# amidos2006/gym-pcgrl

Hardware: AMD Instinct MI355X
Metric: env-steps/sec (whole node), binary-narrow 14x14 @ 65536 envs (higher is better)
Workload: dtype u8; 1 GPU; binary-narrow-v0 14x14, 65536 envs/GPU; envs_per_gpu=65536, width=14, height=14, max_changes=39, actions=uniform random, device-generated before the timed region, parallelism=env-axis shard x1, no collective on the step path

## Files before the change

### gym_pcgrl_amd/_lib.py

```python
import ctypes as C
import os
import subprocess

PKG = os.path.dirname(os.path.abspath(__file__))
ROOT = os.path.dirname(PKG)
CSRC = os.path.join(PKG, "csrc")
LIBDIR = os.path.join(PKG, "lib")
SO = os.path.join(LIBDIR, "libpcgrl_hip.so")
SOURCES = [os.path.join(CSRC, "pcgrl_abi.hip")]
HIPCC_FLAGS = ["--offload-arch=gfx950", "-O3", "-std=c++17", "-ffp-contract=off", "-fPIC", "-shared", "-mllvm", "-amdgpu-sched-strategy=max-ilp"]

PCGRL_OK, PCGRL_EINVAL, PCGRL_EHIP, PCGRL_ESTATE = 0, -1, -2, -3


class Config(C.Structure):
    _fields_ = [(n, C.c_int32) for n in (
        "prob", "rep", "num_envs", "width", "height", "prob_width", "prob_height", "max_changes", "max_iterations",
        "random_start", "random_tile", "warp", "random_probs", "auto_reset", "target_path",
        "max_enemies", "target_enemy_dist", "max_crates", "target_solution", "solver_power", "max_potions",
        "max_treasures", "max_diamonds", "min_spikes", "target_jumps", "min_empty", "min_enemies", "min_jumps")] + [
        ("target_col_enemies", C.c_double), ("tile_probs", C.c_double * 8), ("rewards", C.c_double * 12)]


class Layout(C.Structure):
    _fields_ = [(n, C.c_int32) for n in ("group", "mask_bytes", "nplanes", "nstats")] + [
        (n, C.c_size_t) for n in ("map", "old_map", "heatmap", "pos", "planes", "counters", "stats", "start_stats",
                                  "info", "reward", "done", "tile_p", "rng_rep", "rng_prob", "rng_cursor", "scratch")]


TUNING_FIELDS = ("no_fused", "fused_zelda", "step_epb", "no_inc", "inline_reset", "pair_min", "no_wide", "wide_waves", "wide_grid",
                 "wide_pairs", "wide_few", "sok_generic", "sok_hard_cap", "sok_spawn", "md_only_agent", "smb_lds_heap", "full_per_wave", "inc_per_wave", "wide_spin", "step_prio", "no_touch", "touch_tight", "step_pair", "async_split", "big_team", "obs_at_end", "touch_resume",
                 "changes_grid", "changes_chunk")


class Tuning(C.Structure):
    _fields_ = [(n, C.c_int32) for n in TUNING_FIELDS]


TUNING_OVERRIDES = {}


def make_tuning(overrides=None):
    t = Tuning(*([-1] * len(TUNING_FIELDS)))
    for k, v in list(TUNING_OVERRIDES.items()) + list((overrides or {}).items()):
        if k not in TUNING_FIELDS:
            raise KeyError("unknown tuning switch %r (known: %s)" % (k, ", ".join(TUNING_FIELDS)))
        setattr(t, k, int(v))
    return t


BUFFER_NAMES = ("map", "old_map", "heatmap", "pos", "planes", "counters", "stats", "start_stats", "info", "reward",
                "done", "tile_p", "rng_rep", "rng_prob", "rng_cursor", "scratch")


class Buffers(C.Structure):
    _fields_ = [(n, C.c_void_p) for n in BUFFER_NAMES]


ROW_FIELDS = ("actions_out", "reward", "done", "start_in", "start_out", "ep_return", "ep_length", "took", "fresh")


class Row(C.Structure):
    _fields_ = [(n, C.c_void_p) for n in ROW_FIELDS] + [("actions_i64", C.c_int32)]


class RenderDesc(C.Structure):
    _fields_ = [("indices", C.c_void_p), ("count", C.c_int32), ("tiles", C.c_void_p), ("tile_size", C.c_int32),
                ("border_x", C.c_int32), ("border_y", C.c_int32), ("border_tile", C.c_int32), ("cursor", C.c_int32),
                ("grid_rows", C.c_int32), ("grid_cols", C.c_int32), ("out", C.c_void_p)]


class TileGraphDesc(C.Structure):
    _fields_ = [("maps", C.c_void_p), ("count", C.c_int32), ("passable", C.c_uint32), ("source_tiles", C.c_uint32), ("reach_tiles", C.c_uint32),
                ("sources", C.c_void_p), ("regions_out", C.c_void_p), ("longest_out", C.c_void_p), ("labels_out", C.c_void_p),
                ("dist_out", C.c_void_p), ("reach_out", C.c_void_p), ("source_out", C.c_void_p)]


ABI_VERSION = 15
EXPORTS = ("pcgrl_abi_version", "pcgrl_error_string", "pcgrl_last_hip_error", "pcgrl_query_layout", "pcgrl_create",
           "pcgrl_destroy", "pcgrl_bind", "pcgrl_configure", "pcgrl_seed", "pcgrl_set_tile_probs", "pcgrl_reset",
           "pcgrl_step", "pcgrl_set_maps", "pcgrl_observe", "pcgrl_action_map", "pcgrl_status", "pcgrl_profile",
           "pcgrl_profile_read", "pcgrl_bind_episode_stats", "pcgrl_seed_words", "pcgrl_rollout", "pcgrl_bind_observation", "pcgrl_selftest_heap",
           "pcgrl_tuning_defaults", "pcgrl_set_tuning", "pcgrl_clear_status", "pcgrl_step_flat",
           "pcgrl_async_bytes", "pcgrl_bind_async", "pcgrl_step_async", "pcgrl_async_flush", "pcgrl_step_multi", "pcgrl_selftest_step_pool", "pcgrl_step_threads", "pcgrl_selftest_range_reward",
           "pcgrl_bind_row", "pcgrl_render", "pcgrl_get_stats_bytes", "pcgrl_get_stats", "pcgrl_get_reward",
           "pcgrl_get_solution_bytes", "pcgrl_get_solution", "pcgrl_get_playthrough_bytes", "pcgrl_get_playthrough",
           "pcgrl_get_smb_play_bytes", "pcgrl_get_smb_play", "pcgrl_get_paths_legs", "pcgrl_get_paths_bytes", "pcgrl_get_paths",
           "pcgrl_get_changes_bytes", "pcgrl_get_changes", "pcgrl_tile_graph_bytes", "pcgrl_tile_graph")
NPHASE = 6
PHASES = ("update", "stats", "reset_or_idle", "solver_or_reset", "reset2", "solver2")


def sources_newer_than_lib():
    if not os.path.exists(SO):
        return True
    t = os.path.getmtime(SO)
    deps = [os.path.join(CSRC, f) for f in os.listdir(CSRC)] + [os.path.join(ROOT, "include", "pcgrl_hip.h")]
    return any(os.path.getmtime(d) > t for d in deps)


def source_hash():
    import hashlib
    h = hashlib.sha256()
    files = sorted(os.path.join(CSRC, f) for f in os.listdir(CSRC)) + [os.path.join(ROOT, "include", "pcgrl_hip.h")]
    h.update(" ".join(HIPCC_FLAGS).encode() + b"\0")
    for f in files:
        h.update(os.path.basename(f).encode() + b"\0")
        with open(f, "rb") as fh:
            h.update(fh.read())
    return h.hexdigest()[:16]


NPARTS = 8


def build(force=False, verbose=False, jobs=None):
    if not force and not sources_newer_than_lib():
        return SO
    os.makedirs(LIBDIR, exist_ok=True)
    objdir = os.path.join(LIBDIR, "obj")
    os.makedirs(objdir, exist_ok=True)
    hipcc = os.environ.get("HIPCC", "hipcc")
    flags = [f for f in HIPCC_FLAGS if f != "-shared"]
    jobs = jobs or int(os.environ.get("PCGRL_BUILD_JOBS", "0")) or min(NPARTS, os.cpu_count() or 1)
    objs = [os.path.join(objdir, "part%d.o" % k) for k in range(NPARTS)]
    cmds = [[hipcc] + flags + ["-DPCGRL_PART=%d" % k, "-c", SOURCES[0], "-o", objs[k]] for k in range(NPARTS)]
    running, todo, failed = [], list(range(NPARTS)), []
    while todo or running:
        while todo and len(running) < jobs:
            k = todo.pop(0)
            if verbose:
                print(" ".join(cmds[k]), flush=True)
            running.append((k, subprocess.Popen(cmds[k])))
        k, p = running.pop(0)
        if p.wait() != 0:
            failed.append(k)
    if failed:
        raise subprocess.CalledProcessError(1, cmds[failed[0]])
    link = [hipcc, "--offload-arch=gfx950", "-shared", "-fPIC"] + objs + ["-o", SO]
    if verbose:
        print(" ".join(link), flush=True)
    subprocess.check_call(link)
    return SO


_lib = None


def load():
    global _lib, SO
    if _lib is not None:
        return _lib
    SO = os.environ.get("PCGRL_HIP_SO", SO)
    if not os.path.exists(SO):
        raise RuntimeError(
            "gym_pcgrl_amd: HIP library %s is missing. Build it with `python -c 'import __graft_entry__ as g; g.build()'` "
            "(hipcc --offload-arch=gfx950). There is no CPU fallback for the batched environment." % SO)
    import torch
    L = C.CDLL(SO)
    for name in EXPORTS:
        if not hasattr(L, name):
            raise RuntimeError("gym_pcgrl_amd: %s does not export %s (stale build?)" % (SO, name))
    L.pcgrl_abi_version.restype = C.c_int
    if L.pcgrl_abi_version() != ABI_VERSION:
        raise RuntimeError("gym_pcgrl_amd: %s has ABI version %d, this package needs %d (stale build?)" % (SO, L.pcgrl_abi_version(), ABI_VERSION))
    L.pcgrl_error_string.restype = C.c_char_p
    L.pcgrl_error_string.argtypes = [C.c_int]
    L.pcgrl_last_hip_error.restype = C.c_int
    L.pcgrl_query_layout.argtypes = [C.POINTER(Config), C.POINTER(Layout)]
    L.pcgrl_create.argtypes = [C.POINTER(Config), C.POINTER(C.c_void_p)]
    L.pcgrl_destroy.argtypes = [C.c_void_p]
    L.pcgrl_tuning_defaults.argtypes = [C.POINTER(Tuning)]
    L.pcgrl_tuning_defaults.restype = None
    L.pcgrl_set_tuning.argtypes = [C.c_void_p, C.POINTER(Tuning)]
    L.pcgrl_bind.argtypes = [C.c_void_p, C.POINTER(Buffers), C.c_void_p]
    L.pcgrl_configure.argtypes = [C.c_void_p, C.POINTER(Config)]
    L.pcgrl_seed.argtypes = [C.c_void_p, C.c_void_p, C.c_int32, C.c_int32, C.c_void_p]
    L.pcgrl_seed_words.argtypes = [C.c_void_p, C.c_void_p, C.c_int32, C.c_int32, C.c_void_p]
    L.pcgrl_set_tile_probs.argtypes = [C.c_void_p, C.c_void_p]
    L.pcgrl_reset.argtypes = [C.c_void_p, C.c_void_p]
    L.pcgrl_step.argtypes = [C.c_void_p, C.c_void_p, C.c_void_p]
    L.pcgrl_rollout.argtypes = [C.c_void_p, C.c_void_p, C.c_int32, C.c_void_p, C.c_void_p, C.c_void_p, C.c_void_p]
    L.pcgrl_set_maps.argtypes = [C.c_void_p, C.c_void_p, C.c_void_p]
    L.pcgrl_observe.argtypes = [C.c_void_p, C.c_void_p, C.c_int32, C.c_int32, C.c_int32, C.c_int32, C.c_int32, C.c_void_p]
    L.pcgrl_bind_observation.argtypes = [C.c_void_p, C.c_void_p, C.c_int32, C.c_int32, C.c_int32, C.c_int32, C.c_int32, C.c_int32]
    L.pcgrl_bind_row.argtypes = [C.c_void_p, C.POINTER(Row)]
    L.pcgrl_render.argtypes = [C.c_void_p, C.POINTER(RenderDesc), C.c_void_p]
    L.pcgrl_get_stats_bytes.argtypes = [C.POINTER(Config), C.c_int32]
    L.pcgrl_get_stats_bytes.restype = C.c_size_t
    L.pcgrl_get_stats.argtypes = [C.c_void_p, C.c_void_p, C.c_int32, C.c_void_p, C.c_void_p, C.c_size_t, C.c_void_p]
    L.pcgrl_get_reward.argtypes = [C.c_void_p, C.c_void_p, C.c_void_p, C.c_int32, C.c_void_p, C.c_void_p, C.c_void_p]
    moves_args = (C.c_void_p, C.c_void_p, C.c_int32, C.c_int32, C.c_void_p, C.c_void_p, C.c_void_p, C.c_void_p, C.c_void_p, C.c_size_t, C.c_void_p)
    for name in ("pcgrl_get_solution", "pcgrl_get_playthrough", "pcgrl_get_smb_play"):
        getattr(L, name + "_bytes").argtypes = [C.POINTER(Config), C.c_int32, C.c_int32]
        getattr(L, name + "_bytes").restype = C.c_size_t
        getattr(L, name).argtypes = list(moves_args)
    L.pcgrl_get_paths_legs.argtypes = [C.POINTER(Config)]
    L.pcgrl_get_paths_legs.restype = C.c_int32
    L.pcgrl_get_paths_bytes.argtypes = [C.POINTER(Config), C.c_int32, C.c_int32]
    L.pcgrl_get_paths_bytes.restype = C.c_size_t
    L.pcgrl_get_paths.argtypes = [C.c_void_p, C.c_void_p, C.c_int32, C.c_int32, C.c_void_p, C.c_void_p, C.c_void_p, C.c_void_p, C.c_size_t, C.c_void_p]
    L.pcgrl_get_changes_bytes.argtypes = [C.POINTER(Config), C.c_int32, C.c_int32]
    L.pcgrl_get_changes_bytes.restype = C.c_size_t
    L.pcgrl_get_changes.argtypes = [C.c_void_p, C.c_void_p, C.c_int32, C.c_void_p, C.c_int32, C.c_void_p, C.c_void_p, C.c_void_p, C.c_void_p, C.c_void_p,
                                    C.c_void_p, C.c_size_t, C.c_void_p]
    L.pcgrl_tile_graph_bytes.argtypes = [C.POINTER(Config), C.c_int32]
    L.pcgrl_tile_graph_bytes.restype = C.c_size_t
    L.pcgrl_tile_graph.argtypes = [C.c_void_p, C.POINTER(TileGraphDesc), C.c_void_p, C.c_size_t, C.c_void_p]
    L.pcgrl_action_map.argtypes = [C.c_void_p, C.c_void_p, C.c_void_p, C.c_void_p]
    L.pcgrl_step_flat.argtypes = [C.c_void_p, C.c_void_p, C.c_void_p, C.c_void_p]
    L.pcgrl_selftest_heap.argtypes = [C.c_void_p, C.c_int32, C.c_void_p, C.c_void_p, C.c_void_p, C.c_void_p]
    L.pcgrl_selftest_step_pool.argtypes = [C.c_int32, C.c_int32, C.c_int32, C.c_void_p]
    L.pcgrl_selftest_range_reward.argtypes = [C.c_void_p, C.c_int32, C.c_void_p, C.c_void_p]
    L.pcgrl_step_threads.argtypes = [C.c_int32]
    L.pcgrl_step_threads.restype = C.c_int32
    L.pcgrl_status.argtypes = [C.c_void_p, C.c_void_p, C.POINTER(C.c_int32)]
    L.pcgrl_clear_status.argtypes = [C.c_void_p, C.c_void_p]
    L.pcgrl_profile.argtypes = [C.c_void_p, C.c_int]
    L.pcgrl_bind_episode_stats.argtypes = [C.c_void_p, C.c_void_p, C.c_void_p, C.c_void_p, C.c_void_p, C.c_void_p]
    L.pcgrl_profile_read.argtypes = [C.c_void_p, C.POINTER(C.c_double), C.POINTER(C.c_int32)]
    L.pcgrl_async_bytes.argtypes = [C.POINTER(Config), C.c_int32]
    L.pcgrl_async_bytes.restype = C.c_size_t
    L.pcgrl_bind_async.argtypes = [C.c_void_p, C.c_void_p, C.c_size_t, C.c_int32, C.c_void_p]
    L.pcgrl_step_async.argtypes = [C.c_void_p, C.c_void_p, C.c_int32, C.c_void_p]
    L.pcgrl_async_flush.argtypes = [C.c_void_p, C.c_void_p]
    L.pcgrl_step_multi.argtypes = [C.POINTER(C.c_void_p), C.POINTER(C.c_void_p), C.POINTER(C.c_void_p), C.c_int32]
    _lib = L
    return L


def check(rc, what):
    if rc != 0:
        L = load()
        msg = L.pcgrl_error_string(rc).decode()
        extra = " (hipError %d)" % L.pcgrl_last_hip_error() if rc == PCGRL_EHIP else ""
        raise RuntimeError("gym_pcgrl_amd: %s failed: %s%s" % (what, msg, extra))
```

### gym_pcgrl_amd/csrc/kernels_stats.h

```cpp
#pragma once
template <class MaskT>
__device__ __forceinline__ MaskT row_valid(int lane, int W, int H) {
    MaskT full = (W >= (int)(8 * sizeof(MaskT))) ? ~(MaskT)0 : (((MaskT)1 << W) - 1);
    return lane < H ? full : (MaskT)0;
}

template <int PROB = -1>
__device__ __forceinline__ bool finalize_item(const PcgrlParams& P, const DevBufs& B, int e, const int32_t* s,
                                              int mode, int parity, int shard, bool push_reset = true, int rst_list = WL_RST,
                                              const int2* pre = nullptr, const double* reward_pre = nullptr) {
    const int prob = PROB >= 0 ? PROB : P.prob;
    int32_t* st = B.stats + (size_t)e * 8;
    int32_t* start = B.start_stats + (size_t)e * 8;
    if (mode == MODE_STEP) {
        int32_t old[PCGRL_MAX_STATS], sv[PCGRL_MAX_STATS];
        for (int k = 0; k < 8; k++) { old[k] = st[k]; sv[k] = start[k]; }
        const int2 c = pre ? *pre : reinterpret_cast<const int2*>(B.counters)[e];
        const double r = reward_pre ? *reward_pre : compute_reward(P, s, old, prob);
        const bool d = episode_over(P, s, sv, prob) || c.y >= P.max_changes || c.x >= P.max_iterations;
        B.reward[e] = r;
        B.done[e] = d ? 1 : 0;
        episode_account(B, e, r, d);
        int32_t* inf = B.info + (size_t)e * 10;
#pragma unroll
        for (int k = 0; k < 8; k++) {
            st[k] = s[k];
            inf[k] = (prob == PCGRL_PROB_BINARY && k == 2) ? s[1] - sv[1] : ((prob == PCGRL_PROB_BINARY && k == 3) ? 0 : s[k]);
        }
        inf[8] = c.x; inf[9] = c.y;
        if (d && P.auto_reset && push_reset) wl_push(B, parity, rst_list, shard, e);
        return d && P.auto_reset;
    } else {
        for (int k = 0; k < 8; k++) st[k] = s[k];
        if (mode == MODE_START)
            for (int k = 0; k < 8; k++) start[k] = s[k];
    }
    return false;
}

template <int PROB, class G, class MaskT>
__device__ __forceinline__ bool compute_item_stats(G& g, const PcgrlParams& P, MaskT b0, MaskT b1, MaskT b2, MaskT valid, int32_t* s,
                                                   int32_t* status, MaskT& champ, bool tight = true) {
    champ = 0;
    if (PROB == PCGRL_PROB_BINARY) {
        int regions, path;
        if (G::kGroup == 16) {
            int ub2;
            regions_and_longest_path(g, (MaskT)(~b0 & valid), regions, path, champ, ub2, tight);
            s[3] = ub2 + 1;
        } else {
            regions_and_longest_path(g, (MaskT)(~b0 & valid), regions, path, champ);
        }
        s[0] = regions; s[1] = path; s[2] = g.any(champ) ? 1 : 0;
        return false;
    }
    if (PROB == PCGRL_PROB_ZELDA) { zelda_stats(g, P, b0, b1, b2, valid, s); return false; }
    if (PROB == PCGRL_PROB_MDUNGEON) return mdungeon_stats(g, P, b0, b1, b2, valid, s);
    if (PROB == PCGRL_PROB_DDAVE) {
        bool overflow = false;
        const bool ns = ddave_stats(g, P, b0, b1, b2, valid, s, &overflow);
        if (overflow && g.lane == 0) atomicOr(status, PCGRL_STATUS_TOO_MANY_CRATES);
        return ns;
    }
    if (PROB == PCGRL_PROB_SMB) return true;
    return sokoban_stats(g, P, b0, b1, b2, valid, s);
}
template <int PROB, class G, class MaskT>
__device__ __forceinline__ bool compute_item_stats(G& g, const PcgrlParams& P, MaskT b0, MaskT b1, MaskT b2, MaskT valid, int32_t* s, int32_t* status) {
    MaskT champ;
    return compute_item_stats<PROB>(g, P, b0, b1, b2, valid, s, status, champ);
}

template <int PROB = -1>
__device__ __forceinline__ bool finish_or_park(const PcgrlParams& P, const DevBufs& B, int e, const int32_t* s, bool need_solver,
                                               int mode, int parity, int shard, bool push_reset = true, int park_list = -1,
                                               const double* reward_pre = nullptr) {
    if (need_solver) {
        int32_t* park = (mode == MODE_STEP) ? B.info + (size_t)e * 10 : B.stats + (size_t)e * 8;
        for (int k = 0; k < 8; k++) park[k] = s[k];
        wl_push(B, parity, park_list >= 0 ? park_list : (mode == MODE_STEP ? WL_SOL : WL_SOL2), shard, e);
        return false;
    }
    return finalize_item<PROB>(P, B, e, s, mode, parity, shard, push_reset, WL_RST, nullptr, reward_pre);
}

template <int J>
__device__ __forceinline__ double dpp_down(double v) {
    const long long b = __double_as_longlong(v);
    const int lo = __builtin_amdgcn_update_dpp(0, (int)b, 0x100 + J, 0xF, 0xF, true), hi = __builtin_amdgcn_update_dpp(0, (int)(b >> 32), 0x100 + J, 0xF, 0xF, true);
    return __longlong_as_double(((long long)hi << 32) | (unsigned)lo);
}
__device__ __forceinline__ void zelda_reward_tab(const PcgrlParams& P, ZeldaRewardTab* T) {
    T->w[0] = P.rewards[0]; T->w[1] = P.rewards[1]; T->w[2] = P.rewards[2]; T->w[3] = P.rewards[4]; T->w[4] = P.rewards[3];
    T->w[5] = P.rewards[5]; T->w[6] = P.rewards[6]; T->w[7] = 0.0;
    T->lo[0] = 1; T->lo[1] = 1; T->lo[2] = 1; T->lo[3] = 2; T->lo[4] = 1; T->lo[5] = P.target_enemy_dist; T->lo[6] = PCGRL_IPOS; T->lo[7] = 0;
    T->hi[0] = 1; T->hi[1] = 1; T->hi[2] = 1; T->hi[3] = P.max_enemies; T->hi[4] = 1; T->hi[5] = PCGRL_IPOS; T->hi[6] = PCGRL_IPOS; T->hi[7] = 0;
}
__device__ __forceinline__ double zelda_reward_lanes(const ZeldaRewardTab* T, const int32_t* old, const int32_t* s, int k) {
    const int s0 = s[0], s1 = s[1], s2 = s[2], s3 = s[3], s4 = s[4], s5 = s[5], s6 = s[6];
    int n = s6;
    n = k == 5 ? s5 : n; n = k == 4 ? s4 : n; n = k == 3 ? s3 : n; n = k == 2 ? s2 : n; n = k == 1 ? s1 : n; n = k == 0 ? s0 : n;
    const int kk = k & 7;
    const int o = old[kk];
    const double t = k < 7 ? (double)range_reward_i(n, o, T->lo[kk], T->hi[kk]) * T->w[kk] : 0.0;
    double r = t;
    r = r + dpp_down<1>(t); r = r + dpp_down<2>(t); r = r + dpp_down<3>(t);
    r = r + dpp_down<4>(t); r = r + dpp_down<5>(t); r = r + dpp_down<6>(t);
    return r;
}

template <int PROB, int G, class MaskT, bool FUSED = false>
__device__ __forceinline__ void stats_wave_task(const PcgrlParams& P, const DevBufs& B, DevGroup<G, MaskT>& g, int lane64, int gw, bool lone,
                                                bool inc, bool pair, bool zinc, bool have, int raw, int shard, int mode, int parity,
                                                int inline_reset, int gen_map, uint32_t* mt, uint8_t* tiles, MaskT rowmask,
                                                StepLocal* SL = nullptr, bool step_obs = false) {
    constexpr bool kCanReset = PROB == PCGRL_PROB_BINARY || PROB == PCGRL_PROB_ZELDA;
    if (!kCanReset) inline_reset = 0;
    constexpr int GPW = 64 / G;
    constexpr bool kInc = PROB == PCGRL_PROB_BINARY;
    constexpr bool kZinc = PROB == PCGRL_PROB_ZELDA && G == 16 && sizeof(MaskT) == 4;
    constexpr int NPL = (PROB == PCGRL_PROB_BINARY) ? 1 : 3;
    MaskT* champ_base = reinterpret_cast<MaskT*>(B.champ);
    const bool tch = kInc && G == 16 && !inc && !lone && have && raw < 0;
    const bool packed = inc || (kZinc && zinc && !lone) || tch;
    const bool reset_only = have && !packed && (raw & WL_RESET_ONLY) != 0;
    const bool compute = have && !reset_only && !(lone && (gw & 1));
    const int e = packed ? wl_inc_env<G>(raw) : (raw & ~WL_RESET_ONLY);
    MaskT* planes_e = reinterpret_cast<MaskT*>(B.planes) + (size_t)e * NPL * G;
    MaskT b0 = 0, b1 = 0, b2 = 0;
    if (compute) {
        b0 = planes_e[g.lane * NPL];
        if (NPL > 1) { b1 = planes_e[g.lane * NPL + 1]; b2 = planes_e[g.lane * NPL + 2]; }
    }
    if (GPW >= 2 && lone && inline_reset) {
        const int role = gw & 1;
        int2 pre = make_int2(0, 0);
        if (g.lane == 0 && role == 0 && have) pre = reinterpret_cast<const int2*>(B.counters)[e];
        asm volatile("s_waitcnt vmcnt(0)" ::: "memory");
#pragma unroll
        for (int k = 0; k < GPW / 2; k++) {
            if (k > 0 && !pair) break;
            if (!__builtin_amdgcn_readlane((int)have, 2 * k * G)) continue;
            const int ek = __builtin_amdgcn_readlane(e, 2 * k * G);
            const int step_draws = (SL && P.rep == PCGRL_REP_NARROW && P.random_tile) ? 1 : 0;
            if (SL && lane64 == 0) SL->dirty[ek - SL->e0] = 1;
            ResetRows rr;
            wave_reset_env<PROB, !FUSED, FUSED>(P, B, ek, gen_map, mt, (uint8_t*)nullptr, lane64, step_draws, gw == 2 * k + 1 ? g.lane : -1, &rr);
            MaskT t0, t1, t2;
            reset_rows_to_planes<MaskT>(P, reinterpret_cast<MaskT*>(B.planes) + (size_t)ek * NPL * G, gw == 2 * k + 1 ? g.lane : -1, rr.m0, rr.m1, rr.m2, t0, t1, t2);
            if (gw == 2 * k + 1) { b0 = t0; b1 = t1; b2 = t2; }
            __builtin_amdgcn_wave_barrier();
        }
        TL(9);
        const bool act = have && (role == 1 || !reset_only);
        int32_t sl[PCGRL_MAX_STATS] = {0, 0, 0, 0, 0, 0, 0, 0};
        MaskT champ_l = 0;
        bool ns = false;
        if (act) ns = compute_item_stats<PROB>(g, P, b0, b1, b2, rowmask, sl, B.status, champ_l, (B.step_tight & 2) != 0);
        TL(10);
        constexpr bool kLaneReward = PROB == PCGRL_PROB_ZELDA && G == 16;
        double rpre = 0.0;
        if (kLaneReward && SL && role == 0 && act) rpre = zelda_reward_lanes(&SL->zr, B.stats + (size_t)e * 8, sl, g.lane);
        if (g.lane == 0 && role == 0 && act) finalize_item<PROB>(P, B, e, sl, MODE_STEP, parity, shard, false, WL_RST, &pre, (kLaneReward && SL) ? &rpre : nullptr);
        __builtin_amdgcn_wave_barrier();
        if (role == 1 && have) {
            if (kInc && champ_base) champ_base[(size_t)e * G + g.lane] = champ_l;
            if (g.lane == 0) finish_or_park<PROB>(P, B, e, sl, ns, MODE_START, parity, shard);
        }
        if (FUSED && step_obs) {
#pragma unroll
            for (int k = 0; k < GPW / 2; k++) {
                if (k > 0 && !pair) break;
                if (!__builtin_amdgcn_readlane((int)have, 2 * k * G)) continue;
                const ObsPlanes<MaskT, NPL> src = {reinterpret_cast<const MaskT*>(B.planes), G};
                obs_write_env_lean(src, obs_view_from_lds(&SL->obs_v), B.pos, __builtin_amdgcn_readlane(e, 2 * k * G), lane64);
            }
        }
        return;
    }
    int32_t s[PCGRL_MAX_STATS] = {0, 0, 0, 0, 0, 0, 0, 0};
    bool need_solver = false;
    MaskT champ = 0;
    if (kInc && inc) {
        if (compute) {
            const MaskT cbit = (g.lane == wl_inc_row<G>(raw)) ? (MaskT)1 << wl_inc_col<G>(raw) : (MaskT)0;
            const MaskT champ_old = champ_base[(size_t)e * G + g.lane];
            const int4 old = *reinterpret_cast<const int4*>(B.stats + (size_t)e * 8);
            int regions, path, ub2;
            binary_incremental(g, (MaskT)(~b0 & rowmask), cbit, wl_inc_code<G>(raw) != 0, old.x, old.y, champ_old, old.w - 1, regions, path, champ, ub2);
            s[0] = regions; s[1] = path; s[2] = 1; s[3] = ub2 + 1;
        }
    } else if (kZinc && packed) {
        if (compute) {
            const MaskT cbit = (g.lane == wl_inc_row<G>(raw)) ? (MaskT)1 << wl_inc_col<G>(raw) : (MaskT)0;
            zelda_stats(g, P, b0, b1, b2, rowmask, s, (int)wl_inc_code<G>(raw), cbit, B.stats[(size_t)e * 8 + 4]);
        }
    } else {
        bool full = compute;
        if (kInc && G == 16) {
            const bool t = compute && tch;
            TouchMemo<MaskT> memo = touch_memo_empty(g, b0);
            if (t) {
                const MaskT cbit = (g.lane == wl_inc_row<G>(raw)) ? (MaskT)1 << wl_inc_col<G>(raw) : (MaskT)0;
                const MaskT champ_old = champ_base[(size_t)e * G + g.lane];
                const int4 old = *reinterpret_cast<const int4*>(B.stats + (size_t)e * 8);
                int regions, path, ub2;
                if (binary_touch(g, (MaskT)(~b0 & rowmask), cbit, (wl_inc_code<G>(raw) & 1u) != 0, old.x, champ_old, old.w - 1, regions, path, champ, ub2, memo)) {
                    s[0] = regions; s[1] = path; s[2] = 1; s[3] = ub2 + 1;
                    full = false;
                }
            }
#ifdef PCGRL_TIMELINE
            {
                const uint64_t gu = __ballot(t && full && g.lane == 0), pl = __ballot(compute && !tch && g.lane == 0);
                TL(32 + __popcll(gu) + 8 * __popcll(pl));
            }
#endif
            constexpr bool kResume = FUSED && sizeof(MaskT) == 4;
            if (kResume && B.touch_resume) {
                if (full) {
                    int regions, path, ub2;
                    rlp_resume(g, (MaskT)(~b0 & rowmask), memo, regions, path, champ, ub2, (B.step_tight & 1) != 0);
                    s[0] = regions; s[1] = path; s[2] = g.any(champ) ? 1 : 0; s[3] = ub2 + 1;
                }
                full = false;
            }
        }
        if (full) need_solver = compute_item_stats<PROB>(g, P, b0, b1, b2, rowmask, s, B.status, champ, (B.step_tight & 1) != 0);
    }
    if (kInc && compute && champ_base) champ_base[(size_t)e * G + g.lane] = champ;
    TL(10);
    int want_reset = 0;
    constexpr bool kLaneReward = PROB == PCGRL_PROB_ZELDA && G == 16;
    double rpre = 0.0;
    const bool lane_reward = kLaneReward && SL != nullptr && mode == MODE_STEP;
    if (lane_reward && have && !reset_only) rpre = zelda_reward_lanes(&SL->zr, B.stats + (size_t)e * 8, s, g.lane);
    if (g.lane == 0 && have) {
        if (reset_only) want_reset = 1;
        else want_reset = finish_or_park<PROB>(P, B, e, s, need_solver, mode, parity, shard, !inline_reset, -1, lane_reward ? &rpre : nullptr) ? 1 : 0;
    }
    if (inline_reset) {
        const uint64_t want = __ballot(want_reset != 0);
        TL(11);
        if (want) {
            TL(12);
            if (SL) { while (__hip_atomic_load(&SL->refill_done[SL->par], __ATOMIC_ACQUIRE, __HIP_MEMORY_SCOPE_WORKGROUP) < SL->need) __builtin_amdgcn_s_sleep(2); }
            bool mine = false;
#pragma unroll
            for (int k = 0; k < GPW; k++) {
                if ((want >> (k * G)) & 1ull) {
                    const int ek = __builtin_amdgcn_readlane(e, k * G);
                    if (SL && lane64 == 0) { SL->dirty[ek - SL->e0] = 1; SL->late[ek - SL->e0] = 1; SL->n_late = 1; }
                    int pend = 0;
                    if (SL) {
                        if (lane64 == 0) {
                            pend = atomicExch(&SL->pend[ek - SL->e0], 0);
                            if (pend < 0) {
                                while (__hip_atomic_load(&SL->late_done[(ek - SL->e0) >> 6], __ATOMIC_ACQUIRE, __HIP_MEMORY_SCOPE_WORKGROUP) == 0) __builtin_amdgcn_s_sleep(2);
                                pend = 0;
                            }
                        }
                        pend = __builtin_amdgcn_readfirstlane(pend);
                    }
                    ResetRows rr;
                    wave_reset_env<PROB, !FUSED, FUSED>(P, B, ek, gen_map, mt, (uint8_t*)nullptr, lane64, 0, gw == k ? g.lane : -1, &rr, pend);
                    MaskT t0, t1, t2;
                    reset_rows_to_planes<MaskT>(P, reinterpret_cast<MaskT*>(B.planes) + (size_t)ek * NPL * G, gw == k ? g.lane : -1, rr.m0, rr.m1, rr.m2, t0, t1, t2);
                    if (gw == k) { b0 = t0; b1 = t1; b2 = t2; mine = true; }
                    __builtin_amdgcn_wave_barrier();
                }
            }
            if (mine) {
                int32_t st[PCGRL_MAX_STATS] = {0, 0, 0, 0, 0, 0, 0, 0};
                const bool ns = compute_item_stats<PROB>(g, P, b0, b1, b2, rowmask, st, B.status, champ, (B.step_tight & 2) != 0);
                if (kInc && champ_base) champ_base[(size_t)e * G + g.lane] = champ;
                if (g.lane == 0) finish_or_park<PROB>(P, B, e, st, ns, MODE_START, parity, shard);
            }
        }
    }
}

template <int PROB, int G, class MaskT>
__global__ __launch_bounds__(PCGRL_BLOCK) __attribute__((amdgpu_waves_per_eu(4, 8))) void k_stats(PcgrlParams P, DevBufs B, int list, int parity, int mode, int clear_parity,
                                                        int inline_reset, int gen_map, int lone0) {
    extern __shared__ __attribute__((aligned(16))) uint8_t smem[];
    __shared__ int s_pref[WL_NSHARD + 1], s_pref_inc[WL_NSHARD + 1], s_pref_rst[WL_NSHARD + 1];
    if (clear_parity >= 0 && blockIdx.x == 0) wl_clear(B, clear_parity);
    DevGroup<G, MaskT> g;
    constexpr int GPB = PCGRL_BLOCK / G, GPW = 64 / G;
    constexpr bool kInc = PROB == PCGRL_PROB_BINARY;
    constexpr bool kZinc = PROB == PCGRL_PROB_ZELDA && G == 16 && sizeof(MaskT) == 4;
    const bool zinc = kZinc && mode == MODE_STEP && B.zelda_inc;
    const bool with_inc = (kInc && mode == MODE_STEP && B.champ != nullptr) || zinc;
    int n_inc = 0, n_rst = 0;
    const int n_full = (with_inc || lone0 == 2 || list < 0) ? wl_load_prefix3(B, parity, list, with_inc ? WL_INC : -1, lone0 == 2 ? WL_RST : -1,
                                                                              s_pref, s_pref_inc, s_pref_rst, &n_inc, &n_rst)
                                                             : wl_load_prefix(B, parity, list, s_pref);
    const int n0 = lone0 == 1 ? s_pref[1] : (lone0 == 2 ? n_rst : 0);
    const int f0 = lone0 == 1 ? n0 : 0;
    const int w_full = (n_full - f0 + GPW - 1) / GPW;
    const bool pair = GPW >= 4 && n0 >= B.pair_min;
    const int w_lone = pair ? (n0 + 1) >> 1 : n0;
    const int w_total = w_lone + w_full + (n_inc + GPW - 1) / GPW;
    MaskT* champ_base = reinterpret_cast<MaskT*>(B.champ);
    const int lane64 = threadIdx.x & 63, wv = threadIdx.x >> 6, gw = lane64 / G;
    const int NPL = (PROB == PCGRL_PROB_BINARY) ? 1 : 3;
    const int W = P.width, H = P.height;
    uint32_t* mt = reinterpret_cast<uint32_t*>(smem + (size_t)wv * reset_stage_bytes(W * H));
    uint8_t* tiles = reinterpret_cast<uint8_t*>(mt + PCGRL_MT_N);
    const MaskT rowmask = row_valid<MaskT>(g.lane, W, H);
    for (int wid = blockIdx.x * (PCGRL_BLOCK / 64) + wv; wid < w_total; wid += gridDim.x * (PCGRL_BLOCK / 64)) {
        const bool lone = wid < w_lone;
        const bool inc = wid >= w_lone + w_full;
        const int item = lone ? (pair ? 2 * wid + (gw >> 1) : wid) : (inc ? (wid - w_lone - w_full) * GPW + gw : f0 + (wid - w_lone) * GPW + gw);
        const bool have = lone ? (item < n0 && (pair || gw < 2)) : item < (inc ? n_inc : n_full);
        const bool from_rst = lone && lone0 == 2;
        const int raw = !have ? 0 : (inc ? wl_get(B, WL_INC, s_pref_inc, item) : (from_rst ? wl_get(B, WL_RST, s_pref_rst, item) : wl_get(B, list, s_pref, item)));
        const int shard = (item >> 4) & (WL_NSHARD - 1);
        stats_wave_task<PROB, G, MaskT>(P, B, g, lane64, gw, lone, inc, pair, zinc, have, raw, shard, mode, parity, inline_reset, gen_map, mt, tiles, rowmask);
    }
}

template <class MaskT>
struct LdsShared {
    MaskT* rest; int* bestp; int lane;
    __device__ __forceinline__ MaskT load_rest() const { return *reinterpret_cast<volatile MaskT*>(rest + lane); }
    template <class G>
    __device__ __forceinline__ bool retire(G& g, MaskT comp) const {
        const MaskT fb = g.first_bit(comp);
        MaskT old = 0;
        if (fb) old = atomicAnd(rest + lane, ~fb);
        const bool won = __ballot((old & fb) != 0) != 0;
        if (comp) atomicAnd(rest + lane, ~comp);
        return won;
    }
    __device__ __forceinline__ int best() const { return *reinterpret_cast<volatile int*>(bestp); }
    __device__ __forceinline__ void raise(int v) const { if (lane == 0 && v > 0) atomicMax(bestp, v); }
};
template <class MaskT>
__device__ __forceinline__ void block_regions_and_path(DevGroup<64, MaskT>& g, MaskT pass, int tw, int ts, int lane, int H,
                                                       MaskT* s_rest, int* s_regions, int* s_best, int* s_owner, MaskT* champ_e) {
    const int bh = (H + ts - 1) / ts;
    const int row_lo = tw * bh, row_hi = (row_lo + bh < H) ? row_lo + bh : H;
    int tiny_regions, tiny_path;
    TL(20);
    const MaskT nontiny = rlp_prepare(g, pass, tiny_regions, tiny_path);
    TL(21);
    if (tw == 0) {
        s_rest[lane] = nontiny;
        if (lane == 0) { *s_regions = tiny_regions; *s_best = tiny_path; *s_owner = -1; }
    }
    __syncthreads();
    LdsShared<MaskT> sh = {s_rest, s_best, lane};
    int regions = 0, my_best = 0;
    MaskT my_champ = 0;
    MaskT rest = sh.load_rest();
    if (g.any(rest)) {
        const PcgFillCtx<DevGroup<64, MaskT>> ctx = pcg_fill_ctx(g, pass);
        do {
            rlp_process_seed(g, rlp_choose_seed(g, rest, row_lo, row_hi), ctx, sh, regions, my_best, my_champ);
            rest = sh.load_rest();
        } while (g.any(rest));
    }
    TL(22);
    if (lane == 0 && regions) atomicAdd(s_regions, regions);
    __syncthreads();
    TL(23);
    if (lane == 0 && my_best > tiny_path && my_best == *s_best) atomicCAS(s_owner, -1, tw);
    __syncthreads();
    if (champ_e) {
        const int owner = *s_owner;
        if (tw == (owner < 0 ? 0 : owner)) champ_e[lane] = owner < 0 ? (MaskT)0 : my_champ;
    }
}

template <class MaskT>
__device__ __forceinline__ void wave_incremental_item(const PcgrlParams& P, const DevBufs& B, DevGroup<64, MaskT>& g, int raw, int parity,
                                                      int inline_reset, int gen_map, uint32_t* mt, uint8_t* tiles, int lane, MaskT rowmask) {
    const int e = wl_inc_env<64>(raw);
    MaskT* planes_e = reinterpret_cast<MaskT*>(B.planes) + (size_t)e * 64;
    MaskT* champ_e = reinterpret_cast<MaskT*>(B.champ) + (size_t)e * 64;
    const MaskT b0 = planes_e[lane];
    const MaskT champ_old = champ_e[lane];
    const int2 old = *reinterpret_cast<const int2*>(B.stats + (size_t)e * 8);
    const MaskT cbit = (lane == wl_inc_row<64>(raw)) ? (MaskT)1 << wl_inc_col<64>(raw) : (MaskT)0;
    int regions, path;
    MaskT champ;
    binary_incremental(g, (MaskT)(~b0 & rowmask), cbit, wl_inc_code<64>(raw) != 0, old.x, old.y, champ_old, regions, path, champ);
    champ_e[lane] = champ;
    int want = 0;
    if (lane == 0) {
        int32_t s[PCGRL_MAX_STATS] = {regions, path, 1, 0, 0, 0, 0, 0};
        want = finalize_item<PCGRL_PROB_BINARY>(P, B, e, s, MODE_STEP, parity, e & (WL_NSHARD - 1), !inline_reset) ? 1 : 0;
    }
    want = __builtin_amdgcn_readfirstlane(want);
    if (inline_reset && want) {
        ResetRows rr;
        wave_reset_env<PCGRL_PROB_BINARY>(P, B, e, gen_map, mt, (uint8_t*)nullptr, lane, 0, lane, &rr);
        MaskT n0, n1, n2;
        reset_rows_to_planes<MaskT>(P, planes_e, lane, rr.m0, rr.m1, rr.m2, n0, n1, n2);
        int32_t st[PCGRL_MAX_STATS] = {0, 0, 0, 0, 0, 0, 0, 0};
        compute_item_stats<PCGRL_PROB_BINARY>(g, P, n0, n1, n2, rowmask, st, B.status, champ);
        champ_e[lane] = champ;
        if (lane == 0) finalize_item<PCGRL_PROB_BINARY>(P, B, e, st, MODE_START, parity, e & (WL_NSHARD - 1));
    }
}

#define WIDE_SPIN_LIMIT 400
__device__ __forceinline__ int wide_claim(int32_t* word, int epoch, int who) {
    int cur = __hip_atomic_load(word, __ATOMIC_RELAXED, __HIP_MEMORY_SCOPE_AGENT);
    for (;;) {
        if ((cur >> 1) == epoch) return 0;
        const int seen = atomicCAS(word, cur, (epoch << 1) | who);
        if (seen == cur) return 1;
        cur = seen;
    }
}

template <class MaskT, int NWAVES>
__global__ __launch_bounds__(NWAVES * 64) void k_stats_wide(PcgrlParams P, DevBufs B, int list, int parity, int mode, int clear_parity,
                                                             int inline_reset, int gen_map, int pair_few) {
    extern __shared__ __attribute__((aligned(16))) uint8_t smem[];
    __shared__ int s_pref[WL_NSHARD + 1], s_pref_rst[WL_NSHARD + 1], s_pref_inc[WL_NSHARD + 1];
    __shared__ MaskT s_rest[2][64];
    __shared__ int s_regions[2], s_best[2], s_owner[2], s_flag, s_flag2[2], s_cur, s_claim;
    __shared__ int2 s_pre;
    if (clear_parity >= 0 && blockIdx.x == 0) wl_clear(B, clear_parity);
// ... 167 lines not shown
```

### gym_pcgrl_amd/csrc/kernels_step.h

```cpp
#pragma once

struct StepLds { int planes, champ, stats, start, cnt, cur, fifo, tag, pos, act, flat, in_total, info, rew, done, total; };
__host__ __device__ constexpr StepLds step_lds_layout(int plane_row_bytes, int champ_row_bytes, bool fifo, int action_width, int epb) {
    StepLds L = {};
    int o = 0;
    L.planes = o; o += epb * plane_row_bytes;
    L.champ = o; o += epb * champ_row_bytes;
    L.stats = o; o += epb * 32;
    L.start = o; o += epb * 32;
    L.cnt = o; o += epb * 8;
    L.cur = o; o += epb * 8;
    L.fifo = o; o += fifo ? epb * PCGRL_FIFO_N * 4 : 0;
    L.tag = o; o += fifo ? epb * 4 : 0;
    L.pos = o; o += epb * 2;
    L.act = o; o += epb * 4 * action_width;
    L.flat = o; o += action_width == 3 ? epb * 4 : 0;
    L.in_total = o;
    L.info = o; o += epb * 40;
    L.rew = o; o += epb * 8;
    L.done = o; o += epb;
    L.total = (o + 15) & ~15;
    return L;
}

template <int TPB>
__device__ __forceinline__ void blk_copy(uint8_t* dst, const uint8_t* src, int bytes) {
    const int nv = bytes >> 4;
    for (int i = threadIdx.x; i < nv; i += TPB) reinterpret_cast<uint4*>(dst)[i] = reinterpret_cast<const uint4*>(src)[i];
    for (int i = (nv << 4) + threadIdx.x; i < bytes; i += TPB) dst[i] = src[i];
}
template <int TPB>
__device__ __forceinline__ void blk_copy_rows(uint8_t* dst, const uint8_t* src, int rows, int row, const uint8_t* flag) {
    const int per = row >> 4;
    for (int i = threadIdx.x; i < rows * per; i += TPB)
        if (flag[i / per]) reinterpret_cast<uint4*>(dst)[i] = reinterpret_cast<const uint4*>(src)[i];
}

template <int TPB, int C, int SLOT0, int NV>
__device__ __forceinline__ void seg_load_c(uint4& rc, const void* g, bool on, int tid) {
    if (C * TPB + TPB - 1 < SLOT0 || C * TPB >= SLOT0 + NV) return;
    const int slot = C * TPB + tid;
    if (on && slot >= SLOT0 && slot < SLOT0 + NV) rc = reinterpret_cast<const uint4*>(g)[slot - SLOT0];
}
#define PCGRL_SEG_LOAD(SLOT0, NV, G, ON) do { const void* g_ = (G); const bool on_ = (ON); \
    seg_load_c<TPB, 0, SLOT0, NV>(r0, g_, on_, tid0); seg_load_c<TPB, 1, SLOT0, NV>(r1, g_, on_, tid0); seg_load_c<TPB, 2, SLOT0, NV>(r2, g_, on_, tid0); \
    seg_load_c<TPB, 3, SLOT0, NV>(r3, g_, on_, tid0); seg_load_c<TPB, 4, SLOT0, NV>(r4, g_, on_, tid0); seg_load_c<TPB, 5, SLOT0, NV>(r5, g_, on_, tid0); \
    seg_load_c<TPB, 6, SLOT0, NV>(r6, g_, on_, tid0); seg_load_c<TPB, 7, SLOT0, NV>(r7, g_, on_, tid0); seg_load_c<TPB, 8, SLOT0, NV>(r8, g_, on_, tid0); } while (0)
template <int TPB, int C, int TOTAL>
__device__ __forceinline__ void seg_store_c(uint8_t* smem, const uint4& rc, int tid) {
    if (C * TPB >= TOTAL) return;
    const int slot = C * TPB + tid;
    if (slot < TOTAL) reinterpret_cast<uint4*>(smem)[slot] = rc;
}

__device__ __forceinline__ void fifo_refill(const DevBufs& B, int e, int k, int cur0) {
    uint32_t* ring = B.rng_rep + (size_t)e * PCGRL_MT_N;
    uint32_t* fl = B.fifo + (size_t)e * PCGRL_FIFO_N;
    const int base = mt_wrap(cur0 + PCGRL_FIFO_N), basem = mt_wrap(base + PCGRL_MT_M);
    uint32_t a[PCGRL_FIFO_N + 1], m[PCGRL_FIFO_N];
#pragma unroll
    for (int i = 0; i <= PCGRL_FIFO_N; i++) a[i] = (i <= k) ? ring[mt_wrap(base + i)] : 0u;
#pragma unroll
    for (int i = 0; i < PCGRL_FIFO_N; i++) m[i] = (i < k) ? ring[mt_wrap(basem + i)] : 0u;
#pragma unroll
    for (int i = 0; i < PCGRL_FIFO_N; i++) if (i < k) ring[mt_wrap(cur0 + i)] = fl[i];
#pragma unroll
    for (int j = 0; j < PCGRL_FIFO_N; j++) if (j + k < PCGRL_FIFO_N) fl[j] = fl[j + k];
#pragma unroll
    for (int i = 0; i < PCGRL_FIFO_N; i++) if (i < k) fl[PCGRL_FIFO_N - k + i] = mt_twist(a[i], a[i + 1], m[i]);
    B.fifo_tag[e] = mt_wrap(cur0 + k);
}

__device__ __forceinline__ void step_set_prio(int p) {
    if (p == 0) __builtin_amdgcn_s_setprio(0);
    else if (p == 1) __builtin_amdgcn_s_setprio(1);
    else if (p == 2) __builtin_amdgcn_s_setprio(2);
    else __builtin_amdgcn_s_setprio(3);
}

template <int PROB, int REP, class MaskT, bool MULTI, int EPB, bool OBS = false, bool ROW = false>
__global__ __launch_bounds__(EPB * 4) __attribute__((amdgpu_waves_per_eu(4, 8))) void k_step(PcgrlParams P, DevBufs Bg, const int32_t* __restrict__ actions, int parity, int gen_map,
                                                                                                     int steps, size_t action_stride, double* reward_out, uint8_t* done_out, int32_t* info_out) {
    extern __shared__ __attribute__((aligned(16))) uint8_t smem[];
    constexpr int TPB = EPB * 4, NUPD = EPB / 64;
    __shared__ int s_items[3][EPB];
    __shared__ int s_n[2][4];
    __shared__ StepLocal s_loc;
    __shared__ int s_obs_ticket;
    static_assert(!(OBS && MULTI), "the tape form writes its images at the end");
    static_assert(!(ROW && MULTI), "the tape form has its own outputs (pcgrl_rollout ignores the row binding)");
    constexpr int G = 16, GPW = 4;
    constexpr int NPL = (PROB == PCGRL_PROB_BINARY) ? 1 : 3;
    constexpr int kPlaneRow = G * NPL * (int)sizeof(MaskT);
    const int W = P.width, H = P.height;
    TL_INIT(); TL(1);
    const int e0 = blockIdx.x * EPB;
    const int ne = (P.num_envs - e0) < EPB ? (P.num_envs - e0) : EPB;
    const bool has_champ = PROB == PCGRL_PROB_BINARY && Bg.champ != nullptr;
    const bool has_fifo = REP == PCGRL_REP_NARROW && Bg.fifo != nullptr;
    constexpr int kChampRow = PROB == PCGRL_PROB_BINARY ? G * (int)sizeof(MaskT) : 0;
    constexpr int AW = REP == PCGRL_REP_WIDE ? 3 : 1;
    constexpr StepLds L = step_lds_layout(kPlaneRow, kChampRow, REP == PCGRL_REP_NARROW, AW, EPB);
    const int champ_row = kChampRow;
    DevBufs B = Bg;
    const size_t cells_ = (size_t)W * H;
    B.map = Bg.map + (size_t)e0 * cells_;
    B.old_map = Bg.old_map + (size_t)e0 * cells_;
    B.heat = Bg.heat + (size_t)e0 * cells_;
    B.tile_p = Bg.tile_p + (size_t)e0 * 2;
    B.rng_rep = Bg.rng_rep + (size_t)e0 * PCGRL_MT_N;
    if (Bg.rng_prob) B.rng_prob = Bg.rng_prob + (size_t)e0 * PCGRL_MT_N;
    if (Bg.ep_return) { B.ep_return = Bg.ep_return + e0; B.ep_length = Bg.ep_length + e0; B.last_return = Bg.last_return + e0; B.last_length = Bg.last_length + e0; }
    B.planes = smem + L.planes;
    if (has_champ) B.champ = smem + L.champ;
    B.stats = reinterpret_cast<int32_t*>(smem + L.stats);
    B.start_stats = reinterpret_cast<int32_t*>(smem + L.start);
    B.info = reinterpret_cast<int32_t*>(smem + L.info);
    B.reward = reinterpret_cast<double*>(smem + L.rew);
    B.counters = reinterpret_cast<int32_t*>(smem + L.cnt);
    B.rng_cur = reinterpret_cast<int32_t*>(smem + L.cur);
    if (has_fifo) {
        B.fifo = reinterpret_cast<uint32_t*>(smem + L.fifo);
        B.fifo_tag = reinterpret_cast<int32_t*>(smem + L.tag);
    } else {
        B.fifo = nullptr; B.fifo_tag = nullptr;
    }
    B.pos = smem + L.pos;
    B.done = smem + L.done;
    const int32_t* act_lds = reinterpret_cast<const int32_t*>(smem + L.act);
    const uint8_t* g_planes = reinterpret_cast<const uint8_t*>(Bg.planes) + (size_t)e0 * kPlaneRow;
    const uint8_t* g_champ = has_champ ? reinterpret_cast<const uint8_t*>(Bg.champ) + (size_t)e0 * champ_row : nullptr;
    const bool row_fl = ROW && AW == 3 && Bg.flat;
    const int row_per = row_fl ? 1 : AW;
    const size_t row_a0 = (size_t)e0 * row_per + threadIdx.x;
    const bool row_have = ROW && (int)threadIdx.x < ne * row_per;
    int64_t row_act = 0;
    static_assert(AW <= 4, "one action value per thread");
    if (row_have) {
        const int32_t* src = row_fl ? Bg.flat : actions;
        row_act = Bg.act_i64 ? reinterpret_cast<const int64_t*>(src)[row_a0] : (int64_t)src[row_a0];
    }
    if (ne == EPB) {
        static_assert(L.in_total / 16 <= 9 * TPB, "nine 16-byte slots per thread");
        uint4 r0 = {}, r1 = {}, r2 = {}, r3 = {}, r4 = {}, r5 = {}, r6 = {}, r7 = {}, r8 = {};
        const int tid0 = (int)threadIdx.x;
        PCGRL_SEG_LOAD(L.planes / 16, EPB * kPlaneRow / 16, g_planes, true);
        if (kChampRow) PCGRL_SEG_LOAD(L.champ / 16, (kChampRow ? EPB * kChampRow / 16 : 1), g_champ, has_champ);
        PCGRL_SEG_LOAD(L.stats / 16, EPB * 2, Bg.stats + (size_t)e0 * 8, true);
        PCGRL_SEG_LOAD(L.start / 16, EPB * 2, Bg.start_stats + (size_t)e0 * 8, true);
        PCGRL_SEG_LOAD(L.cnt / 16, EPB / 2, Bg.counters + (size_t)e0 * 2, true);
        PCGRL_SEG_LOAD(L.cur / 16, EPB / 2, Bg.rng_cur + (size_t)e0 * 2, true);
        if (REP == PCGRL_REP_NARROW) {
            PCGRL_SEG_LOAD(L.fifo / 16, EPB * PCGRL_FIFO_N * 4 / 16, has_fifo ? Bg.fifo + (size_t)e0 * PCGRL_FIFO_N : nullptr, has_fifo);
            PCGRL_SEG_LOAD(L.tag / 16, EPB / 4, has_fifo ? Bg.fifo_tag + e0 : nullptr, has_fifo);
        }
        PCGRL_SEG_LOAD(L.pos / 16, EPB / 8, Bg.pos + (size_t)e0 * 2, true);
        if (!ROW) PCGRL_SEG_LOAD(L.act / 16, EPB / 4 * AW, actions + (size_t)e0 * AW, !(AW == 3 && Bg.flat));
        if (!ROW && AW == 3) PCGRL_SEG_LOAD(L.flat / 16, (AW == 3 ? EPB / 4 : 1), Bg.flat ? Bg.flat + e0 : nullptr, Bg.flat != nullptr);
        asm volatile("" ::: "memory");
        static_assert(L.act % 16 == 0, "the prefetch ends on a slot boundary in front of the actions");
        constexpr int TOT = (ROW ? L.act : L.in_total) / 16;
        seg_store_c<TPB, 0, TOT>(smem, r0, tid0); seg_store_c<TPB, 1, TOT>(smem, r1, tid0); seg_store_c<TPB, 2, TOT>(smem, r2, tid0);
        seg_store_c<TPB, 3, TOT>(smem, r3, tid0); seg_store_c<TPB, 4, TOT>(smem, r4, tid0); seg_store_c<TPB, 5, TOT>(smem, r5, tid0);
        seg_store_c<TPB, 6, TOT>(smem, r6, tid0); seg_store_c<TPB, 7, TOT>(smem, r7, tid0); seg_store_c<TPB, 8, TOT>(smem, r8, tid0);
    } else {
        blk_copy<TPB>(smem + L.planes, g_planes, ne * kPlaneRow);
        if (has_champ) blk_copy<TPB>(smem + L.champ, g_champ, ne * champ_row);
        blk_copy<TPB>(smem + L.stats, reinterpret_cast<const uint8_t*>(Bg.stats + (size_t)e0 * 8), ne * 32);
        blk_copy<TPB>(smem + L.start, reinterpret_cast<const uint8_t*>(Bg.start_stats + (size_t)e0 * 8), ne * 32);
        blk_copy<TPB>(smem + L.cnt, reinterpret_cast<const uint8_t*>(Bg.counters + (size_t)e0 * 2), ne * 8);
        blk_copy<TPB>(smem + L.cur, reinterpret_cast<const uint8_t*>(Bg.rng_cur + (size_t)e0 * 2), ne * 8);
        blk_copy<TPB>(smem + L.pos, Bg.pos + (size_t)e0 * 2, ne * 2);
        if (has_fifo) {
            blk_copy<TPB>(smem + L.fifo, reinterpret_cast<const uint8_t*>(Bg.fifo + (size_t)e0 * PCGRL_FIFO_N), ne * PCGRL_FIFO_N * 4);
            blk_copy<TPB>(smem + L.tag, reinterpret_cast<const uint8_t*>(Bg.fifo_tag + e0), ne * 4);
        }
        if (ROW) {}
        else if (AW == 3 && Bg.flat) blk_copy<TPB>(smem + L.flat, reinterpret_cast<const uint8_t*>(Bg.flat + e0), ne * 4);
        else blk_copy<TPB>(smem + L.act, reinterpret_cast<const uint8_t*>(actions + (size_t)e0 * AW), ne * 4 * AW);
    }
    if (row_have) {
        reinterpret_cast<int32_t*>(smem + (row_fl ? L.flat : L.act))[threadIdx.x] = (int32_t)row_act;
        if (Bg.row.actions_out) Bg.row.actions_out[row_a0] = row_act;
    }
    if (threadIdx.x < EPB) { s_loc.dirty[threadIdx.x] = 0; if (OBS) { s_loc.obs_skip[threadIdx.x] = 0; s_loc.late[threadIdx.x] = 0; } }
    if (threadIdx.x < 8) s_n[threadIdx.x >> 2][threadIdx.x & 3] = 0;
    if (threadIdx.x == 0) { s_loc.e0 = 0; s_loc.need = NUPD; s_loc.refill_done[0] = 0; s_loc.refill_done[1] = 0; s_loc.n_late = 0; s_obs_ticket = 0; }
    constexpr int OBS_PER_TASK = 8;
    const bool obs_delta = OBS && REP == PCGRL_REP_WIDE && NPL == 3 && Bg.obs.delta;
    const int n_obs = (OBS && !obs_delta) ? (ne + OBS_PER_TASK - 1) / OBS_PER_TASK : 0;
    const ObsPlanes<MaskT, NPL> obs_src = {reinterpret_cast<const MaskT*>(smem + L.planes), G};
    if (OBS && threadIdx.x == 0) s_loc.obs_v = obs_view(P, Bg.obs, e0);
    if (PROB == PCGRL_PROB_ZELDA && threadIdx.x == 64) zelda_reward_tab(P, &s_loc.zr);
    uint8_t* reset_scratch = smem + L.total;
#pragma clang loop unroll(disable)
  for (int t = 0; t < (MULTI ? steps : 1); t++) {
    int tid = (int)threadIdx.x;
    if (MULTI) asm volatile("" : "+v"(tid));
    const int lane64 = tid & 63, wv = tid >> 6, gw = lane64 / G;
    const int sp = t & 1;
    DevGroup<G, MaskT> g(lane64);
    if (MULTI && t > 0) {
        const int32_t* row = actions + (size_t)t * action_stride + (size_t)e0 * AW;
        for (int i = tid; i < ne * AW; i += TPB) reinterpret_cast<int32_t*>(smem + L.act)[i] = row[i];
    }
    __syncthreads();
    TL(17);
    const int prio = B.step_prio, prio_nfull = (prio >> 8) & 15;
    int prio_now = 0;
    if (wv < NUPD) {
        if ((prio >> 6) & 3) { prio_now = (prio >> 6) & 3; step_set_prio(prio_now); }
        const int e = wv * 64 + lane64;
        UpdateOut u = {};
        UpdateMid mid = {};
        if (REP == PCGRL_REP_WIDE && !MULTI && Bg.flat && e < ne) {
            const int dim = P.ntiles, total = W * H * dim;
            int a = reinterpret_cast<const int32_t*>(smem + L.flat)[e];
            if (a < 0 || a >= total) atomicOr(B.status, PCGRL_STATUS_BAD_ACTION);
            a = a < 0 ? 0 : (a >= total ? total - 1 : a);
            int32_t* t3 = reinterpret_cast<int32_t*>(smem + L.act) + 3 * e;
            const int q = a / dim;
            t3[0] = q % W; t3[1] = q / W; t3[2] = a - q * dim;
        }
        if (e < ne) u = update_env<REP, MaskT, true, true, true>(P, B, act_lds, e, &mid);
        TL(2);
        const bool first = u.rst || u.sure_done;
        const bool packed_full = PROB == PCGRL_PROB_ZELDA && B.zelda_inc;
        int dest = -1, v = e;
        if (first) { dest = 0; v = u.rst ? (e | WL_RESET_ONLY) : e; }
        else if (u.chg) { dest = u.cheap ? 2 : 1; v = (u.cheap || packed_full) ? u.inc_item : ((u.touch && B.step_touch) ? (u.inc_item | (int)0x80000000) : e); }
        if (u.chg) s_loc.dirty[e] = 1;
        if (OBS && first && e < EPB) s_loc.obs_skip[e] = 1;
        const uint64_t m0 = __ballot(dest == 0), m1 = __ballot(dest == 1), m2 = __ballot(dest == 2);
        const uint64_t below = (1ull << lane64) - 1ull;
        int b0 = 0, b1 = 0, b2 = 0;
        if (lane64 == 0) {
            b0 = m0 ? atomicAdd(&s_n[sp][0], __popcll(m0)) : 0;
            b1 = m1 ? atomicAdd(&s_n[sp][1], __popcll(m1)) : 0;
            b2 = m2 ? atomicAdd(&s_n[sp][2], __popcll(m2)) : 0;
            if (wv == 0) { s_n[sp ^ 1][0] = 0; s_n[sp ^ 1][1] = 0; s_n[sp ^ 1][2] = 0; s_n[sp ^ 1][3] = 0; s_loc.refill_done[sp ^ 1] = 0; s_loc.par = sp; }
        }
        b0 = __builtin_amdgcn_readfirstlane(b0); b1 = __builtin_amdgcn_readfirstlane(b1); b2 = __builtin_amdgcn_readfirstlane(b2);
        if (dest == 0) s_items[0][b0 + __popcll(m0 & below)] = v;
        if (dest == 2) s_items[2][b2 + __popcll(m2 & below)] = v;
        {
            const int lvl = (u.bucket >> 3) & 7;
            int pos1 = 0;
#pragma unroll
            for (int b = 0; b < 8; b++) {
                const uint64_t mb = __ballot(dest == 1 && lvl == b);
                pos1 += b > lvl ? __popcll(mb) : (b == lvl ? __popcll(mb & below) : 0);
            }
            if (dest == 1) s_items[1][b1 + pos1] = v;
        }
        asm volatile("s_waitcnt lgkmcnt(0)" ::: "memory");
        __builtin_amdgcn_s_barrier();
        int k_used = 0, cur0 = 0;
        if (lane64 == 0) s_loc.late_done[wv] = 0;
        if (e < ne && !first) update_env_cursor<REP, MaskT>(P, B, e, mid, k_used, cur0);
        if (OBS && REP == PCGRL_REP_WIDE && NPL == 3 && obs_delta && e < ne && !first && u.chg) obs_write_delta_piece(obs_src, obs_view_from_lds(&s_loc.obs_v), e, act_lds[3 * e], act_lds[3 * e + 1]);
        if (e < EPB) s_loc.pend[e] = (has_fifo && e < ne && !first) ? k_used : 0;
        asm volatile("s_waitcnt vmcnt(0) lgkmcnt(0)" ::: "memory");
        if (lane64 == 0) __hip_atomic_fetch_add(&s_loc.refill_done[sp], 1, __ATOMIC_RELEASE, __HIP_MEMORY_SCOPE_WORKGROUP);
    }
    int n0 = 0, n1 = 0, n2 = 0, w_full = 0, w_total = 0, w_lone = 0;
    bool stats_left = true, obs_left = OBS;
    bool pair = false;
    const int fpw = B.step_fpw, ipw = B.step_ipw;
    const int tiles_bytes = (W * H + 15) & ~15;
    uint32_t* mt = reinterpret_cast<uint32_t*>(reset_scratch + (size_t)wv * (PCGRL_MT_N * 4 + tiles_bytes));
    uint8_t* tiles = reinterpret_cast<uint8_t*>(mt + PCGRL_MT_N);
    const MaskT rowmask = row_valid<MaskT>(g.lane, W, H);
    const bool zinc = PROB == PCGRL_PROB_ZELDA && sizeof(MaskT) == 4 && B.zelda_inc;
    for (bool first_round = true;; first_round = false) {
        if (first_round) {
            if (wv >= NUPD) {
                asm volatile("s_waitcnt lgkmcnt(0)" ::: "memory");
                __builtin_amdgcn_s_barrier();
                asm volatile("" ::: "memory");
            }
            TL(3);
            n0 = s_n[sp][0]; n1 = s_n[sp][1]; n2 = s_n[sp][2];
            w_full = (n1 + fpw - 1) / fpw;
            pair = PROB == PCGRL_PROB_ZELDA && B.step_pair > 0 && n0 >= B.step_pair;
            w_lone = pair ? (n0 + 1) >> 1 : n0;
            w_total = w_lone + w_full + (n2 + ipw - 1) / ipw;
        }
        if (OBS && !first_round && obs_left) {
            int oid = 0;
            if (lane64 == 0) oid = atomicAdd(&s_obs_ticket, 1);
            oid = __builtin_amdgcn_readfirstlane(oid);
            if (oid >= n_obs) obs_left = false;
            else {
                if (prio_now) { prio_now = 0; step_set_prio(0); }
                while (__hip_atomic_load(&s_loc.refill_done[sp], __ATOMIC_ACQUIRE, __HIP_MEMORY_SCOPE_WORKGROUP) < NUPD) __builtin_amdgcn_s_sleep(2);
                const int o0 = oid * OBS_PER_TASK;
                const ObsView V = obs_view_from_lds(&s_loc.obs_v);
#pragma clang loop unroll(disable)
                for (int j = 0; j < OBS_PER_TASK; j++) {
                    const int eo = o0 + j;
                    if (eo < ne && !s_loc.obs_skip[eo]) obs_write_env_lean(obs_src, V, smem + L.pos, eo, lane64);
                }
            }
        }
        if (!stats_left) { if (!OBS || !obs_left) break; continue; }
        int wid = 0;
        if (lane64 == 0) wid = atomicAdd(&s_n[sp][3], 1);
        wid = __builtin_amdgcn_readfirstlane(wid);
        TL(18);
        if (wid >= w_total) { stats_left = false; if (!OBS || !obs_left) break; continue; }
        const bool lone = wid < w_lone, inc = wid >= w_lone + w_full;
        const int item = lone ? (pair ? 2 * wid + (gw >> 1) : wid) : (inc ? (wid - w_lone - w_full) * ipw + gw : (wid - w_lone) * fpw + gw);
        const bool have = lone ? (item < n0 && (pair || gw < 2)) : (gw < (inc ? ipw : fpw) && item < (inc ? n2 : n1));
        const int raw = have ? s_items[lone ? 0 : (inc ? 2 : 1)][item] : 0;
        TL(lone ? 4 : (inc ? 6 : 5));
        if (prio) {
            const int want = lone ? (prio & 3) : (inc ? ((prio >> 4) & 3) : ((prio_nfull == 0 || wid - w_lone < prio_nfull) ? ((prio >> 2) & 3) : 0));
            if (want != prio_now) { prio_now = want; step_set_prio(want); }
        }
        stats_wave_task<PROB, G, MaskT, true>(P, B, g, lane64, gw, lone, inc, PROB == PCGRL_PROB_ZELDA && pair, zinc, have, raw, lane64, MODE_STEP, parity, 1, gen_map, mt, tiles, rowmask, &s_loc, OBS);
        TL(7);
    }
    if (prio_now) { prio_now = 0; step_set_prio(0); }
    if (has_fifo && wv < NUPD) {
        const int e = wv * 64 + lane64;
        int k = 0;
        if (e < ne) k = atomicExch(&s_loc.pend[e], -1);
        if (k > 0) {
            int c0 = B.rng_cur[2 * e] - k;
            c0 = c0 < 0 ? c0 + PCGRL_MT_N : c0;
            fifo_refill(B, e, k, c0);
        }
        asm volatile("s_waitcnt vmcnt(0) lgkmcnt(0)" ::: "memory");
        if (lane64 == 0) __hip_atomic_store(&s_loc.late_done[wv], 1, __ATOMIC_RELEASE, __HIP_MEMORY_SCOPE_WORKGROUP);
    }
    TL(8);
    if (MULTI && (reward_out || done_out || info_out)) {
        __syncthreads();
        const size_t row = (size_t)t * P.num_envs + e0;
        if (reward_out && tid < ne) reward_out[row + tid] = reinterpret_cast<const double*>(smem + L.rew)[tid];
        if (done_out && tid >= TPB / 2 && tid - TPB / 2 < ne) done_out[row + tid - TPB / 2] = smem[L.done + tid - TPB / 2];
        if (info_out) for (int i = tid; i < ne * 10; i += TPB) info_out[row * 10 + i] = reinterpret_cast<const int32_t*>(smem + L.info)[i];
    }
  }
    __syncthreads();
    blk_copy<TPB>(reinterpret_cast<uint8_t*>(Bg.stats + (size_t)e0 * 8), smem + L.stats, ne * 32);
    blk_copy<TPB>(reinterpret_cast<uint8_t*>(Bg.info + (size_t)e0 * 10), smem + L.info, ne * 40);
    blk_copy<TPB>(reinterpret_cast<uint8_t*>(Bg.reward + e0), smem + L.rew, ne * 8);
    blk_copy<TPB>(reinterpret_cast<uint8_t*>(Bg.counters + (size_t)e0 * 2), smem + L.cnt, ne * 8);
    blk_copy<TPB>(reinterpret_cast<uint8_t*>(Bg.rng_cur + (size_t)e0 * 2), smem + L.cur, ne * 8);
    blk_copy<TPB>(Bg.pos + (size_t)e0 * 2, smem + L.pos, ne * 2);
    blk_copy<TPB>(Bg.done + e0, smem + L.done, ne);
    if (has_fifo) {
        blk_copy<TPB>(reinterpret_cast<uint8_t*>(Bg.fifo + (size_t)e0 * PCGRL_FIFO_N), smem + L.fifo, ne * PCGRL_FIFO_N * 4);
        blk_copy<TPB>(reinterpret_cast<uint8_t*>(Bg.fifo_tag + e0), smem + L.tag, ne * 4);
    }
    blk_copy_rows<TPB>(reinterpret_cast<uint8_t*>(Bg.planes) + (size_t)e0 * kPlaneRow, smem + L.planes, ne, kPlaneRow, s_loc.dirty);
    if (has_champ) blk_copy_rows<TPB>(reinterpret_cast<uint8_t*>(Bg.champ) + (size_t)e0 * champ_row, smem + L.champ, ne, champ_row, s_loc.dirty);
    blk_copy_rows<TPB>(reinterpret_cast<uint8_t*>(Bg.start_stats + (size_t)e0 * 8), smem + L.start, ne, 32, s_loc.dirty);
    if (ROW) {
        const RowBind& R = Bg.row;
        const int q = (int)threadIdx.x / EPB, i = (int)threadIdx.x % EPB;
        if (i < ne) {
            const uint8_t d = smem[L.done + i] ? 1 : 0;
            if (q == 0) { if (R.reward) R.reward[e0 + i] = reinterpret_cast<const double*>(smem + L.rew)[i]; }
            else if (q == 1) {
                if (R.done) R.done[e0 + i] = d;
                if (R.start_out) R.start_out[e0 + i] = d;
                if (R.took) R.took[e0 + i] = 1;
                if (R.fresh) R.fresh[e0 + i] = 1;
            }
            else if (q == 2) { if (R.ep_return) R.ep_return[e0 + i] = d ? Bg.last_return[e0 + i] : __longlong_as_double(0x7FF8000000000000ll); }
            else if (R.ep_length) R.ep_length[e0 + i] = d ? Bg.last_length[e0 + i] : 0;
        }
    }
    if (!OBS && Bg.obs.out && Bg.obs.fused) {
        const ObsPlanes<MaskT, NPL> src = {reinterpret_cast<const MaskT*>(smem + L.planes), G};
        obs_write_block_lean(src, obs_view(P, Bg.obs, e0), smem + L.pos, ne, REP == PCGRL_REP_WIDE && !MULTI && Bg.obs.delta, act_lds, s_loc.dirty,
                             smem + L.done, (int)threadIdx.x, TPB);
    }
    if (OBS && s_loc.n_late) {
        asm volatile("s_waitcnt vmcnt(0)" ::: "memory");
        __syncthreads();
        const ObsView V = obs_view_from_lds(&s_loc.obs_v);
        for (int eo = __builtin_amdgcn_readfirstlane((int)threadIdx.x >> 6); eo < ne; eo += TPB >> 6)
            if (s_loc.late[eo]) obs_write_env_lean(obs_src, V, smem + L.pos, eo, (int)threadIdx.x & 63);
    }
}
```

### gym_pcgrl_amd/csrc/lanegroup_dev.h

```cpp
#pragma once
#include <hip/hip_runtime.h>
#include "pcgrl_common.h"
#include "bfs_asm.h"

template <int CTRL>
__device__ __forceinline__ uint32_t dpp_mov0(uint32_t v) {
    return (uint32_t)__builtin_amdgcn_update_dpp(0, (int)v, CTRL, 0xF, 0xF, true);
}
template <int CTRL>
__device__ __forceinline__ uint64_t dpp_mov0(uint64_t v) {
    uint32_t lo = dpp_mov0<CTRL>((uint32_t)v), hi = dpp_mov0<CTRL>((uint32_t)(v >> 32));
    return ((uint64_t)hi << 32) | lo;
}
__device__ __forceinline__ int pcg_popc(uint32_t v) { return __popc(v); }
__device__ __forceinline__ int pcg_popc(uint64_t v) { return __popcll(v); }
__device__ __forceinline__ uint32_t pcg_brev(uint32_t v) { return __brev(v); }
__device__ __forceinline__ uint64_t pcg_brev(uint64_t v) { return __brevll(v); }

template <class MaskT>
struct DevLaneOps {
    typedef MaskT mask_t;
    typedef int ivec_t;
    __device__ __forceinline__ ivec_t izero() const { return 0; }
    __device__ __forceinline__ bool wave_any(mask_t m) const { return __ballot(m != 0) != 0; }
    __device__ __forceinline__ ivec_t popc_lanes(mask_t m) const { return pcg_popc(m); }
    __device__ __forceinline__ ivec_t isel_ne(mask_t a, mask_t b, int x, ivec_t y) const { return a != b ? x : y; }
    __device__ __forceinline__ mask_t msel_ne(mask_t a, mask_t b, mask_t x, mask_t y) const { return a != b ? x : y; }
    __device__ __forceinline__ mask_t keep_where_eq(ivec_t v, int x, mask_t m) const { return v == x ? m : (mask_t)0; }
    __device__ __forceinline__ mask_t bitrev(mask_t m) const { return pcg_brev(m); }
};

template <int G, class MaskT>
struct DevGroup;

template <class MaskT>
struct DevGroup<16, MaskT> : DevLaneOps<MaskT> {
    typedef MaskT mask_t;
    enum { kGroup = 16, kLog2Group = 4, kHistBfs = 1 };
    template <bool WANT_LAST>
    __device__ __forceinline__ bool bfs_run(MaskT& n, MaskT pass, int& hist, MaskT& prev, int& it) const { return pcg_bfs_run<WANT_LAST, false>(n, pass, hist, prev, it); }
    __device__ __forceinline__ int hist_fold(int hist, int it, int last_it) const { return hist != 0 ? it - (int)__builtin_ctz((unsigned)hist) : last_it; }
    __device__ __forceinline__ mask_t rows_down(mask_t m, int k) const {
        switch (k) { case 0: return dpp_mov0<0x111>(m); case 1: return dpp_mov0<0x112>(m); case 2: return dpp_mov0<0x114>(m); default: return dpp_mov0<0x118>(m); }
    }
    __device__ __forceinline__ mask_t rows_up(mask_t m, int k) const {
        switch (k) { case 0: return dpp_mov0<0x101>(m); case 1: return dpp_mov0<0x102>(m); case 2: return dpp_mov0<0x104>(m); default: return dpp_mov0<0x108>(m); }
    }
    int lane;
    int shift;
    __device__ __forceinline__ DevGroup() {
        int l = (int)(threadIdx.x & 63);
        lane = l & 15;
        shift = l & 48;
    }
    __device__ __forceinline__ explicit DevGroup(int lane64) { lane = lane64 & 15; shift = lane64 & 48; }
    __device__ __forceinline__ mask_t up(mask_t m) const { return dpp_mov0<0x111>(m); }
    __device__ __forceinline__ mask_t down(mask_t m) const { return dpp_mov0<0x101>(m); }
    __device__ __forceinline__ uint32_t ballot(bool p) const {
        return (uint32_t)(__ballot(p) >> shift) & 0xFFFFu;
    }
    __device__ __forceinline__ bool any(mask_t m) const { return ballot(m != 0) != 0; }
    __device__ __forceinline__ mask_t rows_between(mask_t m, int lo, int hi) const { return (lane >= lo && lane < hi) ? m : (mask_t)0; }
    __device__ __forceinline__ int first_row(mask_t m) const { return __ffs((int)ballot(m != 0)) - 1; }
    __device__ __forceinline__ bool any_ne(mask_t a, mask_t b) const { return ballot(a != b) != 0; }
    __device__ __forceinline__ mask_t first_bit(mask_t m) const {
        uint32_t b = ballot(m != 0);
        int first = __ffs((int)b) - 1;
        return lane == first ? (m & (mask_t)(0 - m)) : (mask_t)0;
    }
    __device__ __forceinline__ int sum(int v) const {
        v += __builtin_amdgcn_update_dpp(0, v, 0xB1, 0xF, 0xF, true);
        v += __builtin_amdgcn_update_dpp(0, v, 0x4E, 0xF, 0xF, true);
        v += __builtin_amdgcn_update_dpp(0, v, 0x141, 0xF, 0xF, true);
        v += __builtin_amdgcn_update_dpp(0, v, 0x140, 0xF, 0xF, true);
        return v;
    }
    __device__ __forceinline__ int imax(int v) const {
        v = max(v, __builtin_amdgcn_update_dpp(0, v, 0xB1, 0xF, 0xF, true));
        v = max(v, __builtin_amdgcn_update_dpp(0, v, 0x4E, 0xF, 0xF, true));
        v = max(v, __builtin_amdgcn_update_dpp(0, v, 0x141, 0xF, 0xF, true));
        v = max(v, __builtin_amdgcn_update_dpp(0, v, 0x140, 0xF, 0xF, true));
        return v;
    }
    __device__ __forceinline__ int popcount_sum(mask_t m) const { return sum(pcg_popc(m)); }
    __device__ __forceinline__ void popcount_sum2(mask_t a, mask_t b, int& x, int& y) const {
        const int v = sum(pcg_popc(a) | (pcg_popc(b) << 16));
        x = v & 0xFFFF; y = (int)((unsigned)v >> 16);
    }
    __device__ __forceinline__ void popcount_sum3(mask_t a, mask_t b, mask_t c, int& x, int& y, int& z) const {
        if (sizeof(MaskT) == 4) {
            const int v = sum(pcg_popc(a) | (pcg_popc(b) << 10) | (pcg_popc(c) << 20));
            x = v & 1023; y = (v >> 10) & 1023; z = (int)((unsigned)v >> 20);
        } else { popcount_sum2(a, b, x, y); z = popcount_sum(c); }
    }
};

template <class MaskT>
struct DevGroup<64, MaskT> : DevLaneOps<MaskT> {
    typedef MaskT mask_t;
    enum { kGroup = 64, kLog2Group = 4, kHistBfs = 0 };
    template <bool WANT_LAST>
    __device__ __forceinline__ bool bfs_run(MaskT& n, MaskT pass, int& hist, MaskT& prev, int& it) const { return pcg_bfs_run<WANT_LAST, true>(n, pass, hist, prev, it); }
    __device__ __forceinline__ int hist_fold(int hist, int it, int last_it) const { return hist != 0 ? it - (int)__builtin_ctz((unsigned)hist) : last_it; }
    int lane;
    __device__ __forceinline__ DevGroup() { lane = (int)(threadIdx.x & 63); }
    __device__ __forceinline__ mask_t up(mask_t m) const { return dpp_mov0<0x138>(m); }
    __device__ __forceinline__ mask_t down(mask_t m) const { return dpp_mov0<0x130>(m); }
    __device__ __forceinline__ mask_t rows_down(mask_t m, int k) const {
        switch (k) { case 0: return dpp_mov0<0x111>(m); case 1: return dpp_mov0<0x112>(m); case 2: return dpp_mov0<0x114>(m); default: return dpp_mov0<0x118>(m); }
    }
    __device__ __forceinline__ mask_t rows_up(mask_t m, int k) const {
        switch (k) { case 0: return dpp_mov0<0x101>(m); case 1: return dpp_mov0<0x102>(m); case 2: return dpp_mov0<0x104>(m); default: return dpp_mov0<0x108>(m); }
    }
    __device__ __forceinline__ bool any(mask_t m) const { return __ballot(m != 0) != 0; }
    __device__ __forceinline__ mask_t rows_between(mask_t m, int lo, int hi) const { return (lane >= lo && lane < hi) ? m : (mask_t)0; }
    __device__ __forceinline__ int first_row(mask_t m) const { return __ffsll((unsigned long long)__ballot(m != 0)) - 1; }
    __device__ __forceinline__ bool any_ne(mask_t a, mask_t b) const { return __ballot(a != b) != 0; }
    __device__ __forceinline__ mask_t first_bit(mask_t m) const {
        uint64_t b = __ballot(m != 0);
        int first = __ffsll((unsigned long long)b) - 1;
        return lane == first ? (m & (mask_t)(0 - m)) : (mask_t)0;
    }
    __device__ __forceinline__ int sum(int v) const {
        v += __builtin_amdgcn_update_dpp(0, v, 0xB1, 0xF, 0xF, true);
        v += __builtin_amdgcn_update_dpp(0, v, 0x4E, 0xF, 0xF, true);
        v += __builtin_amdgcn_update_dpp(0, v, 0x141, 0xF, 0xF, true);
        v += __builtin_amdgcn_update_dpp(0, v, 0x140, 0xF, 0xF, true);
        return __builtin_amdgcn_readlane(v, 0) + __builtin_amdgcn_readlane(v, 16) + __builtin_amdgcn_readlane(v, 32) +
               __builtin_amdgcn_readlane(v, 48);
    }
    __device__ __forceinline__ int imax(int v) const {
        v = max(v, __builtin_amdgcn_update_dpp(0, v, 0xB1, 0xF, 0xF, true));
        v = max(v, __builtin_amdgcn_update_dpp(0, v, 0x4E, 0xF, 0xF, true));
        v = max(v, __builtin_amdgcn_update_dpp(0, v, 0x141, 0xF, 0xF, true));
        v = max(v, __builtin_amdgcn_update_dpp(0, v, 0x140, 0xF, 0xF, true));
        return max(max(__builtin_amdgcn_readlane(v, 0), __builtin_amdgcn_readlane(v, 16)),
                   max(__builtin_amdgcn_readlane(v, 32), __builtin_amdgcn_readlane(v, 48)));
    }
    __device__ __forceinline__ int popcount_sum(mask_t m) const { return sum(pcg_popc(m)); }
    __device__ __forceinline__ void popcount_sum2(mask_t a, mask_t b, int& x, int& y) const {
        const int v = sum(pcg_popc(a) | (pcg_popc(b) << 16));
        x = v & 0xFFFF; y = (int)((unsigned)v >> 16);
    }
    __device__ __forceinline__ void popcount_sum3(mask_t a, mask_t b, mask_t c, int& x, int& y, int& z) const { popcount_sum2(a, b, x, y); z = popcount_sum(c); }
};
```

### gym_pcgrl_amd/csrc/pcgrl_abi.hip

```cpp
#include <hip/hip_runtime.h>
#include <stdio.h>
#include <stdlib.h>
#include <string.h>

#include <type_traits>
#include <vector>

#include "../../include/pcgrl_hip.h"

#ifdef PCGRL_PART
#define PCGRL_IN_PART(k) (PCGRL_PART == (k))
#else
#define PCGRL_IN_PART(k) 1
#endif
#define PCGRL_LOCAL __attribute__((visibility("hidden")))
#define PART_CORE 0
#define PART_STATS 1
#define PART_UPDATE 2
#define PART_STEP_BINARY 3
#define PART_STEP_ZELDA 4
#define PART_SEARCH 5
#define PART_SMB 6
#define PART_STEP_SOLVER 7

#include "lanegroup_dev.h"
#include "mt19937.h"
#include "pcgrl_algos.h"
#include "path_trace.h"
#include "sokoban_solver.h"
#include "sokoban_fast.h"
#include "mdungeon_solver.h"
#include "mdungeon_fast.h"
#include "ddave_solver.h"
#include "ddave_fast.h"
#include "level_build_wave.h"

#include "worklist.h"
#include "kernels_update.h"
#include "kernels_obs.h"
#include "reset_env.h"
#include "kernels_stats.h"
#include "kernels_reset.h"
#include "bigmap.h"
#include "bigmap_team.h"
#include "kernels_big.h"
#include "kernels_step.h"
#include "search_game.h"
#include "kernels_sokoban.h"
#include "kernels_agents4.h"
#include "kernels_smb.h"
#include "kernels_step_solver.h"
#include "kernels_search_async.h"
#include "kernels_evaluate.h"
#include "kernels_changes.h"
#include "kernels_paths.h"
#include "kernels_tile_graph.h"
#include "kernels_moves.h"
#include "kernels_smb_play.h"
#include "search_big.h"
#include "kernels_search_big.h"
#if PCGRL_IN_PART(PART_CORE)
#include "kernels_misc.h"
#include "kernels_render.h"
#endif

#if PCGRL_IN_PART(PART_CORE)
PCGRL_LOCAL thread_local int g_last_hip = 0;
#else
extern PCGRL_LOCAL thread_local int g_last_hip;
#endif
#if PCGRL_IN_PART(PART_CORE)
#include "step_pool.h"
#endif
struct BigArenaDims { int nblocks, nodes_cap, tsize, stride; size_t heap_off, table_off, block_bytes; };
struct pcgrl_env {
    BigArenaDims big_dims;
    pcgrl_config cfg;
    PcgrlParams P;
    pcgrl_layout L;
    DevBufs B;
    int bound;
    int has_old;
    int was_reset;
    int parity;
    int device;
    int alloc_solver_power;
    int smb_replay;
    pcgrl_tuning tun;
    int no_wide, wide_waves, wide_grid, wide_pairs, fused_zelda, no_fused, step_epb, smb_heap, obs_at_end, no_inc;
    int profiling;
    int obs_incremental;
    const uint8_t* obs_synced;
    int obs_hold;
    RowBind row; int row_on, row_i64, row_live;
    AsyncCtl async;
    int async_on, async_dirty, async_split;
    int big_team_waves;
    std::vector<hipEvent_t> events;
    size_t ev_used;
    int prof_steps;
};
static int gen_flag(const pcgrl_env* h) { return (h->P.random_start || !h->has_old) ? 1 : 0; }
#define PCGRL_NPHASE 6
static int prof_mark(pcgrl_env* h, hipStream_t st) {
    if (!h->profiling) return PCGRL_OK;
    if (h->ev_used == h->events.size()) {
        hipEvent_t e;
        if (hipEventCreate(&e) != hipSuccess) return PCGRL_EHIP;
        h->events.push_back(e);
    }
    if (hipEventRecord(h->events[h->ev_used++], st) != hipSuccess) return PCGRL_EHIP;
    return PCGRL_OK;
}

#define HIPCHK(expr) do { hipError_t err_ = (expr); if (err_ != hipSuccess) { g_last_hip = (int)err_; return PCGRL_EHIP; } } while (0)

static size_t align_up(size_t v, size_t a) { return (v + a - 1) / a * a; }
static int tun_or(int v, int dflt) { return v < 0 ? dflt : v; }

struct DeviceGuard {
    int prev, dev;
    explicit DeviceGuard(int d) : prev(-1), dev(d) {
        if (hipGetDevice(&prev) != hipSuccess) prev = -1;
        if (prev != dev) (void)hipSetDevice(dev);
    }
    ~DeviceGuard() { if (prev >= 0 && prev != dev) (void)hipSetDevice(prev); }
};

static bool solver_prob(int prob) { return prob == PCGRL_SOKOBAN || prob == PCGRL_MDUNGEON || prob == PCGRL_DDAVE || prob == PCGRL_SMB; }
#define PCGRL_MAX_DIM 255
#define PCGRL_MAX_DIM_WIDE 4096
#define PCGRL_BIG_LDS_BUDGET ((size_t)150 * 1024)
#define PCGRL_MAX_LEVEL_CELLS 16384
#define PCGRL_MAX_SOLVER_POWER 1000000
static bool big_map(const pcgrl_config* c) { return c->prob != PCGRL_SMB && (c->width > 64 || c->height > 64); }
static bool big_search(const pcgrl_config* c) {
    return solver_prob(c->prob) && c->prob != PCGRL_SMB && ((c->width + 2) * (c->height + 2) > 256 || c->solver_power > 16383);
}
static int validate_config(const pcgrl_config* c) {
    if (!c) return PCGRL_EINVAL;
    if (c->prob < 0 || c->prob > 5 || c->rep < 0 || c->rep > 5) return PCGRL_EINVAL;
    if (c->num_envs < 1) return PCGRL_EINVAL;
    if (c->prob == PCGRL_SMB) {
        if (c->width < 1 || c->width > 250 || c->height < 3 || c->height > SMB_MAX_H) return PCGRL_EINVAL;
    } else {
        const int max_dim = c->rep == PCGRL_REP_WIDE ? PCGRL_MAX_DIM_WIDE : PCGRL_MAX_DIM;
        if (c->width < 1 || c->width > max_dim || c->height < 1 || c->height > max_dim) return PCGRL_EINVAL;
        if (big_map(c)) {
            const int kw = (c->width + 63) >> 6;
            if (big_wave_lds(c->width, c->height) > PCGRL_BIG_LDS_BUDGET || (long long)big_words(c->width, c->height) * kw >= 65536) return PCGRL_EINVAL;
        }
    }
    if (c->max_changes < 1 || c->max_iterations < 1) return PCGRL_EINVAL;
    if (c->auto_reset && c->max_changes > 65535) return PCGRL_EINVAL;
    if (solver_prob(c->prob)) {
        if (c->prob != PCGRL_SMB && (c->width + 2) * (c->height + 2) > PCGRL_MAX_LEVEL_CELLS) return PCGRL_EINVAL;
        if (c->solver_power < 1 || c->solver_power > (c->prob == PCGRL_SMB ? 16383 : PCGRL_MAX_SOLVER_POWER)) return PCGRL_EINVAL;
    }
    return PCGRL_OK;
}
static int ntiles_of(int prob) { return prob == PCGRL_BINARY ? 2 : (prob == PCGRL_SOKOBAN ? 5 : ((prob == PCGRL_DDAVE || prob == PCGRL_SMB) ? 7 : 8)); }

static void fill_params(const pcgrl_config* c, PcgrlParams* P) {
    memset(P, 0, sizeof(*P));
    P->prob = c->prob; P->rep = c->rep; P->num_envs = c->num_envs;
    P->width = c->width; P->height = c->height;
    P->prob_width = c->prob_width > 0 ? c->prob_width : c->width;
    P->prob_height = c->prob_height > 0 ? c->prob_height : c->height;
    P->ntiles = ntiles_of(c->prob);
    P->big = big_map(c) ? 1 : 0;
    P->big_search = big_search(c) ? 1 : 0;
    P->nplanes = (c->prob == PCGRL_SMB || P->big) ? 0 : (c->prob == PCGRL_BINARY ? 1 : 3);
    P->group = c->height <= 16 ? 16 : 64;
    P->mask_bytes = c->width <= 32 ? 4 : 8;
    P->max_changes = c->max_changes; P->max_iterations = c->max_iterations;
    P->random_start = c->random_start; P->random_tile = c->random_tile; P->warp = c->warp;
    P->random_probs = c->random_probs; P->auto_reset = c->auto_reset;
    P->target_path = c->target_path; P->max_enemies = c->max_enemies; P->target_enemy_dist = c->target_enemy_dist;
    P->max_crates = c->max_crates; P->target_solution = c->target_solution; P->solver_power = c->solver_power;
    P->max_potions = c->max_potions; P->max_treasures = c->max_treasures; P->target_col_enemies = c->target_col_enemies;
    P->max_diamonds = c->max_diamonds; P->min_spikes = c->min_spikes; P->target_jumps = c->target_jumps;
    P->min_empty = c->min_empty; P->min_enemies = c->min_enemies; P->min_jumps = c->min_jumps;
    for (int i = 0; i < PCGRL_MAX_REWARDS; i++) P->rewards[i] = c->rewards[i];
    pcgrl_build_cdf(c->tile_probs, P->ntiles, P->cdf);
}

static const size_t WL_CNT_BYTES = 2 * WL_NLIST * WL_NSHARD * WL_CSTRIDE * sizeof(int32_t);
static int wl_capacity(int num_envs, int list) {
    return list == WL_CHG ? num_envs : 2 * ((num_envs + WL_NSHARD - 1) / WL_NSHARD + 256);
}
static size_t wl_list_bytes(int num_envs, int list) { return align_up((size_t)WL_NSHARD * wl_capacity(num_envs, list) * 4, 256); }
#define SOK_BLOCKS 256
enum { SOK_RES_WORDS = 16, SOK_CNT_WORDS = 1, SOK_STOP_WORDS = 1 };
static int sok_table_size(int power) { int t = 1024; while (t < 2 * power) t <<= 1; return t; }
static bool sok_in_lds(const pcgrl_config* c) { return c->solver_power <= SOK_LDS_POWER || c->prob == PCGRL_SMB; }
static size_t sok_heap_bytes(int power) { return align_up((4 * (size_t)power + 4) * 4, 256); }
static size_t sok_pool_bytes(const pcgrl_config* c) {
    const size_t full = 4 * (size_t)c->solver_power + 4, small = (size_t)SS_SEARCH_WAVES * SS_SMALL_NODES;
    size_t nodes = full > small ? full : small;
    if (c->prob == PCGRL_SMB)
        nodes = (SMB_MAX_WAVES * smb_wave_arena_bytes(c->solver_power) + sizeof(SokNode) - 1) / sizeof(SokNode);
    return align_up(nodes * sizeof(SokNode), 256);
}
static int play_trace_words(const pcgrl_config* c) { return (int)(align_up(sok_pool_bytes(c) / sizeof(SokNode) * 4, 256) / 4); }
static_assert(SS_SMALL_NODES >= 4 * SS_SMALL_POPS + 4, "a small-tier search pushes up to four nodes per pop");
static size_t champ_bytes(const pcgrl_config* c) {
    if (c->prob == PCGRL_SMB) return (c->rep <= PCGRL_REP_TURTLE && c->num_envs < SMB_KEEP_PLAY) ? align_up((size_t)c->num_envs * c->width * 4, 256) : 0;
    if (c->prob != PCGRL_BINARY) return 0;
    if (big_map(c))
        return (c->rep <= PCGRL_REP_TURTLE && c->width <= 256 && c->height <= 256 && c->num_envs <= WL_INCBIG_ENV_MASK + 1)
                   ? align_up((size_t)c->num_envs * big_words(c->width, c->height) * 8, 256) : 0;
    if (c->height <= 16) return (c->width <= 32 && c->num_envs <= WL_INC_ENV_MASK) ? align_up((size_t)c->num_envs * 64, 256) : 0;
    return c->num_envs <= WL_INC64_ENV_MASK ? align_up((size_t)c->num_envs * 64 * (c->width > 32 ? 8 : 4), 256) : 0;
}
static BigArenaDims big_arena_of(const pcgrl_config* c) {
    BigArenaDims A;
    const int cells = (c->width + 2) * (c->height + 2), nwb = (cells + 63) / 64, inner = c->width * c->height;
    A.nodes_cap = 4 * c->solver_power + 4;
    A.tsize = sok_table_size(c->solver_power);
    while (align_up((size_t)A.nodes_cap * 8, 256) + (size_t)A.tsize * 4 < (size_t)2 * cells) A.tsize <<= 1;
    A.stride = c->prob == PCGRL_SOKOBAN ? sokb_stride(inner < SOKB_MAXC ? inner : SOKB_MAXC) : mdb_stride(nwb);
    A.heap_off = align_up((size_t)A.nodes_cap * A.stride, 256);
    A.table_off = A.heap_off + align_up((size_t)A.nodes_cap * 8, 256);
    A.block_bytes = A.table_off + align_up((size_t)A.tsize * 4, 256);
    const size_t budget = (size_t)6 << 30;
    size_t nb = budget / A.block_bytes;
    nb = nb > SOK_BLOCKS ? SOK_BLOCKS : (nb < 4 ? 4 : nb);
    if (nb > (size_t)c->num_envs) nb = (size_t)c->num_envs;
    A.nblocks = (int)nb;
    return A;
}
struct Region { size_t off, bytes; };
struct Bump { size_t off; Region take(size_t bytes) { const Region r = {off, bytes}; off += bytes; return r; } };
template <class T> static T* at(uint8_t* base, Region r) { return r.bytes ? reinterpret_cast<T*>(base + r.off) : nullptr; }
struct ScratchPlan {
    Region wl_cnt, status, wl_items[WL_NLIST];
    Region arena;
    Region sok_env, sok_sync;
    Region sok_heap, sok_table;
    Region champ, fifo, fifo_tag, wide_sync;
    size_t total;
    BigArenaDims big;
};
static ScratchPlan scratch_plan(const pcgrl_config* c) {
    ScratchPlan S = {};
    Bump b = {0};
    S.wl_cnt = b.take(WL_CNT_BYTES);
    S.status = b.take(256);
    for (int k = 0; k < WL_NLIST; k++) S.wl_items[k] = b.take(wl_list_bytes(c->num_envs, k));
    if (solver_prob(c->prob)) {
        const bool big = big_search(c);
        if (big) S.big = big_arena_of(c);
        S.arena = b.take(big ? (size_t)S.big.nblocks * S.big.block_bytes : SOK_BLOCKS * sok_pool_bytes(c));
        S.sok_env = b.take(align_up((size_t)c->num_envs * (SOK_RES_WORDS + SOK_CNT_WORDS + SOK_STOP_WORDS) * 4, 256));
        S.sok_sync = b.take(align_up(2 * (size_t)(SOK_SY_WORDS + SOK_HARD_CAP) * 4, 256));
        if (!big && !sok_in_lds(c)) {
            S.sok_heap = b.take(SOK_BLOCKS * sok_heap_bytes(c->solver_power));
            S.sok_table = b.take(SOK_BLOCKS * (size_t)sok_table_size(c->solver_power) * 4);
        }
    }
    S.champ = b.take(champ_bytes(c));
    const size_t n = (size_t)c->num_envs;
    S.fifo = b.take(c->rep == PCGRL_NARROW ? align_up(n * PCGRL_FIFO_N * 4, 256) : 0);
    S.fifo_tag = b.take(c->rep == PCGRL_NARROW ? align_up(n * 4, 256) : 0);
    S.wide_sync = b.take((c->prob == PCGRL_BINARY && c->height > 16 && !big_map(c)) ? align_up(n * 16, 256) : 0);
    S.total = b.off;
    return S;
}

PCGRL_LOCAL int search_device_setup(pcgrl_env* h);
PCGRL_LOCAL int smb_device_setup(pcgrl_env* h);
#if PCGRL_IN_PART(PART_CORE)
static int device_setup(pcgrl_env* h) {
    {
        uint32_t tab[PCGRL_MT_N];
        tab[0] = 19650218u;
        for (int i = 1; i < PCGRL_MT_N; i++) tab[i] = 1812433253u * (tab[i - 1] ^ (tab[i - 1] >> 30)) + (uint32_t)i;
        HIPCHK(hipMemcpyToSymbol(HIP_SYMBOL(g_mt_genrand), tab, sizeof(tab)));
    }
    if (h->cfg.prob == PCGRL_SMB) return smb_device_setup(h);
    if (solver_prob(h->cfg.prob) && !big_search(&h->cfg)) return search_device_setup(h);
    return PCGRL_OK;
}

static void resolve_tuning(pcgrl_env* h) {
    const pcgrl_tuning& T = h->tun;
    DevBufs& B = h->B;
    h->no_wide = tun_or(T.no_wide, 0) ? 1 : 0;
    h->wide_waves = tun_or(T.wide_waves, 8);
    h->wide_pairs = tun_or(T.wide_pairs, 1);
    h->wide_grid = tun_or(T.wide_grid, 2048);
    if (h->wide_grid < 1) h->wide_grid = 2048;
    h->fused_zelda = tun_or(T.fused_zelda, 1) ? 1 : 0;
    h->no_fused = tun_or(T.no_fused, 0) ? 1 : 0;
    h->obs_at_end = tun_or(T.obs_at_end, 0) ? 1 : 0;
    h->async_split = tun_or(T.async_split, h->cfg.prob == PCGRL_SOKOBAN ? 1 : 0) ? 1 : 0;
    const int n_ = h->cfg.num_envs;
    h->step_epb = T.step_epb > 0 ? T.step_epb : ((n_ >= 192 * 256 && n_ <= 256 * 256) ? 256 : (n_ >= 192 * 128 ? 128 : 64));
    if (h->step_epb != 128 && h->step_epb != 256) h->step_epb = 64;
    h->smb_heap = T.smb_lds_heap > 0 ? T.smb_lds_heap : SMB_LDS_HEAP;
    if (h->smb_heap < 256 || h->smb_heap > 4096) h->smb_heap = SMB_LDS_HEAP;
    const int f = tun_or(T.full_per_wave, 4), i = tun_or(T.inc_per_wave, 4);
    B.step_fpw = (f == 1 || f == 2) ? f : 4;
    B.step_prio = tun_or(T.step_prio, h->cfg.prob == PCGRL_BINARY ? (h->cfg.rep == PCGRL_NARROW ? (15 | (3 << 6)) : 15) : 0) & 0xFFF;
    B.step_ipw = (i == 1 || i == 2) ? i : 4;
    B.step_touch = tun_or(T.no_touch, 0) ? 0 : 1;
    B.touch_resume = tun_or(T.touch_resume, 1) ? 1 : 0;
    B.step_pair = tun_or(T.step_pair, 6);
    B.step_tight = B.step_touch ? tun_or(T.touch_tight, 1) : 0;
    h->no_inc = tun_or(T.no_inc, 0) != 0;
    B.zelda_inc = (h->cfg.prob == PCGRL_ZELDA && h->cfg.rep <= PCGRL_REP_TURTLE && h->cfg.height <= 16 && h->cfg.width <= 32 &&
                   h->cfg.num_envs <= WL_INC_ENV_MASK && !h->no_inc) ? 1 : 0;
    B.pair_min = tun_or(T.pair_min, 2048);
    B.big_team = tun_or(T.big_team, 1) ? 1 : 0;
    h->big_team_waves = tun_or(T.big_team, 1) >= 2 ? (tun_or(T.big_team, 1) > BIG_TEAM_MAX_WAVES ? BIG_TEAM_MAX_WAVES : tun_or(T.big_team, 1)) : 4;
    B.wide_few = tun_or(T.wide_few, WL_WIDE_FEW_REGIONS);
    B.wide_spin = T.wide_spin > 0 ? T.wide_spin : WIDE_SPIN_LIMIT;
    B.inline_reset = (!solver_prob(h->cfg.prob) && tun_or(T.inline_reset, 1) != 0) ? 1 : 0;
    if (big_search(&h->cfg)) {
        B.sok_fast_maxc = -1; B.md_only_agent = -1; B.sok_hard_cap = 0; B.sok_spawn_iters = SOK_SPAWN_ITERS;
    } else if (solver_prob(h->cfg.prob)) {
        B.sok_fast_maxc = tun_or(T.sok_generic, 0) ? -1 : SOKF_MAXC;
        B.md_only_agent = T.md_only_agent;
        B.sok_hard_cap = tun_or(T.sok_hard_cap, SOK_HARD_CAP);
        B.sok_spawn_iters = T.sok_spawn > 0 ? T.sok_spawn : SOK_SPAWN_ITERS;
        if (B.sok_hard_cap > SOK_HARD_CAP) B.sok_hard_cap = SOK_HARD_CAP;
    }
}
static int bind_buffers(pcgrl_env* h, const pcgrl_buffers* b, hipStream_t st) {
    const pcgrl_config& c = h->cfg;
    DevBufs& B = h->B;
    B.map = (uint8_t*)b->map; B.old_map = (uint8_t*)b->old_map; B.heat = (uint16_t*)b->heatmap; B.pos = (uint8_t*)b->pos;
    B.heat_end = B.heat + (size_t)c.num_envs * c.width * c.height;
    B.heat32 = c.auto_reset ? 0 : 1;
    B.ep_return = nullptr; B.ep_length = nullptr; B.last_return = nullptr; B.last_length = nullptr;
    B.planes = b->planes; B.counters = (int32_t*)b->counters; B.stats = (int32_t*)b->stats;
    B.start_stats = (int32_t*)b->start_stats; B.info = (int32_t*)b->info; B.reward = (double*)b->reward;
    B.done = (uint8_t*)b->done; B.tile_p = (double*)b->tile_p; B.rng_rep = (uint32_t*)b->rng_rep;
    B.rng_prob = (uint32_t*)b->rng_prob; B.rng_cur = (int32_t*)b->rng_cursor;
    B.obs = ObsSpec{nullptr, 0, 0, 0, 0, 0, 0, 0};
    B.local = nullptr; B.flat = nullptr;
    const ScratchPlan S = scratch_plan(&c);
    uint8_t* s = (uint8_t*)b->scratch;
    B.wl_cnt = at<int32_t>(s, S.wl_cnt); B.status = at<int32_t>(s, S.status);
    for (int k = 0; k < WL_NLIST; k++) { B.wl_cap[k] = wl_capacity(c.num_envs, k); B.wl_items[k] = at<int32_t>(s, S.wl_items[k]); }
    HIPCHK(hipMemsetAsync(B.wl_cnt, 0, S.wl_cnt.bytes + S.status.bytes, st));
    B.champ = h->no_inc ? nullptr : at<uint8_t>(s, S.champ);
    if (B.champ) HIPCHK(hipMemsetAsync(B.champ, c.prob == PCGRL_SMB ? 0xFF : 0, S.champ.bytes, st));
    B.fifo = at<uint32_t>(s, S.fifo); B.fifo_tag = at<int32_t>(s, S.fifo_tag);
    if (B.fifo_tag) HIPCHK(hipMemsetAsync(B.fifo_tag, 0xFF, S.fifo_tag.bytes, st));
    B.wide_sync = at<int32_t>(s, S.wide_sync); B.wide_epoch = 0;
    if (B.wide_sync) HIPCHK(hipMemsetAsync(B.wide_sync, 0, S.wide_sync.bytes, st));
    const bool big = big_search(&c);
    B.big_arena = big ? at<uint8_t>(s, S.arena) : nullptr;
    B.sok_pool = big ? nullptr : at<SokNode>(s, S.arena);
    B.sok_heap = at<uint32_t>(s, S.sok_heap); B.sok_table = at<uint32_t>(s, S.sok_table);
    if (solver_prob(c.prob)) {
        const int power = h->alloc_solver_power = c.solver_power;
        h->big_dims = S.big;
        B.sok_res = at<int32_t>(s, S.sok_env);
        B.sok_cnt = B.sok_res + (size_t)c.num_envs * SOK_RES_WORDS;
        B.sok_stop = B.sok_cnt + (size_t)c.num_envs * SOK_CNT_WORDS;
        B.sok_sync = at<int32_t>(s, S.sok_sync);
        HIPCHK(hipMemsetAsync(B.sok_res, 0, S.sok_env.bytes + S.sok_sync.bytes, st));
        B.sok_use_lds = !big && sok_in_lds(&c);
        B.sok_table_size = big ? S.big.tsize : sok_table_size(power);
        B.sok_pool_stride = big ? 0 : (int32_t)(sok_pool_bytes(&c) / sizeof(SokNode));
        B.sok_heap_stride = big ? 0 : (int32_t)(sok_heap_bytes(power) / 4);
    }
    return PCGRL_OK;
}

extern "C" {

int pcgrl_abi_version(void) { return PCGRL_ABI_VERSION; }
int pcgrl_last_hip_error(void) { return g_last_hip; }
const char* pcgrl_error_string(int code) {
    switch (code) {
        case PCGRL_OK: return "ok";
        case PCGRL_EINVAL: return "invalid argument or unsupported configuration";
        case PCGRL_EHIP: return "HIP runtime error";
        case PCGRL_ESTATE: return "call order violated (bind, seed and reset before step)";
        default: return "unknown error";
    }
}

int pcgrl_query_layout(const pcgrl_config* c, pcgrl_layout* L) {
    int rc = validate_config(c);
    if (rc) return rc;
    if (!L) return PCGRL_EINVAL;
    PcgrlParams P;
    fill_params(c, &P);
    const size_t n = (size_t)c->num_envs, cells = (size_t)c->width * c->height;
    memset(L, 0, sizeof(*L));
    L->group = P.group; L->mask_bytes = P.mask_bytes; L->nplanes = P.nplanes; L->nstats = num_stats(c->prob);
    L->map = n * cells; L->old_map = n * cells; L->heatmap = n * cells * (c->auto_reset ? 2 : 4); L->pos = n * 2;
    L->planes = n * P.nplanes * P.group * P.mask_bytes;
    L->counters = n * 8; L->stats = n * 32; L->start_stats = n * 32; L->info = n * 40;
    L->reward = n * 8; L->done = n; L->tile_p = n * 16;
    L->rng_rep = n * PCGRL_MT_N * 4; L->rng_prob = c->prob == PCGRL_BINARY ? n * PCGRL_MT_N * 4 : 0;
    L->rng_cursor = n * 8;
    L->scratch = scratch_plan(c).total;
    return PCGRL_OK;
}

int pcgrl_create(const pcgrl_config* c, pcgrl_env** out) {
    int rc = validate_config(c);
    if (rc) return rc;
    if (!out) return PCGRL_EINVAL;
    pcgrl_env* h = new pcgrl_env();
    h->bound = h->has_old = h->was_reset = h->parity = h->device = 0;
    h->smb_replay = 0;
    h->profiling = 0; h->ev_used = 0; h->prof_steps = 0; h->obs_hold = 0; h->obs_incremental = 0; h->obs_synced = nullptr;
    memset(&h->row, 0, sizeof(h->row)); h->row_on = h->row_i64 = h->row_live = 0;
    memset(&h->async, 0, sizeof(h->async)); h->async_on = h->async_dirty = 0;
    memset(&h->B, 0, sizeof(h->B));
    pcgrl_tuning_defaults(&h->tun);
    h->cfg = *c;
    fill_params(c, &h->P);
    pcgrl_query_layout(c, &h->L);
    *out = h;
    return PCGRL_OK;
}

void pcgrl_tuning_defaults(pcgrl_tuning* t) {
    if (!t) return;
    int32_t* f = reinterpret_cast<int32_t*>(t);
    for (size_t i = 0; i < sizeof(pcgrl_tuning) / sizeof(int32_t); i++) f[i] = -1;
}
int pcgrl_set_tuning(pcgrl_env* h, const pcgrl_tuning* t) {
    if (!h || !t) return PCGRL_EINVAL;
    if (h->bound) return PCGRL_ESTATE;
    h->tun = *t;
    return PCGRL_OK;
}

int pcgrl_destroy(pcgrl_env* h) {
    if (h) {
        for (hipEvent_t e : h->events) (void)hipEventDestroy(e);
    }
    delete h;
    return PCGRL_OK;
}

int pcgrl_bind(pcgrl_env* h, const pcgrl_buffers* b, void* stream) {
    if (!h || !b) return PCGRL_EINVAL;
    if (!b->map || !b->old_map || !b->heatmap || !b->pos || !b->planes || !b->counters || !b->stats ||
        !b->start_stats || !b->info || !b->reward || !b->done || !b->tile_p || !b->rng_rep || !b->rng_cursor || !b->scratch)
        return PCGRL_EINVAL;
    if (h->cfg.prob == PCGRL_BINARY && !b->rng_prob) return PCGRL_EINVAL;
    {
        hipPointerAttribute_t at;
        if (hipPointerGetAttributes(&at, b->map) == hipSuccess) h->device = at.device;
        else { (void)hipGetLastError(); HIPCHK(hipGetDevice(&h->device)); }
    }
    DeviceGuard guard(h->device);
    int rc = device_setup(h);
    if (rc) return rc;
    resolve_tuning(h);
    if ((rc = bind_buffers(h, b, (hipStream_t)stream))) return rc;
    h->bound = 1; h->has_old = 0; h->was_reset = 0; h->parity = 0;
    h->async_on = h->async_dirty = 0;
    return PCGRL_OK;
}

int pcgrl_configure(pcgrl_env* h, const pcgrl_config* c) {
    if (!h) return PCGRL_EINVAL;
    int rc = validate_config(c);
    if (rc) return rc;
    if (c->prob != h->cfg.prob || c->rep != h->cfg.rep || c->num_envs != h->cfg.num_envs ||
        c->width != h->cfg.width || c->height != h->cfg.height)
        return PCGRL_EINVAL;
    if (h->bound && solver_prob(c->prob) && c->solver_power > h->alloc_solver_power) return PCGRL_EINVAL;
    const bool was_big = h->bound && h->P.big_search;
    if (h->bound && big_search(c) && !was_big) return PCGRL_EINVAL;
    if (h->bound && c->prob == PCGRL_SMB && c->solver_power != h->cfg.solver_power) h->smb_replay = 1;
    h->cfg = *c;
    fill_params(c, &h->P);
    if (was_big) h->P.big_search = 1;
    return PCGRL_OK;
}

int pcgrl_set_tile_probs(pcgrl_env* h, void* stream) {
    if (!h || !h->bound) return PCGRL_ESTATE;
    DeviceGuard guard(h->device);
    const int n = h->cfg.num_envs;
    hipLaunchKernelGGL(k_bcast_tile_p, dim3((n + 255) / 256), dim3(256), 0, (hipStream_t)stream, h->B.tile_p, n,
                       h->cfg.tile_probs[0], h->cfg.tile_probs[1]);
    HIPCHK(hipGetLastError());
    return PCGRL_OK;
}

int pcgrl_seed(pcgrl_env* h, const uint32_t* keys, int32_t first, int32_t count, void* stream) {
    if (!h || !h->bound) return PCGRL_ESTATE;
    if (!keys || first < 0 || count < 1 || first + count > h->cfg.num_envs) return PCGRL_EINVAL;
    DeviceGuard guard(h->device);
    const size_t bytes = (size_t)count * PCGRL_MT_N * 4, off = (size_t)first * PCGRL_MT_N;
    HIPCHK(hipMemcpyAsync(h->B.rng_rep + off, keys, bytes, hipMemcpyHostToDevice, (hipStream_t)stream));
    if (h->B.fifo_tag) HIPCHK(hipMemsetAsync(h->B.fifo_tag + first, 0xFF, (size_t)count * 4, (hipStream_t)stream));
    if (h->B.rng_prob) HIPCHK(hipMemcpyAsync(h->B.rng_prob + off, keys, bytes, hipMemcpyHostToDevice, (hipStream_t)stream));
    hipLaunchKernelGGL(k_zero_cursors, dim3((count + 255) / 256), dim3(256), 0, (hipStream_t)stream, h->B.rng_cur, first, count);
    HIPCHK(hipGetLastError());
    HIPCHK(hipStreamSynchronize((hipStream_t)stream));
    return PCGRL_OK;
}

int pcgrl_seed_words(pcgrl_env* h, const uint32_t* words, int32_t first, int32_t count, void* stream) {
    if (!h || !h->bound) return PCGRL_ESTATE;
    if (!words || first < 0 || count < 1 || first + count > h->cfg.num_envs) return PCGRL_EINVAL;
    DeviceGuard guard(h->device);
    hipStream_t st = (hipStream_t)stream;
    HIPCHK(hipMemcpy2DAsync(h->B.rng_rep + (size_t)first * PCGRL_MT_N, PCGRL_MT_N * 4, words, 12, 12, (size_t)count, hipMemcpyHostToDevice, st));
    if (h->B.fifo_tag) HIPCHK(hipMemsetAsync(h->B.fifo_tag + first, 0xFF, (size_t)count * 4, st));
    hipLaunchKernelGGL(k_init_by_array, dim3((count + 63) / 64), dim3(64), 0, st, h->B.rng_rep, h->B.rng_prob, h->B.rng_cur, first, count);
    HIPCHK(hipGetLastError());
    HIPCHK(hipStreamSynchronize(st));
    return PCGRL_OK;
}

}
#endif

struct RolloutArgs { int steps; size_t action_stride; double* reward_out; uint8_t* done_out; int32_t* info_out; };
PCGRL_LOCAL int launch_stats(pcgrl_env* h, int list, int parity, int mode, int clr, int inline_reset, hipStream_t st);
PCGRL_LOCAL int launch_reset(pcgrl_env* h, int list, int park_list, int parity, int clr, hipStream_t st);
PCGRL_LOCAL int launch_planes_from_map(pcgrl_env* h, const uint8_t* maps, hipStream_t st);
PCGRL_LOCAL int launch_update(pcgrl_env* h, const int32_t* actions, int parity, hipStream_t st);
PCGRL_LOCAL int launch_step_binary(pcgrl_env* h, const int32_t* actions, int parity, hipStream_t st, const RolloutArgs& R);
PCGRL_LOCAL int launch_step_zelda(pcgrl_env* h, const int32_t* actions, int parity, hipStream_t st, const RolloutArgs& R);
PCGRL_LOCAL int launch_search(pcgrl_env* h, int32_t* sync, int list_a, int mode_a, int list_b, int mode_b, int parity, int rst_list, int clr, hipStream_t st);
PCGRL_LOCAL int launch_smb(pcgrl_env* h, int32_t* sync, int list_a, int mode_a, int list_b, int mode_b, int parity, int rst_list, int clr, hipStream_t st, int inline_reset);
PCGRL_LOCAL int launch_step_solver(pcgrl_env* h, const int32_t* actions, hipStream_t st, const RolloutArgs& R, int epb);
PCGRL_LOCAL int launch_get_stats(pcgrl_env* h, const uint8_t* maps, int count, int32_t* rows_out, int32_t* head, int32_t* jobs, hipStream_t st);
PCGRL_LOCAL int launch_get_stats_search(pcgrl_env* h, const uint8_t* maps, int32_t* rows_out, int32_t* head, const int32_t* jobs, SokNode* pools, int blocks, hipStream_t st);
PCGRL_LOCAL int launch_get_paths(pcgrl_env* h, const uint8_t* maps, int count, int max_len, int16_t* cells_out, int32_t* length_out, int32_t* rows_out, hipStream_t st);
PCGRL_LOCAL int launch_tile_graph(pcgrl_env* h, const pcgrl_tile_graph_desc& D, hipStream_t st);
struct ChangesArgs {
    const uint8_t* maps; int count; const int32_t* cells; int ncells; const int32_t* start_rows;
    int32_t* base_rows; int32_t* rows; double* reward; uint8_t* over;
    int chunk, nchunks, grid_cap;
};
PCGRL_LOCAL int launch_get_changes(pcgrl_env* h, const ChangesArgs& A, int32_t* head, int32_t* jobs, hipStream_t st);
static int changes_group(const PcgrlParams& P) { return (P.group == 16 && P.mask_bytes == 8) ? 64 : P.group; }
PCGRL_LOCAL int launch_get_changes_search(pcgrl_env* h, const ChangeJobs& src, int32_t* head, const int32_t* jobs, SokNode* pools, int blocks, hipStream_t st);
PCGRL_LOCAL int launch_get_moves(pcgrl_env* h, const uint8_t* maps, int32_t* rows_out, const SolOut& out, int32_t* head, const int32_t* jobs, SokNode* pools, uint32_t* traces, int blocks, hipStream_t st);
PCGRL_LOCAL int launch_smb_play(pcgrl_env* h, const uint8_t* maps, int count, int32_t* rows_out, const SolOut& out, int32_t* ticket, uint8_t* arenas, int slots, hipStream_t st);
PCGRL_LOCAL int launch_search_async(pcgrl_env* h, int32_t* tickets, int list_a, int mode_a, int list_b, int mode_b, int parity, int rst_list, int clr, int budget, int resume, int small, hipStream_t st);
template <auto KFN>
static int lds_cap(int device, size_t lds) {
    static size_t cap[64];
    if (lds <= 64 * 1024) return PCGRL_OK;
    const int d = device & 63;
    if (lds > cap[d]) {
        HIPCHK(hipFuncSetAttribute(reinterpret_cast<const void*>(KFN), hipFuncAttributeMaxDynamicSharedMemorySize, (int)lds));
        cap[d] = lds;
    }
    return PCGRL_OK;
}
template <class... Params, class... Args>
static int launch_fn(void (*kfn)(Params...), int grid, int block, size_t lds, hipStream_t st, const Args&... args) {
    hipLaunchKernelGGL(kfn, dim3(grid), dim3(block), lds, st, args...);
    HIPCHK(hipGetLastError());
    return PCGRL_OK;
}
template <auto KFN, class... Args>
static int launch(pcgrl_env* h, int grid, int block, size_t lds, hipStream_t st, const Args&... args) {
    { const int rc = lds_cap<KFN>(h->device, lds); if (rc) return rc; }
    return launch_fn(KFN, grid, block, lds, st, args...);
}
static int grid_for(int items, int per_block, int cap) {
    int g = (items + per_block - 1) / per_block;
    if (g < 1) g = 1;
    return g < cap ? g : cap;
}
template <int V> using Int = std::integral_constant<int, V>;
template <class T> struct Type { using type = T; };
template <class Tag> using type_of = typename Tag::type;
template <int... VS, class F>
static int with_value(int v, F&& f) {
    int rc = PCGRL_EINVAL;
    (void)(... || (v == VS ? (rc = f(Int<VS>{}), true) : false));
    return rc;
}
template <int... PROBS, class F> static int with_prob(int prob, F&& f) { return with_value<PROBS...>(prob, f); }
template <int... REPS, class F> static int with_rep(int rep, F&& f) { return with_value<REPS...>(rep, f); }
template <class F> static int with_mask(int mask_bytes, F&& f) { return mask_bytes == 4 ? f(Type<uint32_t>{}) : f(Type<uint64_t>{}); }
template <class F>
static int with_lanes(int group, int mask_bytes, F&& f) {
    if (group == 16) return with_mask(mask_bytes, [&](auto m) { return f(Int<16>{}, m); });
    return with_mask(mask_bytes, [&](auto m) { return f(Int<64>{}, m); });
}

#if PCGRL_IN_PART(PART_STATS)
template <int PROB>
static int launch_stats_p(pcgrl_env* h, int list, int parity, int mode, int clr, int inline_reset, hipStream_t st) {
    const PcgrlParams& P = h->P;
    const int gpb = PCGRL_BLOCK / P.group;
    const int grid = grid_for(P.num_envs, gpb, 8192);
    const size_t lds = inline_reset ? 4 * (size_t)reset_stage_bytes(P.width * P.height) : 0;
    const int gen = gen_flag(h);
    const int lone0 = !(mode == MODE_STEP && inline_reset) ? 0 : ((PROB == PCGRL_PROB_BINARY && P.group == 16 && P.rep <= PCGRL_REP_TURTLE) ? 1 : 2);
    if (PROB == PCGRL_PROB_BINARY && P.group == 64 && !h->no_wide) {
        const int nw = h->wide_waves;
        const size_t set1 = reset_stage_bytes(P.width * P.height);
        const size_t need1 = set1 + (size_t)8 * P.width * P.height + 8 * ((size_t)(P.width * P.height + 63) / 64 + 2);
        const size_t sets1 = (size_t)(nw == 8 ? 8 : 4) * set1;
        const size_t lds1 = inline_reset ? (sets1 > need1 ? sets1 : need1) : 0;
        int gridw = P.num_envs < h->wide_grid ? P.num_envs : h->wide_grid;
        if (gridw > 1) gridw &= ~1;
        h->B.wide_epoch = (h->B.wide_epoch % 0x3FFFFFFF) + 1;
        const int pair_few = (mode == MODE_STEP && list == WL_CHG && P.rep <= PCGRL_REP_TURTLE && h->wide_pairs) ? 1 : 0;
        const auto wide = [&](auto waves) {
            constexpr int NW = waves();
            return with_mask(P.mask_bytes, [&](auto m) {
                return launch<k_stats_wide<type_of<decltype(m)>, NW>>(h, gridw, NW * 64, lds1, st, P, h->B, list, parity, mode, clr, inline_reset, gen, pair_few);
            });
        };
        return nw == 8 ? wide(Int<8>{}) : wide(Int<4>{});
    }
    return with_lanes(P.group, P.mask_bytes, [&](auto g, auto m) {
        return launch<k_stats<PROB, g(), type_of<decltype(m)>>>(h, grid, PCGRL_BLOCK, lds, st, P, h->B, list, parity, mode, clr, inline_reset, gen, lone0);
    });
}
template <int PROB>
static int launch_big_p(pcgrl_env* h, int list, int parity, int mode, int clr, int inline_reset, int park_list, hipStream_t st) {
    const PcgrlParams& P = h->P;
    const size_t per_wave = big_wave_lds(P.width, P.height);
    int nw = (int)(PCGRL_BIG_LDS_BUDGET / per_wave);
    const int nw_max = (PROB == PCGRL_PROB_BINARY && h->B.big_team && mode == MODE_STEP) ? h->big_team_waves : 4;
    nw = nw > nw_max ? nw_max : nw;
    if (nw < 1) return PCGRL_EINVAL;
    const size_t lds = (size_t)nw * per_wave;
    return launch<k_big<PROB>>(h, grid_for(P.num_envs, nw, 2048), nw * 64, lds, st, P, h->B, list, parity, mode, clr, inline_reset, gen_flag(h), park_list);
}
static int launch_big(pcgrl_env* h, int list, int parity, int mode, int clr, int inline_reset, int park_list, hipStream_t st) {
    return with_prob<PCGRL_PROB_BINARY, PCGRL_PROB_ZELDA, PCGRL_PROB_MDUNGEON, PCGRL_PROB_DDAVE, PCGRL_PROB_SOKOBAN>(h->P.prob, [&](auto prob) {
        return launch_big_p<prob()>(h, list, parity, mode, clr, inline_reset, park_list, st);
    });
}
PCGRL_LOCAL int launch_stats(pcgrl_env* h, int list, int parity, int mode, int clr, int inline_reset, hipStream_t st) {
    if (solver_prob(h->P.prob)) inline_reset = 0;
    if (h->P.big) return launch_big(h, list, parity, mode, clr, inline_reset, -1, st);
    return with_prob<PCGRL_PROB_BINARY, PCGRL_PROB_ZELDA, PCGRL_PROB_MDUNGEON, PCGRL_PROB_DDAVE, PCGRL_PROB_SOKOBAN>(h->P.prob, [&](auto prob) {
        return launch_stats_p<prob()>(h, list, parity, mode, clr, inline_reset, st);
    });
}

#endif

#if PCGRL_IN_PART(PART_UPDATE)
PCGRL_LOCAL int launch_update(pcgrl_env* h, const int32_t* actions, int parity, hipStream_t st) {
    const PcgrlParams& P = h->P;
    const int nthreads = P.num_envs > h->B.async_nslots ? P.num_envs : h->B.async_nslots;
    const int grid = (nthreads + PCGRL_BLOCK - 1) / PCGRL_BLOCK;
    return with_mask(P.mask_bytes, [&](auto m) {
        using MaskT = type_of<decltype(m)>;
        return with_rep<PCGRL_REP_NARROW, PCGRL_REP_WIDE, PCGRL_REP_TURTLE, PCGRL_REP_NARROW_CAST, PCGRL_REP_NARROW_MULTI, PCGRL_REP_TURTLE_CAST>(P.rep, [&](auto rep) {
            if constexpr (rep() <= PCGRL_REP_TURTLE) return launch<k_update<rep(), MaskT>>(h, grid, PCGRL_BLOCK, 0, st, P, h->B, actions, parity);
            else return launch<k_update_block<rep(), MaskT>>(h, grid, PCGRL_BLOCK, 0, st, P, h->B, actions, parity);
        });
    });
}
struct MapGrid { int grid; size_t lds; };
static MapGrid map_grid(const PcgrlParams& P, int count) {
    const int per_block = (PCGRL_BLOCK / 64) * (64 / P.group);
    const long long blocks = ((long long)count + per_block - 1) / per_block;
    return {(int)(blocks < 8192 ? blocks : 8192), (size_t)per_block * reset_tile_bytes(P.width * P.height)};
}
PCGRL_LOCAL int launch_get_stats(pcgrl_env* h, const uint8_t* maps, int count, int32_t* rows_out, int32_t* head, int32_t* jobs, hipStream_t st) {
    const PcgrlParams& P = h->P;
    const MapGrid G = map_grid(P, count);
    return with_prob<PCGRL_PROB_BINARY, PCGRL_PROB_ZELDA, PCGRL_PROB_MDUNGEON, PCGRL_PROB_DDAVE, PCGRL_PROB_SOKOBAN>(P.prob, [&](auto prob) {
        constexpr int PROB = prob();
        return with_lanes(P.group, P.mask_bytes, [&](auto g, auto m) {
            return launch<k_get_stats<PROB, g(), type_of<decltype(m)>>>(h, G.grid, PCGRL_BLOCK, G.lds, st, P, maps, count, rows_out, h->B.status, head, jobs);
        });
    });
}
PCGRL_LOCAL int launch_get_paths(pcgrl_env* h, const uint8_t* maps, int count, int max_len, int16_t* cells_out, int32_t* length_out, int32_t* rows_out, hipStream_t st) {
    const PcgrlParams& P = h->P;
    const MapGrid G = map_grid(P, count);
    return with_prob<PCGRL_PROB_BINARY, PCGRL_PROB_ZELDA>(P.prob, [&](auto prob) {
        constexpr int PROB = prob();
        return with_lanes(P.group, P.mask_bytes, [&](auto g, auto m) {
            return launch<k_get_paths<PROB, g(), type_of<decltype(m)>>>(h, G.grid, PCGRL_BLOCK, G.lds, st, P, maps, count, max_len, cells_out, length_out, rows_out, h->B.status);
        });
    });
}
PCGRL_LOCAL int launch_tile_graph(pcgrl_env* h, const pcgrl_tile_graph_desc& D, hipStream_t st) {
    const PcgrlParams& P = h->P;
    const MapGrid G = map_grid(P, D.count);
    return with_lanes(P.group, P.mask_bytes, [&](auto g, auto m) {
        return launch<k_tile_graph<g(), type_of<decltype(m)>>>(h, G.grid, PCGRL_BLOCK, G.lds, st, P, D, h->B.status);
    });
}
PCGRL_LOCAL int launch_get_changes(pcgrl_env* h, const ChangesArgs& A, int32_t* head, int32_t* jobs, hipStream_t st) {
    const PcgrlParams& P = h->P;
    const int group = changes_group(P), per_block = (PCGRL_BLOCK / 64) * (64 / group);
    const long long blocks = ((long long)A.count * A.nchunks + per_block - 1) / per_block;
    const int grid = (int)(blocks < A.grid_cap ? blocks : A.grid_cap);
    const size_t lds = (size_t)per_block * changes_group_bytes(P.width * P.height, group, P.mask_bytes);
    return with_prob<PCGRL_PROB_BINARY, PCGRL_PROB_ZELDA, PCGRL_PROB_MDUNGEON, PCGRL_PROB_DDAVE, PCGRL_PROB_SOKOBAN>(P.prob, [&](auto prob) {
        constexpr int PROB = prob();
        return with_lanes(group, P.mask_bytes, [&](auto g, auto m) {
            if constexpr (g() == 16 && sizeof(type_of<decltype(m)>) == 8) return PCGRL_EINVAL;
            else return launch<k_get_changes<PROB, g(), type_of<decltype(m)>>>(h, grid, PCGRL_BLOCK, lds, st, P, A.maps, A.count, A.cells, A.ncells, A.chunk, A.nchunks,
                                                                          A.start_rows, A.base_rows, A.rows, A.reward, A.over, h->B.status, head, jobs);
        });
    });
}
#endif

static bool fused_step_applies(const pcgrl_env* h, bool rollout = false) {
    const PcgrlParams& P = h->P;
    const bool prob_ok = P.prob == PCGRL_PROB_BINARY || (P.prob == PCGRL_PROB_ZELDA && (rollout || h->fused_zelda));
    return prob_ok && P.group == 16 && !P.big && P.rep <= PCGRL_REP_TURTLE && P.auto_reset &&
           h->B.inline_reset && !h->no_fused;
}
#if PCGRL_IN_PART(PART_STEP_BINARY) || PCGRL_IN_PART(PART_STEP_ZELDA)
template <int PROB, class MaskT, int EPB>
static int launch_step_pme(pcgrl_env* h, const int32_t* actions, int parity, hipStream_t st, const RolloutArgs& R) {
    const PcgrlParams& P = h->P;
    const StepLds SL = step_lds_layout(16 * P.nplanes * (int)sizeof(MaskT), PROB == PCGRL_PROB_BINARY ? 16 * (int)sizeof(MaskT) : 0,
                                       P.rep == PCGRL_REP_NARROW, P.rep == PCGRL_REP_WIDE ? 3 : 1, EPB);
    const size_t lds = (size_t)SL.total + (EPB / 16) * (size_t)reset_stage_bytes(P.width * P.height);
    const int grid = (P.num_envs + EPB - 1) / EPB;
    const bool multi = R.steps > 1 || R.reward_out || R.done_out || R.info_out;
    constexpr std::bool_constant<sizeof(MaskT) == 4> obs_kernel{};
    const bool obs = obs_kernel() && !multi && h->B.obs.out && h->B.obs.fused && !h->obs_at_end;
    const bool row = h->row_live != 0;
    return with_rep<PCGRL_REP_NARROW, PCGRL_REP_WIDE, PCGRL_REP_TURTLE>(P.rep, [&](auto rep) {
        constexpr int REP = rep();
        const auto go = [&](auto multi_t, auto obs_t, auto row_t) {
            return launch<k_step<PROB, REP, MaskT, multi_t(), EPB, obs_t(), row_t()>>(h, grid, EPB * 4, lds, st, P, h->B, actions, parity, gen_flag(h), R.steps,
                                                                                    R.action_stride, R.reward_out, R.done_out, R.info_out);
        };
        constexpr std::true_type yes{};
        constexpr std::false_type no{};
        if (multi) return go(yes, no, no);
        if (obs && row) return go(no, obs_kernel, yes);
        if (obs) return go(no, obs_kernel, no);
        if (row) return go(no, no, yes);
        return go(no, no, no);
    });
}
template <int PROB>
static int launch_step_p(pcgrl_env* h, const int32_t* actions, int parity, hipStream_t st, const RolloutArgs& R) {
    return with_mask(h->P.mask_bytes, [&](auto m) {
        using MaskT = type_of<decltype(m)>;
        if (sizeof(MaskT) == 4 && h->step_epb == 128) return launch_step_pme<PROB, uint32_t, 128>(h, actions, parity, st, R);
        if (sizeof(MaskT) == 4 && h->step_epb == 256) return launch_step_pme<PROB, uint32_t, 256>(h, actions, parity, st, R);
        return launch_step_pme<PROB, MaskT, 64>(h, actions, parity, st, R);
    });
}
#endif
#if PCGRL_IN_PART(PART_STEP_BINARY)
PCGRL_LOCAL int launch_step_binary(pcgrl_env* h, const int32_t* actions, int parity, hipStream_t st, const RolloutArgs& R) {
    return launch_step_p<PCGRL_PROB_BINARY>(h, actions, parity, st, R);
}
#endif
#if PCGRL_IN_PART(PART_STEP_ZELDA)
PCGRL_LOCAL int launch_step_zelda(pcgrl_env* h, const int32_t* actions, int parity, hipStream_t st, const RolloutArgs& R) {
    return launch_step_p<PCGRL_PROB_ZELDA>(h, actions, parity, st, R);
}
#endif
static int launch_step(pcgrl_env* h, const int32_t* actions, int parity, hipStream_t st, const RolloutArgs& R = RolloutArgs{1, 0, nullptr, nullptr, nullptr}) {
    return h->P.prob == PCGRL_PROB_BINARY ? launch_step_binary(h, actions, parity, st, R) : launch_step_zelda(h, actions, parity, st, R);
}
static int action_width(int rep) {
    return rep == PCGRL_REP_WIDE ? 3 : (rep == PCGRL_REP_NARROW_CAST || rep == PCGRL_REP_TURTLE_CAST) ? 2 : rep == PCGRL_REP_NARROW_MULTI ? 9 : 1;
}

#define SMB_LDS_BUDGET (160 * 1024 - 2048)
static size_t smb_play_wave_bytes(int power) { return smb_wave_arena_bytes(power) + smb_play_log_bytes(power); }
#if PCGRL_IN_PART(PART_SMB)
PCGRL_LOCAL int smb_device_setup(pcgrl_env*) {
    HIPCHK(hipFuncSetAttribute(reinterpret_cast<const void*>(k_smb<0>), hipFuncAttributeMaxDynamicSharedMemorySize, SMB_LDS_BUDGET));
    HIPCHK(hipFuncSetAttribute(reinterpret_cast<const void*>(k_smb_play<0>), hipFuncAttributeMaxDynamicSharedMemorySize, SMB_LDS_BUDGET));
    return PCGRL_OK;
}
struct SmbSplit { int heap_n, nw; size_t per_wave; };
static bool smb_lds_split(const pcgrl_env* h, int floor_words, SmbSplit* S) {
    S->heap_n = 4 * h->P.solver_power + 4 < h->smb_heap ? ((4 * h->P.solver_power + 4 + 3) & ~3) : h->smb_heap;
    if (S->heap_n < floor_words) S->heap_n = (floor_words + 3) & ~3;
    const size_t vis_words = ((size_t)((h->P.width + 6) * (h->P.height + SMB_YOFF + 1) * 5 + 31) / 32 + 3) & ~(size_t)3;
    S->per_wave = ((size_t)S->heap_n + vis_words) * 4;
    const int nw = (int)(SMB_LDS_BUDGET / S->per_wave);
    S->nw = nw > SMB_MAX_WAVES ? SMB_MAX_WAVES : (nw < 1 ? 1 : nw);
    return (size_t)S->nw * S->per_wave <= SMB_LDS_BUDGET;
}
PCGRL_LOCAL int launch_smb(pcgrl_env* h, int32_t* sync, int list_a, int mode_a, int list_b, int mode_b, int parity, int rst_list, int clr, hipStream_t st, int inline_reset) {
    SmbSplit S;
    if (!smb_lds_split(h, reset_stage_bytes(h->P.width * h->P.height) / 4, &S)) return PCGRL_EINVAL;
    return launch_fn(k_smb<0>, SOK_BLOCKS, S.nw * 64, S.nw * S.per_wave, st, h->P, h->B, (list_a == WL_CHG && mode_a == MODE_STEP) ? (int)WL_INC : -1,
                     list_a, mode_a, list_b, mode_b, parity, rst_list, sync, clr, S.heap_n, inline_reset, gen_flag(h));
}
PCGRL_LOCAL int launch_smb_play(pcgrl_env* h, const uint8_t* maps, int count, int32_t* rows_out, const SolOut& out, int32_t* ticket, uint8_t* arenas, int slots, hipStream_t st) {
    SmbSplit S;
    if (!smb_lds_split(h, 0, &S)) return PCGRL_EINVAL;
    const int nw = S.nw > count ? count : S.nw;
    int blocks = (count + nw - 1) / nw;
    blocks = blocks > SOK_BLOCKS ? SOK_BLOCKS : blocks;
    if ((long long)blocks * nw > slots) return PCGRL_EINVAL;
    return launch_fn(k_smb_play<0>, blocks, nw * 64, nw * S.per_wave, st, h->P, maps, count, rows_out, out, h->B.status, ticket, arenas,
                     smb_play_wave_bytes(h->P.solver_power), nw, S.heap_n);
}
#endif
#if PCGRL_IN_PART(PART_SEARCH)
typedef void (*AsyncKernel)(PcgrlParams, DevBufs, AsyncCtl, int, int, int, int, int, int, int32_t*, int, int, int, int, int, int);
typedef void (*Agents4Kernel)(PcgrlParams, DevBufs, int, int, int, int, int, int, int32_t*, int);
static AsyncKernel async_kernel(int prob) {
    return prob == PCGRL_PROB_DDAVE ? k_search_async<PCGRL_PROB_DDAVE> : prob == PCGRL_PROB_MDUNGEON ? k_search_async<PCGRL_PROB_MDUNGEON> : k_search_async<PCGRL_PROB_SOKOBAN>;
}
static Agents4Kernel agents4_kernel(int prob) { return prob == PCGRL_PROB_DDAVE ? k_ddave<0> : k_mdungeon<0>; }
PCGRL_LOCAL int search_device_setup(pcgrl_env* h) {
    const int lds = (int)sok_lds_bytes();
    const int prob = h->cfg.prob;
    const void* f = prob == PCGRL_PROB_SOKOBAN ? reinterpret_cast<const void*>(k_sokoban<0>) : reinterpret_cast<const void*>(agents4_kernel(prob));
    HIPCHK(hipFuncSetAttribute(f, hipFuncAttributeMaxDynamicSharedMemorySize, lds));
    HIPCHK(hipFuncSetAttribute(reinterpret_cast<const void*>(async_kernel(prob)), hipFuncAttributeMaxDynamicSharedMemorySize, lds));
    return PCGRL_OK;
}
PCGRL_LOCAL int launch_search_async(pcgrl_env* h, int32_t* tickets, int list_a, int mode_a, int list_b, int mode_b, int parity, int rst_list, int clr, int budget, int resume, int small, hipStream_t st) {
    const int toff = small ? ASYNC_SMALL_HEAP : SOK_LDS_HEAP, tsize = small ? ASYNC_SMALL_TABLE : SOK_LDS_TABLE;
    const size_t lds = (size_t)(toff + 2 * tsize) * 4;
    const int grid = small ? ASYNC_SMALL_BLOCKS : SOK_BLOCKS;
    return launch_fn(async_kernel(h->P.prob), grid, 128, lds, st, h->P, h->B, h->async, list_a, mode_a, list_b, mode_b, parity, rst_list, tickets, clr, budget, resume, toff, tsize, small);
}
template <int PROB>
static int launch_search_big_p(pcgrl_env* h, int32_t* sync, int list_a, int mode_a, int list_b, int mode_b, int parity, int rst_list, int clr, hipStream_t st) {
    const BigArenaDims& D = h->big_dims;
    const BigSearchArena A = {h->B.big_arena, D.block_bytes, D.heap_off, D.table_off, D.nodes_cap, D.tsize};
    const int cells = (h->P.width + 2) * (h->P.height + 2);
    const size_t lds = (((size_t)cells * 4 + 15) & ~(size_t)15) + (size_t)(BIG_MAX_WORDS + SOKB_MAXC / 64) * 8;
    return launch<k_search_big<PROB>>(h, D.nblocks, 64, lds, st, h->P, h->B, A, list_a, mode_a, list_b, mode_b, parity, rst_list, sync, clr);
}
PCGRL_LOCAL int launch_search(pcgrl_env* h, int32_t* sync, int list_a, int mode_a, int list_b, int mode_b, int parity, int rst_list, int clr, hipStream_t st) {
    if (h->P.big_search)
        return with_prob<PCGRL_PROB_DDAVE, PCGRL_PROB_MDUNGEON, PCGRL_PROB_SOKOBAN>(h->P.prob, [&](auto prob) {
            return launch_search_big_p<prob()>(h, sync, list_a, mode_a, list_b, mode_b, parity, rst_list, clr, st);
        });
    const size_t lds = h->B.sok_use_lds ? sok_lds_bytes() : 0;
    if (h->P.prob != PCGRL_PROB_SOKOBAN)
        return launch_fn(agents4_kernel(h->P.prob), SOK_BLOCKS, 128, lds, st, h->P, h->B, list_a, mode_a, list_b, mode_b, parity, rst_list, sync, clr);
    return launch_fn(k_sokoban<0>, SOK_BLOCKS, 128, lds, st, h->P, h->B, list_a, mode_a, list_b, mode_b, parity, rst_list, sync, sync + SOK_SY_WORDS, clr);
}
int pcgrl_selftest_heap(const uint32_t* ops, int32_t n_ops, uint32_t* pops, uint32_t* heap_out, int32_t* n_out, void* stream) {
    if (!ops || !pops || !heap_out || !n_out || n_ops < 0) return PCGRL_EINVAL;
    const int cap = 16384;
    HIPCHK(hipFuncSetAttribute(reinterpret_cast<const void*>(k_selftest_heap<0>), hipFuncAttributeMaxDynamicSharedMemorySize, cap * 4));
    return launch_fn(k_selftest_heap<0>, 1, 64, (size_t)cap * 4, (hipStream_t)stream, ops, n_ops, cap, pops, heap_out, n_out);
}
#endif
static int launch_solver(pcgrl_env* h, int slot, int list_a, int mode_a, int list_b, int mode_b, int parity, int rst_list, int clr,
                         hipStream_t st, int inline_reset = 0) {
    int32_t* sync = h->B.sok_sync + (size_t)slot * (SOK_SY_WORDS + SOK_HARD_CAP);
    HIPCHK(hipMemsetAsync(sync, 0, (size_t)(SOK_SY_WORDS + SOK_HARD_CAP) * 4, st));
    if (h->P.prob == PCGRL_PROB_SMB) return launch_smb(h, sync, list_a, mode_a, list_b, mode_b, parity, rst_list, clr, st, inline_reset);
    return launch_search(h, sync, list_a, mode_a, list_b, mode_b, parity, rst_list, clr, st);
}

#if PCGRL_IN_PART(PART_STATS)
PCGRL_LOCAL int launch_reset(pcgrl_env* h, int list, int park_list, int parity, int clr, hipStream_t st) {
    if (h->P.big) return launch_big(h, list, parity, MODE_START, clr, 0, park_list, st);
    const PcgrlParams& P = h->P;
    const size_t lds = 4 * (size_t)reset_stage_bytes(P.width * P.height);
    const int grid = grid_for(P.num_envs, 4, h->was_reset ? 512 : 4096);
    const int gen = gen_flag(h);
    return with_prob<PCGRL_PROB_BINARY, PCGRL_PROB_ZELDA, PCGRL_PROB_MDUNGEON, PCGRL_PROB_DDAVE, PCGRL_PROB_SMB, PCGRL_PROB_SOKOBAN>(P.prob, [&](auto prob) {
        constexpr int PROB = prob();
        return with_lanes(P.group, P.mask_bytes, [&](auto g, auto m) {
            return launch<k_reset<PROB, g(), type_of<decltype(m)>>>(h, grid, PCGRL_BLOCK, lds, st, P, h->B, list, park_list, parity, gen, clr);
        });
    });
}

PCGRL_LOCAL int launch_planes_from_map(pcgrl_env* h, const uint8_t* maps, hipStream_t st) {
    const PcgrlParams& P = h->P;
    if (P.big) {
        const size_t total = (size_t)P.num_envs * P.width * P.height;
        const size_t g = (total + 255) / 256;
        return launch<k_copy_map<0>>(h, (int)(g < 16384 ? g : 16384), 256, 0, st, P, h->B, maps);
    }
    const size_t lds = 4 * (size_t)reset_tile_bytes(P.width * P.height);
    const int grid = grid_for(P.num_envs, 4, 4096);
    return with_mask(P.mask_bytes, [&](auto m) { return launch<k_planes_from_map<type_of<decltype(m)>>>(h, grid, PCGRL_BLOCK, lds, st, P, h->B, maps); });
}
#endif

static bool solver_rollout_applies(const pcgrl_env* h, int* envs_per_block) {
    const PcgrlParams& P = h->P;
    if (!solver_prob(P.prob) || P.prob == PCGRL_PROB_SMB || P.rep > PCGRL_REP_TURTLE || !P.auto_reset || !h->B.sok_use_lds || P.group != 16 || h->no_fused || P.big ||
        P.big_search) return false;
    int epb = 64 * ((P.num_envs + SOK_BLOCKS * 64 - 1) / (SOK_BLOCKS * 64));
    epb = epb < 64 ? 64 : epb;
    if (epb > WL_LOCAL_CAP) return false;
    *envs_per_block = epb;
    return true;
}
#if PCGRL_IN_PART(PART_STEP_SOLVER)
PCGRL_LOCAL int launch_step_solver(pcgrl_env* h, const int32_t* actions, hipStream_t st, const RolloutArgs& R, int epb) {
    const size_t lds = sok_lds_bytes();
    const int grid = (h->P.num_envs + epb - 1) / epb;
    return with_prob<PCGRL_PROB_SOKOBAN, PCGRL_PROB_MDUNGEON, PCGRL_PROB_DDAVE>(h->P.prob, [&](auto prob) {
        constexpr int PROB = prob();
        return with_mask(h->P.mask_bytes, [&](auto m) {
            using MaskT = type_of<decltype(m)>;
            return with_rep<PCGRL_REP_NARROW, PCGRL_REP_WIDE, PCGRL_REP_TURTLE>(h->P.rep, [&](auto rep) {
                return launch<k_step_solver<PROB, rep(), MaskT>>(h, grid, SS_THREADS, lds, st, h->P, h->B, actions, gen_flag(h), R.steps, R.action_stride, epb,
                                                                 R.reward_out, R.done_out, R.info_out);
            });
        });
    });
}

static DevBufs search_devbufs(const pcgrl_env* h) {
    DevBufs Bs;
    memset(&Bs, 0, sizeof(Bs));
    Bs.status = h->B.status; Bs.sok_use_lds = h->B.sok_use_lds; Bs.sok_fast_maxc = h->B.sok_fast_maxc;
    return Bs;
// ... 813 lines not shown
```

### gym_pcgrl_amd/csrc/pcgrl_algos.h

```cpp
#pragma once
#include "pcgrl_common.h"

#if defined(__HIPCC__) && defined(__HIP_DEVICE_COMPILE__)
#define PCGRL_NO_IFCVT() asm volatile("" ::: "memory")
#else
#define PCGRL_NO_IFCVT() do {} while (0)
#endif
#ifndef PCGRL_TRACE
#define PCGRL_TRACE(g, site)
#endif

struct PcgrlParams {
    int32_t prob, rep, num_envs, width, height, ntiles, nplanes, group, mask_bytes;
    int32_t max_changes, max_iterations;
    int32_t random_start, random_tile, warp, random_probs, auto_reset;
    int32_t target_path, max_enemies, target_enemy_dist, max_crates, target_solution, solver_power;
    int32_t prob_width, prob_height;
    int32_t max_potions, max_treasures;
    int32_t max_diamonds, min_spikes, target_jumps;
    int32_t min_empty, min_enemies, min_jumps;
    int32_t big, big_search;
    double target_col_enemies;
    double rewards[PCGRL_MAX_REWARDS];
    double cdf[PCGRL_MAX_TILES];
// ... 54 lines not shown
        r = r + (double)range_reward_i(n[2], o[2], 1, 1) * w[2];
        r = r + (double)range_reward_i(n[3], o[3], 2, P.max_enemies) * w[4];
        r = r + (double)range_reward_i(n[4], o[4], 1, 1) * w[3];
        r = r + (double)range_reward_i(n[5], o[5], P.target_enemy_dist, PCGRL_IPOS) * w[5];
        r = r + (double)range_reward_i(n[6], o[6], PCGRL_IPOS, PCGRL_IPOS) * w[6];
        return r;
    } else if (prob == PCGRL_PROB_DDAVE) {
        double r = (double)range_reward_i(dd_player(n), dd_player(o), 1, 1) * w[0];
        r = r + (double)range_reward_i(n[1], o[1], 0, 0) * w[1];
        r = r + (double)range_reward_i(dd_exit(n), dd_exit(o), 1, 1) * w[2];
        r = r + (double)range_reward_i(n[3], o[3], P.min_spikes, PCGRL_IPOS) * w[5];
        r = r + (double)range_reward_i(n[2], o[2], PCGRL_INEG, P.max_diamonds) * w[3];
        r = r + (double)range_reward_i(dd_key(n), dd_key(o), 1, 1) * w[4];
        r = r + (double)range_reward_i(n[4], o[4], 1, 1) * w[6];
        r = r + (double)range_reward_i(n[5], o[5], PCGRL_IPOS, PCGRL_IPOS) * w[7];
        r = r + (double)range_reward_i(md_dist_win(n), md_dist_win(o), PCGRL_INEG, PCGRL_INEG) * w[8];
        r = r + (double)range_reward_i(md_sol_length(n), md_sol_length(o), PCGRL_IPOS, PCGRL_IPOS) * w[9];
        return r;
    } else if (prob == PCGRL_PROB_SMB) {
        double r = (double)range_reward_i(n[0], o[0], 0, 0) * w[0];
        r = r + (double)range_reward_i(n[1], o[1], 0, 0) * w[1];
        r = r + (double)range_reward_i(n[2], o[2], P.min_enemies, P.max_enemies) * w[2];
        r = r + (double)range_reward_i(n[3], o[3], P.min_empty, PCGRL_IPOS) * w[3];
        r = r + (double)range_reward_i(n[4], o[4], 0, 0) * w[4];
        r = r + (double)range_reward_i(n[5], o[5], P.min_jumps, PCGRL_IPOS) * w[5];
        r = r + (double)range_reward_i(n[6], o[6], 0, 0) * w[6];
        r = r + (double)range_reward_i(n[7], o[7], 0, 0) * w[7];
        return r;
    } else if (prob == PCGRL_PROB_MDUNGEON) {
        double r = (double)range_reward_i(n[0], o[0], 1, 1) * w[0];
        r = r + (double)range_reward_i(n[1], o[1], 1, 1) * w[1];
        r = r + (double)range_reward_i(n[4], o[4], 1, P.max_enemies) * w[4];
        r = r + (double)range_reward_i(n[3], o[3], PCGRL_INEG, P.max_treasures) * w[3];
        r = r + (double)range_reward_i(n[2], o[2], PCGRL_INEG, P.max_potions) * w[2];
        r = r + (double)range_reward_i(n[5], o[5], 1, 1) * w[5];
        r = r + (double)range_reward_i(md_col_enemies(n), md_col_enemies(o), PCGRL_IPOS, PCGRL_IPOS) * w[6];
        r = r + (double)range_reward_i(md_dist_win(n), md_dist_win(o), PCGRL_INEG, PCGRL_INEG) * w[7];
        r = r + (double)range_reward_i(md_sol_length(n), md_sol_length(o), PCGRL_IPOS, PCGRL_IPOS) * w[8];
        return r;
    } else {
        int nr = n[1] - n[2], orr = o[1] - o[2];
        nr = nr < 0 ? -nr : nr; orr = orr < 0 ? -orr : orr;
        double r = (double)range_reward_i(n[0], o[0], 1, 1) * w[0];
        r = r + (double)range_reward_i(n[1], o[1], 1, P.max_crates) * w[1];
        r = r + (double)range_reward_i(n[2], o[2], 1, P.max_crates) * w[2];
        r = r + (double)range_reward_i(n[3], o[3], 1, 1) * w[3];
        r = r + (double)range_reward_i(nr, orr, PCGRL_INEG, PCGRL_INEG) * w[4];
        r = r + (double)range_reward_i(n[4], o[4], PCGRL_INEG, PCGRL_INEG) * w[5];
        r = r + (double)range_reward_i(n[5], o[5], PCGRL_IPOS, PCGRL_IPOS) * w[6];
        return r;
    }
}
PCGRL_HD double compute_reward(const PcgrlParams& P, const int32_t* n, const int32_t* o) { return compute_reward(P, n, o, P.prob); }
PCGRL_HD bool episode_over(const PcgrlParams& P, const int32_t* n, const int32_t* start, int prob) {
    if (prob == PCGRL_PROB_BINARY) return n[0] == 1 && n[1] - start[1] >= P.target_path;
    if (prob == PCGRL_PROB_ZELDA) return n[5] >= P.target_enemy_dist && n[6] >= P.target_path;
    if (prob == PCGRL_PROB_DDAVE) return md_sol_length(n) >= P.target_solution && n[5] > P.target_jumps;
    if (prob == PCGRL_PROB_SMB) return n[7] <= 0;
    if (prob == PCGRL_PROB_MDUNGEON) {
        const int en = n[4] > 1 ? n[4] : 1;
        return md_sol_length(n) >= P.target_solution && n[4] > 0 && (double)md_col_enemies(n) / (double)en > P.target_col_enemies;
    }
    return n[5] >= P.target_solution;
}
PCGRL_HD bool episode_over(const PcgrlParams& P, const int32_t* n, const int32_t* start) { return episode_over(P, n, start, P.prob); }
PCGRL_HD int num_stats(int prob) { return prob == PCGRL_PROB_BINARY ? 2 : (prob == PCGRL_PROB_ZELDA ? 7 : (prob == PCGRL_PROB_SOKOBAN ? 6 : 8)); }

template <class WordT>
PCGRL_HD void planes_set_cell(WordT& m0, WordT& m1, WordT& m2, int x, int t) {
    const WordT keep = ~((WordT)1 << x);
    m0 = (m0 & keep) | ((WordT)(t & 1) << x);
    m1 = (m1 & keep) | ((WordT)((t >> 1) & 1) << x);
    m2 = (m2 & keep) | ((WordT)((t >> 2) & 1) << x);
}

template <class B>
PCGRL_D typename B::mask_t pcg_expand(B& g, typename B::mask_t f) {
    return f | (f << 1) | (f >> 1) | g.up(f) | g.down(f);
}
template <class B>
PCGRL_D typename B::mask_t pcg_neighbours(B& g, typename B::mask_t f) {
    return (f << 1) | (f >> 1) | g.up(f) | g.down(f);
}

template <class B>
PCGRL_D typename B::mask_t pcg_fill_rows(B& g, typename B::mask_t s, typename B::mask_t p, typename B::mask_t rp) {
    typedef typename B::mask_t M;
    M hi = (((p + s) ^ p) & p) | s;
    M rs = g.bitrev(s);
    M lo = (((rp + rs) ^ rp) & rp) | rs;
    return hi | g.bitrev(lo);
}

template <class B>
struct PcgFillCtx {
    typename B::mask_t pass, rpass;
    typename B::mask_t dn[B::kLog2Group], up[B::kLog2Group];
};
template <class B>
PCGRL_D PcgFillCtx<B> pcg_fill_ctx(B& g, typename B::mask_t pass) {
    PcgFillCtx<B> c;
    c.pass = pass;
    c.rpass = g.bitrev(pass);
    c.dn[0] = pass; c.up[0] = pass;
#pragma unroll
    for (int k = 1; k < B::kLog2Group; k++) {
        c.dn[k] = c.dn[k - 1] & g.rows_down(c.dn[k - 1], k - 1);
        c.up[k] = c.up[k - 1] & g.rows_up(c.up[k - 1], k - 1);
    }
    return c;
}
template <class B>
PCGRL_D typename B::mask_t pcg_fill_cols(B& g, typename B::mask_t f, const PcgFillCtx<B>& c) {
    typename B::mask_t d = f, u = f;
#pragma unroll
    for (int k = 0; k < B::kLog2Group; k++) {
        d = d | (c.dn[k] & g.rows_down(d, k));
        u = u | (c.up[k] & g.rows_up(u, k));
    }
    typename B::mask_t r = d | u;
    if (B::kGroup > 16) r = r | (c.pass & (g.up(r) | g.down(r)));
    return r;
}

template <class B>
PCGRL_D typename B::mask_t pcg_component_fills(B& g, typename B::mask_t seed, const PcgFillCtx<B>& c) {
    typedef typename B::mask_t M;
    M f = pcg_fill_rows(g, seed, c.pass, c.rpass);
    for (;;) {
        M n = pcg_fill_cols(g, f, c);
        f = pcg_fill_rows(g, n, c.pass, c.rpass);
        if (!g.wave_any(pcg_neighbours(g, f) & c.pass & ~f)) break;
    }
    return f;
}

template <class B>
PCGRL_D typename B::mask_t pcg_component(B& g, typename B::mask_t seed, const PcgFillCtx<B>& c) {
    typedef typename B::mask_t M;
    PCGRL_TRACE(g, 1);
    if (B::kGroup != 16) {
        M f = seed;
        for (int i = 0; i < 4; i++) {
            M n = pcg_expand(g, f) & c.pass;
            n = pcg_expand(g, n) & c.pass;
            if (!g.wave_any(n ^ f)) return f;
            f = n;
        }
        seed = f;
    }
    return pcg_component_fills(g, seed, c);
}

template <class B>
PCGRL_D typename B::mask_t pcg_tiny_components(B& g, typename B::mask_t p, int& regions, int& path) {
    typedef typename B::mask_t M;
    const M a = (p << 1) & p, b = (p >> 1) & p, c = g.up(p) & p, d = g.down(p) & p;
    const M s0 = a ^ b, c0 = a & b, s1 = c ^ d, c1 = c & d;
    const M n0 = s0 ^ s1, k = s0 & s1;
    const M two_or_more = c0 | c1 | k;
    const M iso = p & ~(a | b | c | d);
    const M deg1 = n0 & ~two_or_more;
    const M deg2 = ~n0 & (c0 ^ c1 ^ k) & ~(c0 & c1);
    const M dom = deg1 & pcg_neighbours(g, deg1);
    const M e1 = deg1 << 1, e2 = deg1 >> 1, e3 = g.up(deg1), e4 = g.down(deg1);
    const M centre = deg2 & ((e1 & e2) | (e3 & e4) | ((e1 | e2) & (e3 | e4)));
    const M ends = deg1 & pcg_neighbours(g, centre);
    int n_iso, n_dom, n_tri;
    g.popcount_sum3(iso, dom, centre, n_iso, n_dom, n_tri);
    regions += n_iso + (n_dom >> 1) + n_tri;
    const int tiny_path = n_tri > 0 ? 2 : (n_dom > 0 ? 1 : 0);
    path = tiny_path > path ? tiny_path : path;
    return iso | dom | centre | ends;
}

template <bool WANT_LAST = true, class B>
PCGRL_D int bfs_levels(B& g, typename B::mask_t src, typename B::mask_t pass, typename B::mask_t& last) {
    typedef typename B::mask_t M;
    typedef typename B::ivec_t I;
    if constexpr (B::kHistBfs != 0) {
        M n = src, prev = src ^ src;
        I hist = g.izero(), last_it = g.izero();
        int it = 0;
        PCGRL_TRACE(g, 2);
        while (g.template bfs_run<WANT_LAST>(n, pass, hist, prev, it)) { last_it = g.hist_fold(hist, it, last_it); hist = g.izero(); }
        last_it = g.hist_fold(hist, it, last_it);
        const int ecc = g.imax(last_it);
        if (WANT_LAST) last = g.keep_where_eq(last_it, ecc, n & ~prev);
        return ecc;
    }
    M f = src, prev = src ^ src;
    I last_it = g.izero();
    int it = 0;
    constexpr int kLevels = B::kGroup == 16 ? 2 : 4;
    PCGRL_TRACE(g, 2);
    for (;;) {
        M n = f;
        bool more = false;
#if defined(__HIPCC__)
#pragma unroll
#endif
        for (int uu = 0; uu < kLevels; uu++) {
            ++it;
            const M nn = pcg_expand(g, n) & pass;
            last_it = g.isel_ne(nn, n, it, last_it);
            prev = g.msel_ne(nn, n, n, prev);
            if (uu == kLevels - 1) more = g.wave_any(nn ^ n);
            n = nn;
        }
        f = n;
        if (!more) break;
    }
    const int ecc = g.imax(last_it);
    last = g.keep_where_eq(last_it, ecc, f & ~prev);
    return ecc;
}

template <class B>
PCGRL_D int bfs_dist(B& g, typename B::mask_t src, typename B::mask_t dst, typename B::mask_t pass) {
    typedef typename B::mask_t M;
    M f = src;
    int t = 0;
    for (;;) {
        const M n1 = pcg_expand(g, f) & pass, fresh1 = n1 & ~f;
        const M n2 = pcg_expand(g, n1) & pass, fresh2 = n2 & ~n1;
        if (g.any((fresh1 | fresh2) & dst)) return g.any(fresh1 & dst) ? t + 1 : t + 2;
        if (!g.any(fresh2)) return -1;
        t += 2;
        f = n2;
    }
}

template <class B>
PCGRL_D int count_regions(B& g, typename B::mask_t pass) {
    typedef typename B::mask_t M;
    int regions = 0, dummy = 0;
    M rest = pass & ~pcg_tiny_components(g, pass, regions, dummy);
    if (!g.any(rest)) return regions;
    const PcgFillCtx<B> ctx = pcg_fill_ctx(g, pass);
    while (g.any(rest)) {
        M comp = pcg_component(g, g.first_bit(rest), ctx);
        rest = rest & ~comp;
        ++regions;
    }
    return regions;
}

template <class B>
PCGRL_D int pcg_double_sweep(B& g, typename B::mask_t comp, int best, int& bound) {
#ifdef PCGRL_EXP_NOSWEEP
    return bound = g.popcount_sum(comp) / 4 + 1;
#endif
    typename B::mask_t last, unused;
    const int e1 = bfs_levels(g, g.first_bit(comp), comp, last);
    if (2 * e1 <= best) { bound = 2 * e1; return 0; }
    return bound = bfs_levels<false>(g, g.first_bit(last), comp, unused);
}
template <class B>
PCGRL_D int pcg_double_sweep(B& g, typename B::mask_t comp, int best) {
#ifdef PCGRL_EXP_NOSWEEP
    return g.popcount_sum(comp) / 4 + 1;
#endif
    typename B::mask_t last, unused;
    const int e1 = bfs_levels(g, g.first_bit(comp), comp, last);
    if (2 * e1 <= best) return 0;
    return bfs_levels<false>(g, g.first_bit(last), comp, unused);
}

template <class B>
PCGRL_D void regions_and_longest_path(B& g, typename B::mask_t pass, int& regions, int& path, typename B::mask_t& champ, int& ub2, bool tight = true) {
    typedef typename B::mask_t M;
    regions = 0;
    path = 0;
    ub2 = -1;
    champ = pass ^ pass;
    const M nontiny = pass & ~pcg_tiny_components(g, pass, regions, path);
    if (!g.any(nontiny)) return;
    const PcgFillCtx<B> ctx = pcg_fill_ctx(g, pass);
    if (B::kGroup != 16) {
        typedef typename B::ivec_t I;
        M rest = nontiny;
        const I cnt = g.popc_lanes(rest);
        M seed = g.first_bit(g.keep_where_eq(cnt, g.imax(cnt), rest));
        while (g.any(rest)) {
            const M comp = pcg_component(g, seed, ctx);
            rest = rest & ~comp;
            ++regions;
            if (g.popcount_sum(comp) - 1 > path) { const int e = pcg_double_sweep(g, comp, path); if (e > path) { path = e; champ = comp; } }
            seed = g.first_bit(rest);
        }
        return;
    }
    M rest = nontiny, big1 = nontiny ^ nontiny, big2 = big1;
    int size1 = 0, size2 = 0, size3 = 0;
    while (g.any(rest)) {
        const M comp = pcg_component(g, g.first_bit(rest), ctx);
        rest = rest & ~comp;
        ++regions;
        const int size = g.popcount_sum(comp);
        if (size > size1) { size3 = size2; size2 = size1; big2 = big1; size1 = size; big1 = comp; }
        else if (size > size2) { size3 = size2; size2 = size; big2 = comp; }
        else if (size > size3) size3 = size;
    }
    const int tiny_path = path;
    int bd1 = size1 - 1, bd2 = size2 - 1, who = 0;
    if (size1 - 1 > path) { const int e = pcg_double_sweep(g, big1, path, bd1); if (e > path) { path = e; champ = big1; who = 1; } }
    {
        const int rest_b = size3 - 1 > tiny_path ? size3 - 1 : tiny_path;
        if (size2 - 1 > path) { const int e = pcg_double_sweep(g, big2, path, bd2); if (e > path) { path = e; champ = big2; who = 2; } }
        else if (tight && size2 - 1 > rest_b) pcg_double_sweep(g, big2, rest_b, bd2);
    }
    if (size3 - 1 > path) {
        rest = nontiny & ~big1 & ~big2;
        while (g.any(rest)) {
            const M comp = pcg_component(g, g.first_bit(rest), ctx);
            rest = rest & ~comp;
            if (g.popcount_sum(comp) - 1 > path) { const int e = pcg_double_sweep(g, comp, path); if (e > path) { path = e; champ = comp; who = 3; } }
        }
    }
    const int b1 = who == 1 ? 0 : bd1, b2 = who == 2 ? 0 : bd2, b3 = size3 - 1;
    ub2 = tiny_path;
    ub2 = b1 > ub2 ? b1 : ub2; ub2 = b2 > ub2 ? b2 : ub2; ub2 = b3 > ub2 ? b3 : ub2;
    ub2 = ub2 > path ? path : ub2;
}
template <class B>
PCGRL_D void regions_and_longest_path(B& g, typename B::mask_t pass, int& regions, int& path, typename B::mask_t& champ) {
    int ub2;
    regions_and_longest_path(g, pass, regions, path, champ, ub2);
}
template <class B>
PCGRL_D void regions_and_longest_path(B& g, typename B::mask_t pass, int& regions, int& path) {
    typename B::mask_t champ;
    regions_and_longest_path(g, pass, regions, path, champ);
}

template <class B>
PCGRL_D void binary_incremental(B& g, typename B::mask_t pass_new, typename B::mask_t cbit, bool added, int regions_old, int path_old,
                                typename B::mask_t champ_old, int ub2_old, int& regions, int& path, typename B::mask_t& champ, int& ub2) {
    typedef typename B::mask_t M;
    const M base = pass_new & ~cbit;
    M rest = pcg_neighbours(g, cbit) & base;
    path = path_old;
    champ = champ_old;
    constexpr bool kTrack = B::kGroup == 16;
    const bool track = kTrack && ub2_old >= 0;
    int k = 0, ub = track ? ub2_old : 0;
    M uni = cbit;
    if (g.any(rest)) {
        const PcgFillCtx<B> ctx = pcg_fill_ctx(g, base);
        while (g.any(rest)) {
            const M comp = pcg_component(g, g.first_bit(rest), ctx);
            rest = rest & ~comp;
            ++k;
            if (added) uni = uni | comp;
            else {
                int bd = g.popcount_sum(comp) - 1, e = 0;
                const int thr = track ? ub : path;
                if (bd > thr) e = pcg_double_sweep(g, comp, thr, bd);
                if (e > path) { if (kTrack) ub = path > ub ? path : ub; path = e; champ = comp; }
                else if (kTrack) ub = bd > ub ? bd : ub;
            }
        }
    }
    if (added) {
        regions = regions_old + 1 - k;
        int bd = g.popcount_sum(uni) - 1, e = 0;
        const int thr = track ? ub : path;
        if (bd > thr) e = pcg_double_sweep(g, uni, thr, bd);
        if (e > path) { if (kTrack) ub = path > ub ? path : ub; path = e; champ = uni; }
        else if (kTrack) ub = bd > ub ? bd : ub;
    } else {
        regions = regions_old + k - 1;
    }
    ub2 = track ? ub : -1;
}
template <class B>
PCGRL_D void binary_incremental(B& g, typename B::mask_t pass_new, typename B::mask_t cbit, bool added, int regions_old, int path_old,
                                typename B::mask_t champ_old, int& regions, int& path, typename B::mask_t& champ) {
    int ub2;
    binary_incremental(g, pass_new, cbit, added, regions_old, path_old, champ_old, -1, regions, path, champ, ub2);
}

template <class M>
struct TouchMemo {
    M comp1, comp2;
    int val1, bd1, val2, bd2, bd3, regions, k;
    bool valid;
};
template <class B>
PCGRL_D TouchMemo<typename B::mask_t> touch_memo_empty(B& g, typename B::mask_t any_mask) {
    TouchMemo<typename B::mask_t> m;
    m.comp1 = any_mask ^ any_mask; m.comp2 = m.comp1;
    m.val1 = 0; m.bd1 = -1; m.val2 = 0; m.bd2 = -1; m.bd3 = -1; m.regions = 0; m.k = 0; m.valid = false;
    return m;
}
template <class B>
PCGRL_D bool binary_touch(B& g, typename B::mask_t pass_new, typename B::mask_t cbit, bool added, int regions_old,
                          typename B::mask_t champ_old, int ub2_old, int& regions, int& path, typename B::mask_t& champ, int& ub2,
                          TouchMemo<typename B::mask_t>& memo) {
    typedef typename B::mask_t M;
    const M base = pass_new & ~cbit;
    const M dom = added ? (base & ~champ_old) : (champ_old & ~cbit);
    M rest = pcg_neighbours(g, cbit) & dom;
    int k = 0, size1 = 0, size2 = 0, size3 = 0;
    M uni = cbit ^ cbit, big1 = uni, big2 = uni;
    if (g.any(rest)) {
        const PcgFillCtx<B> ctx = pcg_fill_ctx(g, dom);
        while (g.any(rest)) {
            const M comp = pcg_component(g, g.first_bit(rest), ctx);
            rest = rest & ~comp;
            ++k;
            uni = uni | comp;
            const int size = g.popcount_sum(comp);
            if (size > size1) { size3 = size2; size2 = size1; big2 = big1; size1 = size; big1 = comp; }
            else if (size > size2) { size3 = size2; size2 = size; big2 = comp; }
            else if (size > size3) size3 = size;
        }
    }
    const M target = added ? (champ_old | cbit | uni) : big1;
    int bd1 = 0;
    int e = pcg_double_sweep(g, target, added ? ub2_old - 1 : -1, bd1);
    bool ok = true;
    int ub = ub2_old;
    champ = target;
    memo.comp1 = target; memo.val1 = e; memo.bd1 = bd1;
    memo.comp2 = uni ^ uni; memo.val2 = 0; memo.bd2 = -1; memo.bd3 = -1; memo.k = k; memo.valid = true;
    if (added) {
        regions = regions_old - k;
    } else {
        regions = regions_old + k - 1;
        ok = k > 0;
        if (size2 > 0) {
            int bd = size2 - 1, e2 = 0;
            const int thr = e < ub ? e : ub;
            if (bd > thr) e2 = pcg_double_sweep(g, big2, thr, bd);
            memo.comp2 = big2; memo.val2 = e2; memo.bd2 = bd;
            if (e2 > e) { ub = e > ub ? e : ub; e = e2; champ = big2; }
            else ub = bd > ub ? bd : ub;
        }
        if (size3 > 0) {
            memo.bd3 = size3 - 1;
            if (size3 - 1 > e) ok = false;
            else ub = size3 - 1 > ub ? size3 - 1 : ub;
        }
        if (k == 0) { memo.comp1 = uni ^ uni; memo.val1 = 0; memo.bd1 = -1; }
    }
    memo.regions = regions;
    path = e;
    ub2 = ub;
    return ok && e >= ub2_old;
}
template <class B>
PCGRL_D bool binary_touch(B& g, typename B::mask_t pass_new, typename B::mask_t cbit, bool added, int regions_old,
                          typename B::mask_t champ_old, int ub2_old, int& regions, int& path, typename B::mask_t& champ, int& ub2) {
    TouchMemo<typename B::mask_t> memo;
    return binary_touch(g, pass_new, cbit, added, regions_old, champ_old, ub2_old, regions, path, champ, ub2, memo);
}

template <class B>
PCGRL_D void rlp_resume(B& g, typename B::mask_t pass, const TouchMemo<typename B::mask_t>& memo, int& regions, int& path,
                        typename B::mask_t& champ, int& ub2, bool tight = true) {
    typedef typename B::mask_t M;
    typedef typename B::ivec_t I;
    regions = 0;
    path = 0;
    champ = pass ^ pass;
    const M nontiny = pass & ~pcg_tiny_components(g, pass, regions, path);
    const bool known = memo.valid;
    int ub = path;
    if (known && memo.val1 > 0) {
        if (memo.val1 > path) { path = memo.val1; champ = memo.comp1; }
    }
    if (known && memo.val2 > 0) {
        if (memo.val2 > path) { ub = path > ub ? path : ub; path = memo.val2; champ = memo.comp2; }
        else ub = memo.val2 > ub ? memo.val2 : ub;
    } else if (known && memo.bd2 > ub) ub = memo.bd2;
    const bool pend1 = known && memo.val1 <= 0 && g.any(memo.comp1);
    M rest = nontiny & ~memo.comp1 & ~memo.comp2;
    M big1 = pend1 ? memo.comp1 : (pass ^ pass), big2 = pass ^ pass;
    int size1 = 0, size2 = 0, size3 = 0;
    const int count = known ? 0 : 1;
    if (known) regions = memo.regions;
    if (pend1) { size1 = g.popcount_sum(memo.comp1); size1 = memo.bd1 + 1 < size1 ? memo.bd1 + 1 : size1; }
    if (g.any(rest)) {
        const PcgFillCtx<B> ctx = pcg_fill_ctx(g, pass);
        while (g.any(rest)) {
            if (count == 0) {
                const int n = g.popcount_sum(rest);
                if (n - 1 <= path) { ub = n - 1 > ub ? n - 1 : ub; break; }
            }
            const I cnt = g.popc_lanes(rest);
            const M comp = pcg_component(g, g.first_bit(g.keep_where_eq(cnt, g.imax(cnt), rest)), ctx);
            rest = rest & ~comp;
            regions += count;
            const int size = g.popcount_sum(comp);
            if (size > size1) { size3 = size2; size2 = size1; big2 = big1; size1 = size; big1 = comp; }
            else if (size > size2) { size3 = size2; size2 = size; big2 = comp; }
            else if (size > size3) size3 = size;
        }
    }
    int b1 = size1 - 1, b2 = size2 - 1;
    if (b1 > path) {
        const int e = pcg_double_sweep(g, big1, path, b1);
        if (e > path) { ub = path > ub ? path : ub; path = e; champ = big1; b1 = -1; }
    }
    {
        int rest_b = size3 - 1 > ub ? size3 - 1 : ub;
        rest_b = b1 > rest_b ? b1 : rest_b;
        if (b2 > path) {
            const int e = pcg_double_sweep(g, big2, path, b2);
            if (e > path) { ub = path > ub ? path : ub; path = e; champ = big2; b2 = -1; }
        } else if (tight && b2 > rest_b) pcg_double_sweep(g, big2, rest_b, b2);
    }
    if (size3 - 1 > path) {
        rest = nontiny & ~champ & ~big1 & ~big2;
        const PcgFillCtx<B> ctx = pcg_fill_ctx(g, pass);
        while (g.any(rest)) {
            const M comp = pcg_component(g, g.first_bit(rest), ctx);
            rest = rest & ~comp;
            if (g.popcount_sum(comp) - 1 > path) {
                const int e = pcg_double_sweep(g, comp, path);
                if (e > path) { ub = path > ub ? path : ub; path = e; champ = comp; }
            }
        }
    }
    ub = b1 > ub ? b1 : ub; ub = b2 > ub ? b2 : ub; ub = size3 - 1 > ub ? size3 - 1 : ub;
    ub2 = ub > path ? path : ub;
}

template <class B>
PCGRL_D typename B::mask_t rlp_choose_seed(B& g, typename B::mask_t rest, int row_lo, int row_hi) {
    const typename B::mask_t mine = g.rows_between(rest, row_lo, row_hi);
    return g.first_bit(g.any(mine) ? mine : rest);
}
#if defined(PCGRL_TIMELINE) && defined(__HIPCC__)
__device__ __forceinline__ void tl_mark(int tag);
#define PCGRL_TLA(tag) tl_mark(tag)
#else
#define PCGRL_TLA(tag) do {} while (0)
#endif
#if defined(__HIPCC__) && defined(__HIP_DEVICE_COMPILE__) && !defined(PCGRL_EXP_NO_SWEEP_PRIO)
#define PCGRL_SWEEP_PRIO(p) __builtin_amdgcn_s_setprio(p)
#else
#define PCGRL_SWEEP_PRIO(p) do {} while (0)
#endif
template <class B, class Shared>
PCGRL_D void rlp_process_seed(B& g, typename B::mask_t seed, const PcgFillCtx<B>& ctx, Shared& sh, int& regions, int& my_best,
                              typename B::mask_t& my_champ) {
    typedef typename B::mask_t M;
    const M comp = pcg_component(g, seed, ctx);
    PCGRL_TLA(30);
    if (!sh.retire(g, comp)) return;
    ++regions;
    const int best = sh.best();
    if (g.popcount_sum(comp) - 1 > best) {
        PCGRL_TLA(31);
        PCGRL_SWEEP_PRIO(3);
        const int e = pcg_double_sweep(g, comp, best);
        PCGRL_SWEEP_PRIO(0);
        if (e > my_best) { my_best = e; my_champ = comp; }
        sh.raise(e);
        PCGRL_TLA(32);
    }
}
template <class B, class Shared>
PCGRL_D void rlp_process_seed(B& g, typename B::mask_t seed, const PcgFillCtx<B>& ctx, Shared& sh, int& regions) {
    int my_best = 0;
    typename B::mask_t my_champ = seed ^ seed;
    rlp_process_seed(g, seed, ctx, sh, regions, my_best, my_champ);
}
template <class B>
PCGRL_D typename B::mask_t rlp_prepare(B& g, typename B::mask_t pass, int& tiny_regions, int& tiny_path) {
    tiny_regions = 0; tiny_path = 0;
    return pass & ~pcg_tiny_components(g, pass, tiny_regions, tiny_path);
}

template <class M>
struct ZeldaMasks {
    M empty, solid, player, key, door, enemy;
};
template <class M>
PCGRL_D ZeldaMasks<M> zelda_masks(M b0, M b1, M b2, M valid) {
    ZeldaMasks<M> z;
    z.empty = ~b2 & ~b1 & ~b0 & valid;
    z.solid = ~b2 & ~b1 & b0 & valid;
    z.player = ~b2 & b1 & ~b0 & valid;
    z.key = ~b2 & b1 & b0 & valid;
    z.door = b2 & ~b1 & ~b0 & valid;
    z.enemy = b2 & (b1 | b0) & valid;
    return z;
}

template <class B>
PCGRL_D int regions_incremental(B& g, typename B::mask_t pass_new, typename B::mask_t cbit, bool added, int regions_old) {
    typedef typename B::mask_t M;
    const M base = pass_new & ~cbit;
    M rest = pcg_neighbours(g, cbit) & base;
    int k = 0;
    if (g.any(rest)) {
        const PcgFillCtx<B> ctx = pcg_fill_ctx(g, base);
        while (g.any(rest)) {
            rest = rest & ~pcg_component(g, g.first_bit(rest), ctx);
            ++k;
        }
    }
    return added ? regions_old + 1 - k : regions_old - 1 + k;
}

template <class B>
PCGRL_D void zelda_stats(B& g, const PcgrlParams& P, typename B::mask_t b0, typename B::mask_t b1,
                         typename B::mask_t b2, typename B::mask_t valid, int32_t* out,
                         int pass_change = -1, typename B::mask_t cbit = typename B::mask_t(), int regions_old = 0) {
    typedef typename B::mask_t M;
    ZeldaMasks<M> z = zelda_masks(b0, b1, b2, valid);
    int player, key, door;
    g.popcount_sum3(z.player, z.key, z.door, player, key, door);
    int enemies = g.popcount_sum(z.enemy);
    M walk = z.empty | z.player | z.key | z.enemy;
    int regions;
#ifdef PCGRL_EXP_NOREGIONS
    regions = regions_old + g.popcount_sum(cbit);
#else
    if (pass_change < 0) regions = count_regions(g, walk);
    else if (pass_change == 0) regions = regions_old;
    else regions = regions_incremental(g, walk, cbit, pass_change == 1, regions_old);
#endif
    int nearest = 0, path = 0;
    if (player == 1 && regions == 1) {
        if (enemies > 0) {
            int d = bfs_dist(g, z.player, z.enemy, z.empty | z.player | z.enemy);
            nearest = d > 0 ? d : P.prob_width * P.prob_height;
        }
        if (key == 1 && door == 1) {
            path = bfs_dist(g, z.player, z.key, walk);
            path += bfs_dist(g, z.key, z.door, walk | z.door);
        }
    }
    out[0] = player; out[1] = key; out[2] = door; out[3] = enemies; out[4] = regions; out[5] = nearest; out[6] = path;
}

template <class B>
PCGRL_D bool sokoban_stats(B& g, const PcgrlParams& P, typename B::mask_t b0, typename B::mask_t b1,
                           typename B::mask_t b2, typename B::mask_t valid, int32_t* out) {
    typedef typename B::mask_t M;
    M solid = ~b2 & ~b1 & b0 & valid;
    M player = ~b2 & b1 & ~b0 & valid;
    M crate = ~b2 & b1 & b0 & valid;
    M target = b2 & ~b1 & ~b0 & valid;
    int np_ = g.popcount_sum(player), nc = g.popcount_sum(crate), nt = g.popcount_sum(target);
    int regions = count_regions(g, valid & ~solid);
    out[0] = np_; out[1] = nc; out[2] = nt; out[3] = regions;
// ... 67 lines not shown
```

### include/pcgrl_hip.h

```cpp
#ifndef PCGRL_HIP_H
#define PCGRL_HIP_H
#include <stddef.h>
#include <stdint.h>

#ifdef __cplusplus
extern "C" {
#endif

#define PCGRL_ABI_VERSION 15
#define PCGRL_OK 0
#define PCGRL_EINVAL (-1)
#define PCGRL_EHIP (-2)
#define PCGRL_ESTATE (-3)

enum { PCGRL_BINARY = 0, PCGRL_ZELDA = 1, PCGRL_SOKOBAN = 2, PCGRL_MDUNGEON = 3, PCGRL_DDAVE = 4, PCGRL_SMB = 5 };
enum { PCGRL_NARROW = 0, PCGRL_WIDE = 1, PCGRL_TURTLE = 2, PCGRL_NARROW_CAST = 3, PCGRL_NARROW_MULTI = 4, PCGRL_TURTLE_CAST = 5 };

typedef struct pcgrl_config {
    int32_t prob, rep;
    int32_t num_envs;
    int32_t width, height;
    int32_t prob_width, prob_height;
    int32_t max_changes, max_iterations;
    int32_t random_start, random_tile, warp, random_probs;
    int32_t auto_reset;
    int32_t target_path;
    int32_t max_enemies, target_enemy_dist;
    int32_t max_crates, target_solution, solver_power;
    int32_t max_potions, max_treasures;
    int32_t max_diamonds, min_spikes, target_jumps;
    int32_t min_empty, min_enemies, min_jumps;
    double target_col_enemies;
    double tile_probs[8];
    double rewards[12];
} pcgrl_config;

typedef struct pcgrl_layout {
    int32_t group;
    int32_t mask_bytes;
    int32_t nplanes;
    int32_t nstats;
    size_t map;
    size_t old_map;
    size_t heatmap;
    size_t pos;
    size_t planes;
    size_t counters;
    size_t stats;
    size_t start_stats;
    size_t info;
    size_t reward;
    size_t done;
    size_t tile_p;
    size_t rng_rep;
    size_t rng_prob;
    size_t rng_cursor;
    size_t scratch;
} pcgrl_layout;

typedef struct pcgrl_buffers {
    void *map, *old_map, *heatmap, *pos, *planes, *counters, *stats, *start_stats, *info, *reward,
         *done, *tile_p, *rng_rep, *rng_prob, *rng_cursor, *scratch;
} pcgrl_buffers;

typedef struct pcgrl_env pcgrl_env;

typedef struct pcgrl_tuning {
    int32_t no_fused;
    int32_t fused_zelda;
    int32_t step_epb;
    int32_t no_inc;
    int32_t inline_reset;
    int32_t pair_min;
    int32_t no_wide;
    int32_t wide_waves;
    int32_t wide_grid;
    int32_t wide_pairs;
    int32_t wide_few;
    int32_t sok_generic;
    int32_t sok_hard_cap;
    int32_t sok_spawn;
    int32_t md_only_agent;
    int32_t smb_lds_heap;
    int32_t full_per_wave;
    int32_t inc_per_wave;
    int32_t wide_spin;
    int32_t step_prio;
    int32_t no_touch;
    int32_t touch_tight;
    int32_t step_pair;
    int32_t async_split;
    int32_t big_team;
    int32_t obs_at_end;
    int32_t touch_resume;
    int32_t changes_grid;
    int32_t changes_chunk;
} pcgrl_tuning;

int pcgrl_abi_version(void);
const char* pcgrl_error_string(int code);
int pcgrl_last_hip_error(void);

int pcgrl_query_layout(const pcgrl_config* cfg, pcgrl_layout* out);
int pcgrl_create(const pcgrl_config* cfg, pcgrl_env** out);
int pcgrl_destroy(pcgrl_env* env);
void pcgrl_tuning_defaults(pcgrl_tuning* t);
int pcgrl_set_tuning(pcgrl_env* env, const pcgrl_tuning* t);
int pcgrl_bind(pcgrl_env* env, const pcgrl_buffers* bufs, void* stream);
int pcgrl_configure(pcgrl_env* env, const pcgrl_config* cfg);
int pcgrl_seed(pcgrl_env* env, const uint32_t* keys, int32_t first, int32_t count, void* stream);
int pcgrl_seed_words(pcgrl_env* env, const uint32_t* words, int32_t first, int32_t count, void* stream);
int pcgrl_set_tile_probs(pcgrl_env* env, void* stream);
int pcgrl_reset(pcgrl_env* env, void* stream);
int pcgrl_step(pcgrl_env* env, const int32_t* actions, void* stream);
int pcgrl_step_multi(pcgrl_env* const* envs, const int32_t* const* actions, void* const* streams, int32_t count);
int32_t pcgrl_step_threads(int32_t n);
int pcgrl_rollout(pcgrl_env* env, const int32_t* actions, int32_t steps, double* reward_out, uint8_t* done_out,
                  int32_t* info_out, void* stream);
int pcgrl_set_maps(pcgrl_env* env, const uint8_t* maps, void* stream);
int pcgrl_observe(pcgrl_env* env, uint8_t* out, int32_t out_h, int32_t out_w, int32_t centered, int32_t pad_value,
                  int32_t onehot, void* stream);
int pcgrl_bind_observation(pcgrl_env* env, uint8_t* out, int32_t out_h, int32_t out_w, int32_t centered,
                           int32_t pad_value, int32_t onehot, int32_t incremental);
typedef struct pcgrl_row {
    int64_t* actions_out;
    double*  reward;
    uint8_t* done;
    const uint8_t* start_in;
    uint8_t* start_out;
    double*  ep_return;
    int32_t* ep_length;
    uint8_t* took;
    uint8_t* fresh;
    int32_t  actions_i64;
} pcgrl_row;
int pcgrl_bind_row(pcgrl_env* env, const pcgrl_row* row);
typedef struct pcgrl_render_desc {
    const int32_t* indices;
    int32_t count;
    const uint8_t* tiles;
    int32_t tile_size;
    int32_t border_x, border_y, border_tile, cursor;
    int32_t grid_rows, grid_cols;
    uint8_t* out;
} pcgrl_render_desc;
int pcgrl_render(pcgrl_env* env, const pcgrl_render_desc* d, void* stream);
size_t pcgrl_get_stats_bytes(const pcgrl_config* cfg, int32_t count);
int    pcgrl_get_stats(pcgrl_env* env, const uint8_t* maps, int32_t count, int32_t* rows_out,
                       void* work, size_t work_bytes, void* stream);
int    pcgrl_get_reward(pcgrl_env* env, const int32_t* rows, const int32_t* ref_rows, int32_t count,
                        double* reward_out, uint8_t* over_out, void* stream);
size_t pcgrl_get_solution_bytes(const pcgrl_config* cfg, int32_t count, int32_t max_len);
int    pcgrl_get_solution(pcgrl_env* env, const uint8_t* maps, int32_t count, int32_t max_len,
                          int8_t* moves_out, int32_t* length_out, int8_t* agent_out, int32_t* rows_out,
                          void* work, size_t work_bytes, void* stream);
size_t pcgrl_get_playthrough_bytes(const pcgrl_config* cfg, int32_t count, int32_t max_len);
int    pcgrl_get_playthrough(pcgrl_env* env, const uint8_t* maps, int32_t count, int32_t max_len,
                             int8_t* moves_out, int32_t* length_out, int8_t* agent_out, int32_t* rows_out,
                             void* work, size_t work_bytes, void* stream);
size_t pcgrl_get_smb_play_bytes(const pcgrl_config* cfg, int32_t count, int32_t max_len);
int    pcgrl_get_smb_play(pcgrl_env* env, const uint8_t* maps, int32_t count, int32_t max_len,
                          int8_t* moves_out, int32_t* length_out, int8_t* agent_out, int32_t* rows_out,
                          void* work, size_t work_bytes, void* stream);
int32_t pcgrl_get_paths_legs(const pcgrl_config* cfg);
size_t pcgrl_get_paths_bytes(const pcgrl_config* cfg, int32_t count, int32_t max_len);
int    pcgrl_get_paths(pcgrl_env* env, const uint8_t* maps, int32_t count, int32_t max_len,
                       int16_t* cells_out, int32_t* length_out, int32_t* rows_out,
                       void* work, size_t work_bytes, void* stream);
size_t pcgrl_get_changes_bytes(const pcgrl_config* cfg, int32_t count, int32_t ncells);
int    pcgrl_get_changes(pcgrl_env* env, const uint8_t* maps, int32_t count,
                         const int32_t* cells, int32_t ncells, const int32_t* start_rows,
                         int32_t* base_rows_out, int32_t* rows_out, double* reward_out, uint8_t* over_out,
                         void* work, size_t work_bytes, void* stream);
typedef struct pcgrl_tile_graph_desc {
    const uint8_t* maps;
    int32_t count;
    uint32_t passable, source_tiles, reach_tiles;
    const int32_t* sources;
    int32_t *regions_out, *longest_out;
    int16_t *labels_out, *dist_out;
    int32_t *reach_out, *source_out;
} pcgrl_tile_graph_desc;
size_t pcgrl_tile_graph_bytes(const pcgrl_config* cfg, int32_t count);
int    pcgrl_tile_graph(pcgrl_env* env, const pcgrl_tile_graph_desc* desc, void* work, size_t work_bytes, void* stream);
int pcgrl_action_map(pcgrl_env* env, const int32_t* flat, int32_t* xyv, void* stream);
int pcgrl_step_flat(pcgrl_env* env, const int32_t* flat, int32_t* xyv, void* stream);
size_t pcgrl_async_bytes(const pcgrl_config* cfg, int32_t nslots);
int pcgrl_bind_async(pcgrl_env* env, void* arena, size_t bytes, int32_t nslots, void* stream);
int pcgrl_step_async(pcgrl_env* env, const int32_t* actions, int32_t pop_budget, void* stream);
int pcgrl_async_flush(pcgrl_env* env, void* stream);
int pcgrl_bind_episode_stats(pcgrl_env* env, double* ep_return, int32_t* ep_length, double* last_return,
                             int32_t* last_length, void* stream);
int pcgrl_selftest_heap(const uint32_t* ops, int32_t n_ops, uint32_t* pops, uint32_t* heap_out, int32_t* n_out, void* stream);
int pcgrl_selftest_step_pool(int32_t count, int32_t calls, int32_t fail_at, int32_t* hits);
int pcgrl_selftest_range_reward(const int32_t* rows, int32_t n, int32_t* out, void* stream);
int pcgrl_status(pcgrl_env* env, void* stream, int32_t* status);
int pcgrl_clear_status(pcgrl_env* env, void* stream);


#define PCGRL_NPHASE 6
int pcgrl_profile(pcgrl_env* env, int enable);
int pcgrl_profile_read(pcgrl_env* env, double* phase_ms , int32_t* steps);

#ifdef __cplusplus
}
#endif
#endif
```

Before: 2.409 billion env-steps/s.

## Pack two component flood fills into one 32-bit row mask for binary stats

For binary maps at most 15 wide with 32-bit row masks, the passable mask is duplicated into the upper 16 bits so that one flood fill grows two seeds at once, one from the first and one from the last (or farthest) remaining cell. If the two fills meet they are the same region and the second is discarded. This is meant to roughly halve the serial connected-component iterations in the region and longest-path stats, and it applies both to the full computation and to the resume path. It adds a separate compiled kernel variant and a tuning switch that is on by default, and it costs wasted work whenever the two seeds land in the same component.

```diff
diff --git a/gym_pcgrl_amd/_lib.py b/gym_pcgrl_amd/_lib.py
--- a/gym_pcgrl_amd/_lib.py
+++ b/gym_pcgrl_amd/_lib.py
@@ -29,7 +29,7 @@
 
 
 TUNING_FIELDS = ("no_fused", "fused_zelda", "step_epb", "no_inc", "inline_reset", "pair_min", "no_wide", "wide_waves", "wide_grid",
-                 "wide_pairs", "wide_few", "sok_generic", "sok_hard_cap", "sok_spawn", "md_only_agent", "smb_lds_heap", "full_per_wave", "inc_per_wave", "wide_spin", "step_prio", "no_touch", "touch_tight", "step_pair", "async_split", "big_team", "obs_at_end", "touch_resume",
+                 "wide_pairs", "wide_few", "sok_generic", "sok_hard_cap", "sok_spawn", "md_only_agent", "smb_lds_heap", "full_per_wave", "inc_per_wave", "wide_spin", "step_prio", "no_touch", "touch_tight", "step_pair", "async_split", "big_team", "obs_at_end", "touch_resume", "pack2",
                  "changes_grid", "changes_chunk")
 
 
@@ -111,7 +111,7 @@
     return h.hexdigest()[:16]
 
 
-NPARTS = 8
+NPARTS = 9
 
 
 def build(force=False, verbose=False, jobs=None):
diff --git a/gym_pcgrl_amd/csrc/kernels_stats.h b/gym_pcgrl_amd/csrc/kernels_stats.h
--- a/gym_pcgrl_amd/csrc/kernels_stats.h
+++ b/gym_pcgrl_amd/csrc/kernels_stats.h
@@ -38,15 +38,15 @@
     return false;
 }
 
-template <int PROB, class G, class MaskT>
+template <int PROB, bool PACK = false, class G, class MaskT>
 __device__ __forceinline__ bool compute_item_stats(G& g, const PcgrlParams& P, MaskT b0, MaskT b1, MaskT b2, MaskT valid, int32_t* s,
-                                                   int32_t* status, MaskT& champ, bool tight = true) {
+                                                   int32_t* status, MaskT& champ, bool tight = true, bool pack = false) {
     champ = 0;
     if (PROB == PCGRL_PROB_BINARY) {
         int regions, path;
         if (G::kGroup == 16) {
             int ub2;
-            regions_and_longest_path(g, (MaskT)(~b0 & valid), regions, path, champ, ub2, tight);
+            regions_and_longest_path<PACK>(g, (MaskT)(~b0 & valid), regions, path, champ, ub2, tight, pack);
             s[3] = ub2 + 1;
         } else {
             regions_and_longest_path(g, (MaskT)(~b0 & valid), regions, path, champ);
@@ -109,7 +109,7 @@
     return r;
 }
 
-template <int PROB, int G, class MaskT, bool FUSED = false>
+template <int PROB, int G, class MaskT, bool FUSED = false, bool PACK = false>
 __device__ __forceinline__ void stats_wave_task(const PcgrlParams& P, const DevBufs& B, DevGroup<G, MaskT>& g, int lane64, int gw, bool lone,
                                                 bool inc, bool pair, bool zinc, bool have, int raw, int shard, int mode, int parity,
                                                 int inline_reset, int gen_map, uint32_t* mt, uint8_t* tiles, MaskT rowmask,
@@ -120,6 +120,8 @@
     constexpr bool kInc = PROB == PCGRL_PROB_BINARY;
     constexpr bool kZinc = PROB == PCGRL_PROB_ZELDA && G == 16 && sizeof(MaskT) == 4;
     constexpr int NPL = (PROB == PCGRL_PROB_BINARY) ? 1 : 3;
+    static_assert(!PACK || (FUSED && PROB == PCGRL_PROB_BINARY && G == 16 && sizeof(MaskT) == 4), "the packed extraction: k_step, binary, 32-bit row masks");
+    constexpr bool kPack = PACK, pack = PACK;
     MaskT* champ_base = reinterpret_cast<MaskT*>(B.champ);
     const bool tch = kInc && G == 16 && !inc && !lone && have && raw < 0;
     const bool packed = inc || (kZinc && zinc && !lone) || tch;
@@ -156,7 +158,7 @@
         int32_t sl[PCGRL_MAX_STATS] = {0, 0, 0, 0, 0, 0, 0, 0};
         MaskT champ_l = 0;
         bool ns = false;
-        if (act) ns = compute_item_stats<PROB>(g, P, b0, b1, b2, rowmask, sl, B.status, champ_l, (B.step_tight & 2) != 0);
+        if (act) ns = compute_item_stats<PROB, kPack>(g, P, b0, b1, b2, rowmask, sl, B.status, champ_l, (B.step_tight & 2) != 0, pack);
         TL(10);
         constexpr bool kLaneReward = PROB == PCGRL_PROB_ZELDA && G == 16;
         double rpre = 0.0;
@@ -220,13 +222,13 @@
             if (kResume && B.touch_resume) {
                 if (full) {
                     int regions, path, ub2;
-                    rlp_resume(g, (MaskT)(~b0 & rowmask), memo, regions, path, champ, ub2, (B.step_tight & 1) != 0);
+                    rlp_resume<kPack>(g, (MaskT)(~b0 & rowmask), memo, regions, path, champ, ub2, (B.step_tight & 1) != 0, pack);
                     s[0] = regions; s[1] = path; s[2] = g.any(champ) ? 1 : 0; s[3] = ub2 + 1;
                 }
                 full = false;
             }
         }
-        if (full) need_solver = compute_item_stats<PROB>(g, P, b0, b1, b2, rowmask, s, B.status, champ, (B.step_tight & 1) != 0);
+        if (full) need_solver = compute_item_stats<PROB, kPack>(g, P, b0, b1, b2, rowmask, s, B.status, champ, (B.step_tight & 1) != 0, pack);
     }
     if (kInc && compute && champ_base) champ_base[(size_t)e * G + g.lane] = champ;
     TL(10);
@@ -272,7 +274,7 @@
             }
             if (mine) {
                 int32_t st[PCGRL_MAX_STATS] = {0, 0, 0, 0, 0, 0, 0, 0};
-                const bool ns = compute_item_stats<PROB>(g, P, b0, b1, b2, rowmask, st, B.status, champ, (B.step_tight & 2) != 0);
+                const bool ns = compute_item_stats<PROB, kPack>(g, P, b0, b1, b2, rowmask, st, B.status, champ, (B.step_tight & 2) != 0, pack);
                 if (kInc && champ_base) champ_base[(size_t)e * G + g.lane] = champ;
                 if (g.lane == 0) finish_or_park<PROB>(P, B, e, st, ns, MODE_START, parity, shard);
             }
diff --git a/gym_pcgrl_amd/csrc/kernels_step.h b/gym_pcgrl_amd/csrc/kernels_step.h
--- a/gym_pcgrl_amd/csrc/kernels_step.h
+++ b/gym_pcgrl_amd/csrc/kernels_step.h
@@ -78,7 +78,7 @@
     else __builtin_amdgcn_s_setprio(3);
 }
 
-template <int PROB, int REP, class MaskT, bool MULTI, int EPB, bool OBS = false, bool ROW = false>
+template <int PROB, int REP, class MaskT, bool MULTI, int EPB, bool OBS = false, bool ROW = false, bool PACK = false>
 __global__ __launch_bounds__(EPB * 4) __attribute__((amdgpu_waves_per_eu(4, 8))) void k_step(PcgrlParams P, DevBufs Bg, const int32_t* __restrict__ actions, int parity, int gen_map,
                                                                                                      int steps, size_t action_stride, double* reward_out, uint8_t* done_out, int32_t* info_out) {
     extern __shared__ __attribute__((aligned(16))) uint8_t smem[];
@@ -318,7 +318,7 @@
             const int want = lone ? (prio & 3) : (inc ? ((prio >> 4) & 3) : ((prio_nfull == 0 || wid - w_lone < prio_nfull) ? ((prio >> 2) & 3) : 0));
             if (want != prio_now) { prio_now = want; step_set_prio(want); }
         }
-        stats_wave_task<PROB, G, MaskT, true>(P, B, g, lane64, gw, lone, inc, PROB == PCGRL_PROB_ZELDA && pair, zinc, have, raw, lane64, MODE_STEP, parity, 1, gen_map, mt, tiles, rowmask, &s_loc, OBS);
+        stats_wave_task<PROB, G, MaskT, true, PACK>(P, B, g, lane64, gw, lone, inc, PROB == PCGRL_PROB_ZELDA && pair, zinc, have, raw, lane64, MODE_STEP, parity, 1, gen_map, mt, tiles, rowmask, &s_loc, OBS);
         TL(7);
     }
     if (prio_now) { prio_now = 0; step_set_prio(0); }
diff --git a/gym_pcgrl_amd/csrc/lanegroup_dev.h b/gym_pcgrl_amd/csrc/lanegroup_dev.h
--- a/gym_pcgrl_amd/csrc/lanegroup_dev.h
+++ b/gym_pcgrl_amd/csrc/lanegroup_dev.h
@@ -67,6 +67,19 @@
         uint32_t b = ballot(m != 0);
         int first = __ffs((int)b) - 1;
         return lane == first ? (m & (mask_t)(0 - m)) : (mask_t)0;
+    }
+    enum { kPack2 = sizeof(MaskT) == 4 ? 1 : 0 };
+    __device__ __forceinline__ mask_t top_bit(mask_t m) const { return m != 0 ? (mask_t)1 << (8 * (int)sizeof(mask_t) - 1 - (sizeof(mask_t) == 4 ? __clz((int)m) : __clzll((long long)m))) : (mask_t)0; }
+    __device__ __forceinline__ mask_t last_bit(mask_t m) const {
+        const uint32_t b = ballot(m != 0);
+        const int last = 31 - __clz((int)b);
+        return lane == last ? top_bit(m) : (mask_t)0;
+    }
+    __device__ __forceinline__ mask_t far_bit(mask_t m, mask_t a) const {
+        const uint32_t b = ballot(m != 0);
+        const int ra = __ffs((int)ballot(a != 0)) - 1, lo = __ffs((int)b) - 1, hi = 31 - __clz((int)b);
+        const bool use_last = hi - ra >= ra - lo;
+        return lane == (use_last ? hi : lo) ? (use_last ? top_bit(m) : (m & (mask_t)(0 - m))) : (mask_t)0;
     }
     __device__ __forceinline__ int sum(int v) const {
         v += __builtin_amdgcn_update_dpp(0, v, 0xB1, 0xF, 0xF, true);
diff --git a/gym_pcgrl_amd/csrc/pcgrl_abi.hip b/gym_pcgrl_amd/csrc/pcgrl_abi.hip
--- a/gym_pcgrl_amd/csrc/pcgrl_abi.hip
+++ b/gym_pcgrl_amd/csrc/pcgrl_abi.hip
@@ -22,6 +22,7 @@
 #define PART_SEARCH 5
 #define PART_SMB 6
 #define PART_STEP_SOLVER 7
+#define PART_STEP_BINARY_PACK 8
 
 #include "lanegroup_dev.h"
 #include "mt19937.h"
@@ -88,6 +89,7 @@
     int smb_replay;
     pcgrl_tuning tun;
     int no_wide, wide_waves, wide_grid, wide_pairs, fused_zelda, no_fused, step_epb, smb_heap, obs_at_end, no_inc;
+    int pack2;
     int profiling;
     int obs_incremental;
     const uint8_t* obs_synced;
@@ -306,6 +308,7 @@
     B.step_ipw = (i == 1 || i == 2) ? i : 4;
     B.step_touch = tun_or(T.no_touch, 0) ? 0 : 1;
     B.touch_resume = tun_or(T.touch_resume, 1) ? 1 : 0;
+    h->pack2 = tun_or(T.pack2, 1) ? 1 : 0;
     B.step_pair = tun_or(T.step_pair, 6);
     B.step_tight = B.step_touch ? tun_or(T.touch_tight, 1) : 0;
     h->no_inc = tun_or(T.no_inc, 0) != 0;
@@ -527,6 +530,7 @@
 PCGRL_LOCAL int launch_planes_from_map(pcgrl_env* h, const uint8_t* maps, hipStream_t st);
 PCGRL_LOCAL int launch_update(pcgrl_env* h, const int32_t* actions, int parity, hipStream_t st);
 PCGRL_LOCAL int launch_step_binary(pcgrl_env* h, const int32_t* actions, int parity, hipStream_t st, const RolloutArgs& R);
+PCGRL_LOCAL int launch_step_binary_pack(pcgrl_env* h, const int32_t* actions, int parity, hipStream_t st, const RolloutArgs& R);
 PCGRL_LOCAL int launch_step_zelda(pcgrl_env* h, const int32_t* actions, int parity, hipStream_t st, const RolloutArgs& R);
 PCGRL_LOCAL int launch_search(pcgrl_env* h, int32_t* sync, int list_a, int mode_a, int list_b, int mode_b, int parity, int rst_list, int clr, hipStream_t st);
 PCGRL_LOCAL int launch_smb(pcgrl_env* h, int32_t* sync, int list_a, int mode_a, int list_b, int mode_b, int parity, int rst_list, int clr, hipStream_t st, int inline_reset);
@@ -717,8 +721,8 @@
     return prob_ok && P.group == 16 && !P.big && P.rep <= PCGRL_REP_TURTLE && P.auto_reset &&
            h->B.inline_reset && !h->no_fused;
 }
-#if PCGRL_IN_PART(PART_STEP_BINARY) || PCGRL_IN_PART(PART_STEP_ZELDA)
-template <int PROB, class MaskT, int EPB>
+#if PCGRL_IN_PART(PART_STEP_BINARY) || PCGRL_IN_PART(PART_STEP_ZELDA) || PCGRL_IN_PART(PART_STEP_BINARY_PACK)
+template <int PROB, class MaskT, int EPB, bool PACK = false>
 static int launch_step_pme(pcgrl_env* h, const int32_t* actions, int parity, hipStream_t st, const RolloutArgs& R) {
     const PcgrlParams& P = h->P;
     const StepLds SL = step_lds_layout(16 * P.nplanes * (int)sizeof(MaskT), PROB == PCGRL_PROB_BINARY ? 16 * (int)sizeof(MaskT) : 0,
@@ -732,7 +736,7 @@
     return with_rep<PCGRL_REP_NARROW, PCGRL_REP_WIDE, PCGRL_REP_TURTLE>(P.rep, [&](auto rep) {
         constexpr int REP = rep();
         const auto go = [&](auto multi_t, auto obs_t, auto row_t) {
-            return launch<k_step<PROB, REP, MaskT, multi_t(), EPB, obs_t(), row_t()>>(h, grid, EPB * 4, lds, st, P, h->B, actions, parity, gen_flag(h), R.steps,
+            return launch<k_step<PROB, REP, MaskT, multi_t(), EPB, obs_t(), row_t(), PACK>>(h, grid, EPB * 4, lds, st, P, h->B, actions, parity, gen_flag(h), R.steps,
                                                                                     R.action_stride, R.reward_out, R.done_out, R.info_out);
         };
         constexpr std::true_type yes{};
@@ -759,13 +763,22 @@
     return launch_step_p<PCGRL_PROB_BINARY>(h, actions, parity, st, R);
 }
 #endif
+#if PCGRL_IN_PART(PART_STEP_BINARY_PACK)
+PCGRL_LOCAL int launch_step_binary_pack(pcgrl_env* h, const int32_t* actions, int parity, hipStream_t st, const RolloutArgs& R) {
+    if (h->step_epb == 128) return launch_step_pme<PCGRL_PROB_BINARY, uint32_t, 128, true>(h, actions, parity, st, R);
+    if (h->step_epb == 256) return launch_step_pme<PCGRL_PROB_BINARY, uint32_t, 256, true>(h, actions, parity, st, R);
+    return launch_step_pme<PCGRL_PROB_BINARY, uint32_t, 64, true>(h, actions, parity, st, R);
+}
+#endif
 #if PCGRL_IN_PART(PART_STEP_ZELDA)
 PCGRL_LOCAL int launch_step_zelda(pcgrl_env* h, const int32_t* actions, int parity, hipStream_t st, const RolloutArgs& R) {
     return launch_step_p<PCGRL_PROB_ZELDA>(h, actions, parity, st, R);
 }
 #endif
 static int launch_step(pcgrl_env* h, const int32_t* actions, int parity, hipStream_t st, const RolloutArgs& R = RolloutArgs{1, 0, nullptr, nullptr, nullptr}) {
-    return h->P.prob == PCGRL_PROB_BINARY ? launch_step_binary(h, actions, parity, st, R) : launch_step_zelda(h, actions, parity, st, R);
+    if (h->P.prob != PCGRL_PROB_BINARY) return launch_step_zelda(h, actions, parity, st, R);
+    const bool pack = h->pack2 && h->P.mask_bytes == 4 && h->P.width <= 15;
+    return pack ? launch_step_binary_pack(h, actions, parity, st, R) : launch_step_binary(h, actions, parity, st, R);
 }
 static int action_width(int rep) {
     return rep == PCGRL_REP_WIDE ? 3 : (rep == PCGRL_REP_NARROW_CAST || rep == PCGRL_REP_TURTLE_CAST) ? 2 : rep == PCGRL_REP_NARROW_MULTI ? 9 : 1;
diff --git a/gym_pcgrl_amd/csrc/pcgrl_algos.h b/gym_pcgrl_amd/csrc/pcgrl_algos.h
--- a/gym_pcgrl_amd/csrc/pcgrl_algos.h
+++ b/gym_pcgrl_amd/csrc/pcgrl_algos.h
@@ -230,6 +230,30 @@
     return pcg_component_fills(g, seed, c);
 }
 
+template <class...> struct PcgVoid { typedef void type; };
+template <class B, class = void> struct PcgPack2 { static constexpr bool on = false; };
+template <class B> struct PcgPack2<B, typename PcgVoid<decltype(B::kPack2)>::type> { static constexpr bool on = B::kPack2 != 0 && B::kGroup == 16; };
+template <class M> PCGRL_D M pcg_pack2(M pass) { return pass | (pass << 16); }
+
+template <class B>
+PCGRL_D void pcg_component2(B& g, typename B::mask_t seed_a, typename B::mask_t seed_b, const PcgFillCtx<B>& c2,
+                            typename B::mask_t& comp_a, typename B::mask_t& comp_b, int& size_a, int& size_b) {
+    typedef typename B::mask_t M;
+    PCGRL_TRACE(g, 3);
+    const M f = pcg_component_fills(g, seed_a | (seed_b << 16), c2);
+    comp_a = f & M(0xFFFFu);
+    comp_b = f >> 16;
+    int both;
+    g.popcount_sum3(comp_a, comp_b, comp_a & comp_b, size_a, size_b, both);
+    if (both > 0) { comp_b = comp_b ^ comp_b; size_b = 0; }
+}
+template <class M>
+PCGRL_D void pcg_rank(M comp, int size, M& big1, M& big2, int& size1, int& size2, int& size3) {
+    if (size > size1) { size3 = size2; size2 = size1; big2 = big1; size1 = size; big1 = comp; }
+    else if (size > size2) { size3 = size2; size2 = size; big2 = comp; }
+    else if (size > size3) size3 = size;
+}
+
 template <class B>
 PCGRL_D typename B::mask_t pcg_tiny_components(B& g, typename B::mask_t p, int& regions, int& path) {
     typedef typename B::mask_t M;
@@ -345,16 +369,18 @@
     return bfs_levels<false>(g, g.first_bit(last), comp, unused);
 }
 
-template <class B>
-PCGRL_D void regions_and_longest_path(B& g, typename B::mask_t pass, int& regions, int& path, typename B::mask_t& champ, int& ub2, bool tight = true) {
-    typedef typename B::mask_t M;
+template <bool PACK = false, class B>
+PCGRL_D void regions_and_longest_path(B& g, typename B::mask_t pass, int& regions, int& path, typename B::mask_t& champ, int& ub2, bool tight = true,
+                                      bool pack = false) {
+    typedef typename B::mask_t M;
+    constexpr bool kPack = PACK && PcgPack2<B>::on;
     regions = 0;
     path = 0;
     ub2 = -1;
     champ = pass ^ pass;
     const M nontiny = pass & ~pcg_tiny_components(g, pass, regions, path);
     if (!g.any(nontiny)) return;
-    const PcgFillCtx<B> ctx = pcg_fill_ctx(g, pass);
+    const PcgFillCtx<B> ctx = pcg_fill_ctx(g, (kPack && pack) ? pcg_pack2(pass) : pass);
     if (B::kGroup != 16) {
         typedef typename B::ivec_t I;
         M rest = nontiny;
@@ -371,14 +397,26 @@
     }
     M rest = nontiny, big1 = nontiny ^ nontiny, big2 = big1;
     int size1 = 0, size2 = 0, size3 = 0;
-    while (g.any(rest)) {
+    bool plain = true;
+    if constexpr (kPack) {
+        if (pack) {
+            plain = false;
+            while (g.any(rest)) {
+                M comp_a, comp_b;
+                int size_a, size_b;
+                pcg_component2(g, g.first_bit(rest), g.last_bit(rest), ctx, comp_a, comp_b, size_a, size_b);
+                rest = rest & ~(comp_a | comp_b);
+                regions += size_b > 0 ? 2 : 1;
+                pcg_rank(comp_a, size_a, big1, big2, size1, size2, size3);
+                pcg_rank(comp_b, size_b, big1, big2, size1, size2, size3);
+            }
+        }
+    }
+    while (plain && g.any(rest)) {
         const M comp = pcg_component(g, g.first_bit(rest), ctx);
         rest = rest & ~comp;
         ++regions;
-        const int size = g.popcount_sum(comp);
-        if (size > size1) { size3 = size2; size2 = size1; big2 = big1; size1 = size; big1 = comp; }
-        else if (size > size2) { size3 = size2; size2 = size; big2 = comp; }
-        else if (size > size3) size3 = size;
+        pcg_rank(comp, g.popcount_sum(comp), big1, big2, size1, size2, size3);
     }
     const int tiny_path = path;
     int bd1 = size1 - 1, bd2 = size2 - 1, who = 0;
@@ -535,11 +573,12 @@
     return binary_touch(g, pass_new, cbit, added, regions_old, champ_old, ub2_old, regions, path, champ, ub2, memo);
 }
 
-template <class B>
+template <bool PACK = false, class B>
 PCGRL_D void rlp_resume(B& g, typename B::mask_t pass, const TouchMemo<typename B::mask_t>& memo, int& regions, int& path,
-                        typename B::mask_t& champ, int& ub2, bool tight = true) {
+                        typename B::mask_t& champ, int& ub2, bool tight = true, bool pack = false) {
     typedef typename B::mask_t M;
     typedef typename B::ivec_t I;
+    constexpr bool kPack = PACK && PcgPack2<B>::on;
     regions = 0;
     path = 0;
     champ = pass ^ pass;
@@ -561,20 +600,33 @@
     if (known) regions = memo.regions;
     if (pend1) { size1 = g.popcount_sum(memo.comp1); size1 = memo.bd1 + 1 < size1 ? memo.bd1 + 1 : size1; }
     if (g.any(rest)) {
-        const PcgFillCtx<B> ctx = pcg_fill_ctx(g, pass);
+        const PcgFillCtx<B> ctx = pcg_fill_ctx(g, (kPack && pack) ? pcg_pack2(pass) : pass);
         while (g.any(rest)) {
             if (count == 0) {
                 const int n = g.popcount_sum(rest);
                 if (n - 1 <= path) { ub = n - 1 > ub ? n - 1 : ub; break; }
             }
             const I cnt = g.popc_lanes(rest);
-            const M comp = pcg_component(g, g.first_bit(g.keep_where_eq(cnt, g.imax(cnt), rest)), ctx);
-            rest = rest & ~comp;
-            regions += count;
-            const int size = g.popcount_sum(comp);
-            if (size > size1) { size3 = size2; size2 = size1; big2 = big1; size1 = size; big1 = comp; }
-            else if (size > size2) { size3 = size2; size2 = size; big2 = comp; }
-            else if (size > size3) size3 = size;
+            const M seed = g.first_bit(g.keep_where_eq(cnt, g.imax(cnt), rest));
+            bool plain = true;
+            if constexpr (kPack) {
+                if (pack) {
+                    plain = false;
+                    M comp_a, comp_b;
+                    int size_a, size_b;
+                    pcg_component2(g, seed, g.far_bit(rest, seed), ctx, comp_a, comp_b, size_a, size_b);
+                    rest = rest & ~(comp_a | comp_b);
+                    regions += size_b > 0 ? 2 * count : count;
+                    pcg_rank(comp_a, size_a, big1, big2, size1, size2, size3);
+                    pcg_rank(comp_b, size_b, big1, big2, size1, size2, size3);
+                }
+            }
+            if (plain) {
+                const M comp = pcg_component(g, seed, ctx);
+                rest = rest & ~comp;
+                regions += count;
+                pcg_rank(comp, g.popcount_sum(comp), big1, big2, size1, size2, size3);
+            }
         }
     }
     int b1 = size1 - 1, b2 = size2 - 1;
diff --git a/include/pcgrl_hip.h b/include/pcgrl_hip.h
--- a/include/pcgrl_hip.h
+++ b/include/pcgrl_hip.h
@@ -93,6 +93,7 @@
     int32_t big_team;
     int32_t obs_at_end;
     int32_t touch_resume;
+    int32_t pack2;
     int32_t changes_grid;
     int32_t changes_chunk;
 } pcgrl_tuning;
```

Result: no change. 2.428 billion env-steps/s (median of 6 runs) (+0.8%).
